# LongmaoTeamTf/deep_recommenders

Measured on AMD Instinct MI355X. Metric: examples/sec/node DeepFM (26 sparse feats, 10M vocab, dim 64), higher is better.
Workload: dtype f32; 1 GPU; DeepFM Criteo-shape synthetic training step (BASELINE.json configs[2]): 26 sparse + 13 dense, 10000000 vocab/field hashed on device, dim 64, DNN [256, 32]+[1] relu, sigmoid-CE, fused SGD; batch 65536 per GPU, ids uniform; tables on one GPU (66.6 GB); gemm_split=f16x2, global_batch=65536, parallelism=single, per_kernel_events=False

## Files before the change

### deep_recommenders_amd/_lib.py

```python
import ctypes
import os

_HERE = os.path.dirname(os.path.abspath(__file__))
SO_PATH = os.path.join(_HERE, "lib", "libdr_hotpath.so")

_i64, _i32, _u64, _f32, _p = ctypes.c_int64, ctypes.c_int32, ctypes.c_uint64, ctypes.c_float, ctypes.c_void_p

SIGNATURES = {
    "dr_hash_bucket_i64": [_p, _i64, _i32, _p, _p, _p],
    "dr_hash_bucket_bytes": [_p, _p, _i64, _u64, _p, _p],
    "dr_vocab_lookup_i64": [_p, _i64, _p, _i32, _p, _p],
    "dr_vocab_lookup_bytes": [_p, _p, _i64, _p, _p, _i32, _p, _p],
    "dr_emb_pool_fwd": [_p, _i64, _i32, _i32, _p, _p, _p, _i32, _p, _p, _p, _i64, _p, _p, _p],
    "dr_emb_pool_bwd": [_p, _i64, _i32, _i32, _p, _p, _i32, _p, _i64, _p, _i64, _p, _p, _f32, _p, _p, _p, _p],
    "dr_fm2_fwd": [_p, _i64, _i32, _i32, _p, _p],
    "dr_fm2_bwd": [_p, _p, _i64, _i32, _i32, _p, _p],
    "dr_linear_fwd": [_p, _i64, _p, _i64, _p, _i64, _i32, _i32, _i32, _p, _i64, _p],
    "dr_linear_bwd_dx": [_p, _i64, _p, _i64, _i64, _i32, _i32, _p, _i64, _i32, _p, _i64, _p],
    "dr_linear_bwd_dw": [_p, _i64, _p, _i64, _i64, _i32, _i32, _f32, _p, _i64, _p, _p, _i64, _p],
    "dr_emb_pool_fwd_ex": [_p, _i64, _i32, _i32, _p, _p, _p, _i32, _p, _p, _p, _i64, _p, _p, _i32, _p],
    "dr_lin_fields_fwd": [_p, _i64, _i32, _i32, _p, _p, _p, _p, _i64, _p],
    "dr_lin_fields_bwd": [_p, _i64, _i32, _i32, _p, _p, _p, _i64, _f32, _p, _p],
    "dr_emb_pool_bwd_sorted_adam": [_p, _p, _p, _p, _p, _p, _p, _i64, _i32, _i32, _i64, _p, _i64, _p, _i64, _p, _p, _p, _f32, _f32,
                                    _f32, _f32, _p, _p, _p, _p, _p, _p, _p, _p],
    "dr_emb_pool_bwd_sorted_adam_ex": [_p, _p, _p, _p, _p, _p, _p, _i64, _i32, _i32, _i64, _p, _i64, _p, _i64, _p, _p, _p, _f32, _f32,
                                    _f32, _f32, _p, _p, _p, _p, _p, _p, _p, _p, _p, _p],
    "dr_adam_step": [_p, _p, _p, _p, _i64, _f32, _f32, _f32, _f32, _f32, _p],
    "dr_ftrl_step": [_p, _p, _p, _p, _i64, _f32, _f32, _f32, _f32, _f32, _p],
    "dr_linear_bwd_dw_workspace_bytes": [_i64, _i32, _i32],
    "dr_linear_bwd_narrow_workspace_bytes": [_i64, _i32, _i32],
    "dr_tower_head_workspace_bytes": [_i64],
    "dr_tower_head_fwd_bwd": [_p, _i64, _p, _i64, _p, _i64, _i64, _i32, _i32, _i32, _p, _i64, _p, _p, _p, _i32, _f32, _p, _i64, _p,
                              _p, _i64, _p, _p, _p, _i64, _p, _p, _i64, _p],
    "dr_linear_bwd_narrow": [_p, _i64, _p, _i64, _p, _i64, _i64, _i32, _i32, _i32, _f32, _p, _i64, _p, _p, _i64, _p, _i64, _p],
    "dr_linear_bwd_narrow_parts": [_p, _i64, _p, _i64, _p, _i64, _i64, _i32, _i32, _i32, _f32, _p, _i64, _p, _p, _i64, _p, _i64, _i32, _p],
    "dr_linear_bwd_narrow_amax": [_p, _i64, _p, _i64, _p, _i64, _i64, _i32, _i32, _i32, _f32, _p, _i64, _p, _p, _i64, _p, _i64, _i32, _p, _p],
    "dr_tower_head_fwd_bwd_parts": [_p, _i64, _p, _i64, _p, _i64, _i64, _i32, _i32, _i32, _p, _i64, _p, _p, _p, _i32, _f32, _p, _i64, _p,
                                    _p, _i64, _p, _p, _p, _i64, _p, _p, _i64, _i32, _p],
    "dr_cross_fwd": [_p, _p, _i64, _p, _i64, _p, _f32, _i64, _i32, _p, _p, _p],
    "dr_cross_combine_bwd": [_p, _p, _p, _i64, _i32, _i64, _f32, _p, _p, _p, _p],
    "dr_bce_fwd_bwd": [_p, _p, _i64, _p, _i64, _i32, _p, _p, _p, _p, _p],
    "dr_sigmoid_fwd": [_p, _i64, _p, _p],
    "dr_sigmoid_bwd": [_p, _p, _i64, _p, _p],
    "dr_bce_prob_fwd_bwd": [_p, _p, _i64, _i32, _p, _p, _p, _p],
    "dr_shard_bucket_workspace_bytes": [_i64, _i32],
    "dr_shard_bucket_ids": [_p, _i64, _i32, _i64, _i32, _p, _p, _p, _p, _p],
    "dr_shard_bucket_ids_dedup": [_p, _p, _i64, _i32, _i64, _i32, _p, _p, _p, _p, _p],
    "dr_shard_dedup_slots": [_p, _p, _p, _i64, _i64, _p, _p],
    "dr_rows_gather": [_p, _i64, _p, _i32, _p, _p, _p, _p],
    "dr_rows_scatter_add": [_p, _i64, _p, _i32, _p, _f32, _p, _p, _p],
    "dr_axpy": [_i64, _f32, _p, _p, _p],
    "dr_emb_pack_grads": [_p, _i64, _i32, _i32, _p, _i64, _p, _i64, _p, _p, _p, _p, _p, _p],
    "dr_emb_pack_grads_dedup": [_p, _p, _i64, _i32, _i32, _p, _i64, _p, _i64, _p, _p, _p, _p, _p, _p],
    "dr_emb_sort_workspace_bytes": [_i64],
    "dr_emb_sort_slots": [_p, _i64, _i32, _p, _i64, _p, _p, _p, _p, _p, _p, _i64, _p],
    "dr_hash_sort_slots": [_p, _i64, _i32, _p, _p, _p, _p, _i64, _p, _p, _p, _p, _p, _p, _i64, _p],
    "dr_emb_plan_set_small_limit": [_i32],
    "dr_adam_catchup_rows": [_p, _i64, _i32, _p, _i32, _p, _p, _p, _p, _p, _p, _p, _i32, _i32, _f32, _f32, _f32, _f32, _p],
    "dr_emb_pool_bwd_sorted": [_p, _p, _p, _p, _p, _p, _p, _i64, _i32, _i32, _i64, _p, _i64, _p, _i64, _p, _p, _p, _f32, _p, _p,
                               _p, _p, _p],
    "dr_emb_pool_bwd_sorted_parts": [_p, _p, _p, _p, _p, _p, _p, _i64, _i32, _i32, _i64, _p, _i64, _p, _i64, _p, _p, _p, _f32, _p, _p,
                                     _p, _p, _i32, _p],
    "dr_emb_pool_bwd_sorted_ex": [_p, _p, _p, _p, _p, _p, _p, _i64, _i32, _i32, _i64, _p, _i64, _p, _i64, _p, _p, _p, _f32, _p, _p,
                                  _p, _p, _p, _i32, _p, _p],
    "dr_emb_lin_update_unique": [_p, _p, _i64, _i32, _p, _p, _p, _f32, _p, _p],
    "dr_emb_snapshot_sorted_rows": [_p, _p, _p, _p, _i32, _i64, _p, _p],
    "dr_ids_transpose_i32": [_p, _i64, _i32, _p, _p],
    "dr_linear_bwd_dx_fm": [_p, _i64, _p, _i64, _i64, _i32, _i32, _p, _p, _p, _i64, _i32, _i32, _p, _i64, _p],
    "dr_inbatch_softmax_workspace_bytes": [_i64],
    "dr_inbatch_softmax_fwd": [_p, _p, _i64, _i32, _p, _p, _p, _f32, _p, _p, _p, _p, _i64, _p],
    "dr_inbatch_softmax_grad_scores": [_p, _p, _i64, _i32, _p, _p, _p, _f32, _p, _f32, _p, _i64, _p],
    "dr_inbatch_softmax_grad_scores_ws": [_p, _p, _i64, _i32, _p, _p, _p, _f32, _p, _f32, _p, _i64, _p, _i64, _p],
    "dr_scores_nt": [_p, _i64, _p, _i64, _i64, _i32, _i32, _p, _i64, _p],
    "dr_topk_select": [_p, _i64, _i64, _i64, _i32, _i64, _i32, _p, _p, _p],
    "dr_topk_workspace_bytes": [_i64, _i64, _i32],
    "dr_topk_mips": [_p, _i64, _p, _i64, _i32, _i32, _i64, _i32, _p, _p, _p, _i64, _p],
    "dr_topk_index_bytes": [_i64, _i32],
    "dr_topk_index_build": [_p, _i64, _i32, _p, _i64, _p],
    "dr_topk_mips_indexed": [_p, _i64, _p, _p, _i64, _i32, _i32, _i64, _i32, _p, _p, _p, _i64, _p],
    "dr_ivf_pack": [_p, _i64, _i32, _p, _p, _p, _i32, _i64, _p, _p, _p, _p],
    "dr_ivf_scan": [_p, _i64, _i32, _p, _i32, _p, _p, _p, _i32, _p, _p, _p],
    "dr_topk_merge": [_p, _p, _i32, _p, _p, _i32, _i64, _i32, _p, _p, _p],
    "dr_rowdot": [_p, _p, _i64, _i32, _p, _p],
    "dr_rows_scale": [_p, _p, _i32, _p, _i64, _i32, _p, _p],
    "dr_gather_i64": [_p, _i64, _p, _i64, _p, _p],
    "dr_take_along_rows_f32": [_p, _i64, _i64, _i32, _p, _i32, _p, _p],
    "dr_take_along_rows_i64": [_p, _i64, _i64, _i32, _p, _i32, _p, _p],
    "dr_topk_hits": [_p, _p, _i64, _i32, _p, _i32, _p, _p],
    "dr_exclude_adjust": [_p, _p, _i64, _i32, _p, _i32, _p, _p],
    "dr_logits_adjust": [_p, _p, _i64, _i32, _p, _p, _f32, _p, _p],
    "dr_softmax_ce_rows": [_p, _p, _i64, _i32, _f32, _p, _p, _p, _p],
    "dr_softmax_ce_rows_bwd": [_p, _p, _i64, _i32, _f32, _p, _f32, _p, _p, _i64, _p],
    "dr_bf3_split": [_p, _i64, _i64, _i32, _p, _i64, _i64, _i64, _i64, _i32, _p],
    "dr_bf3_join": [_p, _i64, _i64, _i64, _i32, _p, _i64, _p],
    "dr_bf3_gemm_nt": [_p, _i64, _i64, _p, _i64, _i64, _i64, _i32, _i32, _p, _i32, _p, _i64, _p, _i64, _p],
    "dr_bf3_linear_nt": [_p, _i64, _p, _i64, _i64, _i64, _i32, _i32, _p, _i32, _p, _i64, _i32, _p, _i64, _p],
    "dr_bf3_linear_nt_pack": [_p, _i64, _p, _i64, _i64, _i64, _i32, _i32, _p, _i32, _p, _p, _p, _i64, _p, _p, _p, _p],
    "dr_h2_linear_nt_pack": [_p, _i64, _p, _p, _i64, _i64, _p, _i64, _i32, _i32, _p, _i32, _p, _p, _p, _i64, _p, _p, _p, _p],
    "dr_bf3_cross_fwd": [_p, _p, _i64, _p, _i64, _i64, _p, _f32, _i64, _i32, _p, _p, _p],
    "dr_linear_fwd_splitk_workspace_bytes": [_i64, _i32, _i32],
    "dr_linear_fwd_splitk": [_p, _i64, _p, _i64, _i64, _i32, _i32, _p, _i64, _p, _i64, _p],
    "dr_bf3_emb_linear_fwd": [_p, _i64, _i32, _p, _i64, _p, _i32, _p, _p, _p, _p, _i64, _i32, _p, _i64, _i64, _i32, _p, _i32, _p, _p, _p, _i64, _p],
    "dr_bf3_emb_linear_fwd_lv": [_p, _i64, _i32, _p, _i64, _p, _i32, _p, _p, _p, _p, _i64, _i32, _p, _i64, _i64, _i32, _p, _i32, _p, _p, _p, _i64,
                                 _p, _p],
    "dr_bf3_wgrad_workspace_bytes": [_i64, _i32, _i32],
    "dr_bf3_wgrad": [_p, _i64, _p, _i64, _i64, _i32, _i32, _f32, _p, _i64, _p, _p, _i64, _p],
    "dr_bf3_wgrad_emb": [_p, _i64, _i32, _p, _p, _i32, _p, _p, _i64, _i32, _i32, _f32, _p, _i64, _p, _p, _i64, _p],
    "dr_bf3_wgrad_emb_parts": [_p, _i64, _i32, _p, _p, _i32, _p, _p, _i64, _i32, _i32, _f32, _p, _i64, _p, _p, _i64, _i32, _p],
    "dr_bf3_gemm_tn_workspace_bytes": [_i64, _i32, _i32],
    "dr_bf3_gemm_tn": [_p, _i64, _i64, _p, _i64, _i64, _i64, _i32, _i32, _f32, _p, _i64, _p, _p, _p, _i64, _p],
    "dr_h2_amax": [_p, _i64, _i64, _i32, _p, _i32, _p],
    "dr_h2_split": [_p, _i64, _i64, _i32, _p, _i64, _i64, _i64, _i64, _i32, _p, _p],
    "dr_h2_refresh_weight": [_p, _i64, _i64, _i32, _p, _i64, _i64, _p, _i64, _i64, _p, _p, _p],
    "dr_h2_linear_nt": [_p, _i64, _p, _p, _i64, _i64, _p, _i64, _i32, _i32, _p, _i32, _p, _i64, _i32, _p, _i64, _p, _p],
    "dr_h2_cross_fwd": [_p, _p, _i64, _p, _p, _i64, _i64, _p, _p, _f32, _i64, _i32, _p, _p, _p, _p],
    "dr_h2_dgrad_emb_sgd": [_p, _i64, _p, _p, _i64, _i64, _p, _i64, _i32, _i32, _p, _p, _p, _p, _p, _p, _p, _p, _f32, _p, _i64, _p, _p],
    "dr_cross_combine_bwd_amax": [_p, _p, _p, _i64, _i32, _i64, _f32, _p, _p, _p, _p, _p],
    "dr_h2_emb_linear_fwd": [_p, _i64, _i32, _p, _i64, _p, _i32, _p, _p, _p, _p, _p, _p, _i64, _i32, _p, _i64, _i64, _p, _i32, _p, _i32,
                             _p, _p, _p, _i64, _p, _p],
    "dr_h2_wgrad": [_p, _i64, _p, _p, _i64, _p, _i64, _i32, _i32, _f32, _p, _i64, _p, _p, _i64, _p],
    "dr_h2_wgrad_emb": [_p, _i64, _i32, _p, _p, _i32, _p, _p, _p, _p, _i64, _p, _i32, _i32, _f32, _p, _i64, _p, _p, _i64, _i32, _p],
    "dr_cin_fwd": [_p, _p, _i64, _i32, _i32, _i32, _p, _i32, _p, _i32, _p, _p],
    "dr_cin_bwd": [_p, _p, _i64, _i32, _i32, _i32, _p, _i32, _i32, _p, _p, _p, _p, _p, _p, _p],
    "dr_cin_pool_fwd": [_p, _p, _i64, _i32, _i32, _i32, _p, _i32, _p, _i32, _p, _p, _p],
    "dr_cin_pool_bwd_workspace_bytes": [_i64, _i32, _i32, _i32, _i32],
    "dr_cin_pool_bwd": [_p, _p, _i64, _i32, _i32, _i32, _p, _i32, _i32, _p, _p, _p, _p, _i32, _p, _p, _p, _p, _i64, _p],
    "dr_din_concat_fwd": [_p, _p, _i64, _i32, _i32, _p, _i64, _p],
    "dr_din_concat_bwd": [_p, _p, _i64, _i32, _i32, _p, _i64, _p, _p, _p],
    "dr_act_fwd": [_p, _i64, _i32, _i64, _i32, _p],
    "dr_act_bwd": [_p, _i64, _p, _i64, _i64, _i32, _i32, _p],
    "dr_dropout_fwd": [_p, _i64, _i64, _i32, _f32, _u64, _p, _i64, _p, _p],
    "dr_dropout_bwd": [_p, _i64, _p, _i64, _i32, _f32, _p, _i64, _p],
    "dr_reduce_sum": [_p, _i64, _i32, _f32, _i32, _p, _p, _p],
    "dr_clock_stamp": [_p, _p],
    "dr_tower_tail_workspace_bytes": [_i64, _i32],
    "dr_tower_tail_fused": [_p, _i64, _p, _i64, _p, _i64, _i64, _i32, _i32, _p, _i64, _p, _p, _p, _i32, _f32, _p, _i64, _p, _p, _i64, _p,
                            _p, _p, _p, _i64, _p, _i64, _p, _p, _i64, _i32, _p, _p],
    "dr_copy_nt": [_p, _p, _i64, _p],
    "dr_ivf_build_workspace_bytes": [_i64, _i32],
    "dr_ivf_build_lists": [_p, _i64, _i32, _p, _p, _p, _i64, _p],
    "dr_linear_fwd_grouped": [_p, _i64, _i64, _p, _i64, _i64, _p, _i64, _i64, _i32, _i32, _i32, _i32, _p, _i64, _i64, _p],
    "dr_linear_bwd_dx_grouped": [_p, _i64, _i64, _p, _i64, _i64, _i64, _i32, _i32, _i32, _p, _i64, _i64, _i32, _p, _i64, _i64, _p],
    "dr_linear_bwd_dw_grouped_workspace_bytes": [_i64, _i32, _i32, _i32],
    "dr_linear_bwd_dw_grouped": [_p, _i64, _i64, _p, _i64, _i64, _i64, _i32, _i32, _i32, _f32, _p, _i64, _i64, _p, _i64, _p, _i64, _p],
    "dr_mmoe_gate_mix_fwd": [_p, _i64, _p, _i64, _i64, _i32, _i32, _i32, _p, _i64, _p, _i64, _p],
    "dr_mmoe_gate_mix_bwd": [_p, _i64, _p, _i64, _p, _i64, _i64, _i32, _i32, _i32, _p, _i64, _p, _i64, _p],
    "dr_mse_workspace_bytes": [_i32],
    "dr_mse_fwd_bwd": [_p, _i64, _p, _i64, _i64, _i32, _p, _p, _i64, _p, _i64, _p],
    "dr_esmm_head_fwd": [_p, _i64, _i64, _p, _p, _p, _p],
    "dr_esmm_head_bwd": [_p, _p, _p, _p, _p, _i64, _p, _i64, _p],
    "dr_adam_step_2d": [_p, _i64, _p, _i64, _p, _p, _i64, _i64, _i32, _f32, _f32, _f32, _f32, _f32, _p],
    "dr_gather_cols": [_p, _i64, _p, _i64, _p, _i64, _i32, _p, _i64, _p],
    "dr_csr_plan_bytes": [_i64],
    "dr_csr_plan_workspace_bytes": [_i64],
    "dr_csr_plan": [_p, _i64, _i64, _p, _i64, _p, _i64, _p],
    "dr_csr_spmm_workspace_bytes": [_i64, _i32],
    "dr_csr_spmm": [_p, _p, _p, _i64, _i64, _p, _i64, _i32, _p, _i64, _i32, _p, _i64, _p, _p, _i64, _p],
    "dr_csr_transpose_workspace_bytes": [_i64, _i64],
    "dr_csr_transpose": [_p, _p, _p, _i64, _i64, _i64, _p, _p, _p, _p, _i64, _p],
    "dr_softmax_rows_fwd": [_p, _i64, _i64, _i32, _p, _i64, _p],
    "dr_softmax_rows_bwd": [_p, _i64, _p, _i64, _i64, _i32, _p, _i64, _p],
    "dr_cce_prob_rows": [_p, _i64, _p, _i64, _i64, _i32, _p, _p, _p, _i64, _p],
    "dr_attn_fwd": [_p, _i64, _p, _i64, _p, _i64, _p, _i32, _i32, _i32, _i32, _i32, _i32, _f32, _u64, _p, _i64, _p, _p],
    "dr_attn_bwd": [_p, _i64, _p, _i64, _p, _i64, _p, _p, _i64, _p, _i32, _i32, _i32, _i32, _i32, _i32, _f32, _u64, _p, _i64,
                    _p, _i64, _p, _i64, _p, _p],
    "dr_add_layernorm_fwd": [_p, _i64, _p, _i64, _p, _p, _i64, _i32, _f32, _p, _i64, _p, _p],
    "dr_add_layernorm_bwd_workspace_bytes": [_i64, _i32],
    "dr_add_layernorm_bwd": [_p, _i64, _p, _i64, _p, _p, _p, _i64, _i64, _i32, _p, _i64, _p, _p, _p, _i64, _p],
    "dr_token_embedding_fwd": [_p, _i64, _i32, _p, _i64, _i32, _p, _f32, _u64, _p, _i64, _p],
    "dr_token_embedding_bwd": [_p, _p, _i64, _i64, _i32, _p, _i64, _f32, _u64, _p, _p],
    "dr_dice_fwd": [_p, _i64, _p, _i64, _i32, _f32, _p, _i64, _p],
    "dr_dice_bwd_workspace_bytes": [_i64, _i32],
    "dr_dice_bwd": [_p, _i64, _p, _p, _i64, _i64, _i32, _f32, _p, _i64, _p, _p, _i64, _p],
    "dr_din_pool_fwd": [_p, _i64, _p, _i64, _p, _p, _p, _p, _p, _p, _i64, _i32, _i32, _i32, _i32, _i32, _f32, _p, _i64, _p, _p],
    "dr_din_pool_bwd_workspace_bytes": [_i64, _i32, _i32, _i32],
    "dr_din_pool_bwd": [_p, _i64, _p, _i64, _p, _p, _p, _p, _p, _p, _p, _i64, _p, _i64, _i32, _i32, _i32, _i32, _i32, _f32,
                        _p, _i64, _p, _i64, _p, _p, _p, _p, _p, _p, _i64, _p],
    "dr_confusion_hist_workspace_bytes": [_i64, _i32],
    "dr_confusion_hist_update": [_p, _p, _p, _i64, _p, _i32, _i32, _p, _p, _p],
    "dr_version": [],
    "dr_set_gemm_mode": [_i32],
    "dr_get_gemm_mode": [],
    "dr_set_gemm_split": [_i32],
    "dr_get_gemm_split": [],
}
_RESTYPE = {"dr_version": ctypes.c_char_p, "dr_shard_bucket_workspace_bytes": ctypes.c_int64,
            "dr_emb_sort_workspace_bytes": ctypes.c_int64, "dr_tower_tail_workspace_bytes": ctypes.c_int64, "dr_ivf_build_workspace_bytes": ctypes.c_int64,
            "dr_linear_bwd_dw_workspace_bytes": ctypes.c_int64,
            "dr_linear_fwd_splitk_workspace_bytes": ctypes.c_int64,
            "dr_bf3_gemm_tn_workspace_bytes": ctypes.c_int64,
            "dr_bf3_wgrad_workspace_bytes": ctypes.c_int64,
            "dr_linear_bwd_narrow_workspace_bytes": ctypes.c_int64,
            "dr_tower_head_workspace_bytes": ctypes.c_int64,
            "dr_inbatch_softmax_workspace_bytes": ctypes.c_int64, "dr_topk_workspace_bytes": ctypes.c_int64,
            "dr_topk_index_bytes": ctypes.c_int64,
            "dr_linear_bwd_dw_grouped_workspace_bytes": ctypes.c_int64, "dr_mse_workspace_bytes": ctypes.c_int64,
            "dr_csr_plan_bytes": ctypes.c_int64, "dr_csr_plan_workspace_bytes": ctypes.c_int64,
            "dr_csr_spmm_workspace_bytes": ctypes.c_int64, "dr_csr_transpose_workspace_bytes": ctypes.c_int64,
            "dr_add_layernorm_bwd_workspace_bytes": ctypes.c_int64,
            "dr_dice_bwd_workspace_bytes": ctypes.c_int64, "dr_din_pool_bwd_workspace_bytes": ctypes.c_int64,
            "dr_confusion_hist_workspace_bytes": ctypes.c_int64, "dr_cin_pool_bwd_workspace_bytes": ctypes.c_int64}

DR_OK, DR_EINVAL, DR_ELAUNCH, DR_ESHAPE = 0, -1, -2, -3
_ERR = {DR_EINVAL: "DR_EINVAL (bad argument)", DR_ELAUNCH: "DR_ELAUNCH (HIP launch error)",
        DR_ESHAPE: "DR_ESHAPE (shape contract violated)"}

_LIB = None


class HotPathLibraryMissing(RuntimeError):
    pass


def lib():
    global _LIB
    if _LIB is None:
        if not os.path.exists(SO_PATH):
            raise HotPathLibraryMissing(
                "HIP hot-path library not built: %s is missing. Build it with "
                "`python -m deep_recommenders_amd.build` (or __graft_entry__.build()). "
                "There is no CPU/PyTorch fallback." % SO_PATH)
        L = ctypes.CDLL(SO_PATH)
        for name, args in SIGNATURES.items():
            fn = getattr(L, name)
            fn.argtypes = args
            fn.restype = _RESTYPE.get(name, ctypes.c_int)
        _LIB = L
    return _LIB


def check(status, what):
    if status != DR_OK:
        raise RuntimeError("%s failed: %s" % (what, _ERR.get(status, status)))


def ptr(t):
    if t is None:
        return None
    if not t.is_cuda:
# ... 18 lines not shown
```

### deep_recommenders_amd/csrc/bf3_planes.hip

```cpp
#include "bf3_rs_core.h"

namespace {

using namespace drrs;

constexpr int NWAVES = 8;
constexpr int NTHREADS = 64 * NWAVES;

struct NtArgs {
    const __bf16* A; int64_t a_ps, a_ld;
    const __bf16* B; int64_t b_ps, b_ld;
    int64_t M; int32_t N; int32_t K;
    float* C; int64_t ldc;
    const float* bias; int32_t act;
    const float* mask; int64_t ld_mask;
};


template <int NW, int DBG = 0>
__global__ __launch_bounds__(64 * NW, NW / 4) void bf3_gemm_nt_pipe_kernel(NtArgs g) {
    constexpr int BM = 128, BN = 128, NS = 3;
    constexpr int WN = 4, WM = NW / WN, TM = BM / (32 * WM);
    constexpr int A_PLANE = BM * 64, B_PLANE = BN * 64;
    constexpr int STAGE = 3 * (A_PLANE + B_PLANE);
// ... 480 lines not shown
                                                       _Float16* __restrict__ planes, int64_t ps, int64_t ldp, int64_t r0,
                                                       int64_t c0, int32_t transpose, const uint32_t* __restrict__ amax) {
    float sc, inv;
    h2_scale_of(amax[0], sc, inv);
    h2_mode_on();
    const int64_t total = R * C, stride = (int64_t)gridDim.x * blockDim.x;
    if (!transpose && (C & 3) == 0 && (ldp & 3) == 0 && (c0 & 3) == 0 && (ld_src & 3) == 0 && (reinterpret_cast<uintptr_t>(src) & 15) == 0 &&
        (reinterpret_cast<uintptr_t>(planes) & 7) == 0 && (ps & 3) == 0 && total < (int64_t)0x7fffffff) {
        typedef _Float16 f16x4 __attribute__((ext_vector_type(4)));
        typedef float f32x4 __attribute__((ext_vector_type(4)));
        const unsigned cq = (unsigned)C >> 2, tq = (unsigned)(total >> 2);
        for (unsigned i = blockIdx.x * blockDim.x + threadIdx.x; i < tq; i += (unsigned)stride) {
            const unsigned r = i / cq, c = (i - r * cq) << 2;
            const f32x4 v = *reinterpret_cast<const f32x4*>(src + (int64_t)r * ld_src + c) * sc;
            const f16x4 h = __builtin_convertvector(v, f16x4);
            const f16x4 l = __builtin_convertvector(v - __builtin_convertvector(h, f32x4), f16x4);
            const int64_t off = (r0 + r) * ldp + c0 + c;
            *reinterpret_cast<f16x4*>(planes + off) = h;
            *reinterpret_cast<f16x4*>(planes + ps + off) = l;
        }
        return;
    }
    for (int64_t i = (int64_t)blockIdx.x * blockDim.x + threadIdx.x; i < total; i += stride) {
        int64_t r, c, off;
        if (!transpose) { r = i / C; c = i - r * C; off = (r0 + r) * ldp + c0 + c; }
        else { c = i / R; r = i - c * R; off = (r0 + c) * ldp + c0 + r; }
        const float v = src[r * ld_src + c] * sc;
        const _Float16 h = (_Float16)v;
        planes[off] = h;
        planes[ps + off] = (_Float16)(v - (float)h);
    }
}

constexpr int H2_REFRESH_PARTS = 256;
__global__ __launch_bounds__(256) void h2_amax_parts_kernel(const float* __restrict__ src, int64_t ld, int64_t R, int32_t C,
                                                            uint32_t* __restrict__ parts) {
    uint32_t m = 0u;
    const int64_t total = R * (int64_t)C, stride = (int64_t)gridDim.x * blockDim.x;
    for (int64_t i = (int64_t)blockIdx.x * blockDim.x + threadIdx.x; i < total; i += stride) {
        const int64_t r = i / C;
        m = max(m, __float_as_uint(fabsf(src[r * ld + (i - r * C)])));
    }
#pragma unroll
    for (int o = 32; o > 0; o >>= 1) m = max(m, (uint32_t)__shfl_xor((int)m, o, 64));
    __shared__ uint32_t wm[4];
    if ((threadIdx.x & 63) == 0) wm[threadIdx.x >> 6] = m;
    __syncthreads();
    if (threadIdx.x == 0) parts[blockIdx.x] = max(max(wm[0], wm[1]), max(wm[2], wm[3]));
}
__global__ __launch_bounds__(256) void h2_split_both_kernel(const float* __restrict__ src, int64_t ld, int64_t R, int32_t C,
                                                            _Float16* __restrict__ w, int64_t w_ps, int64_t w_ld,
                                                            _Float16* __restrict__ wt, int64_t wt_ps, int64_t wt_ld,
                                                            const uint32_t* __restrict__ parts, int32_t nparts, uint32_t* __restrict__ amax) {
    uint32_t m = (int)threadIdx.x < nparts ? parts[threadIdx.x] : 0u;
#pragma unroll
    for (int o = 32; o > 0; o >>= 1) m = max(m, (uint32_t)__shfl_xor((int)m, o, 64));
    __shared__ uint32_t wm[4];
    if ((threadIdx.x & 63) == 0) wm[threadIdx.x >> 6] = m;
    __syncthreads();
    m = max(max(wm[0], wm[1]), max(wm[2], wm[3]));
    if (blockIdx.x == 0 && threadIdx.x == 0) amax[0] = m;
    float sc, inv;
    h2_scale_of(m, sc, inv);
    h2_mode_on();
    const int64_t total = R * (int64_t)C, stride = (int64_t)gridDim.x * blockDim.x;
    for (int64_t i = (int64_t)blockIdx.x * blockDim.x + threadIdx.x; i < 2 * total; i += stride) {
        int64_t r, c, off;
        _Float16* dst;
        int64_t ps;
        if (i < total) { r = i / C; c = i - r * C; off = r * w_ld + c; dst = w; ps = w_ps; }
        else { const int64_t j = i - total; c = j / R; r = j - c * R; off = c * wt_ld + r; dst = wt; ps = wt_ps; }
        const float v = src[r * ld + c] * sc;
        const _Float16 h = (_Float16)v;
        dst[off] = h;
        dst[ps + off] = (_Float16)(v - (float)h);
    }
}

__global__ __launch_bounds__(256) void bf3_join_kernel(const __bf16* __restrict__ planes, int64_t ps, int64_t ldp, int64_t R,
                                                       int32_t C, float* __restrict__ dst, int64_t ld_dst) {
    const int64_t total = R * C, stride = (int64_t)gridDim.x * blockDim.x;
    for (int64_t i = (int64_t)blockIdx.x * blockDim.x + threadIdx.x; i < total; i += stride) {
        const int64_t r = i / C;
        const int c = (int)(i - r * C);
        const int64_t off = r * ldp + c;
        dst[r * ld_dst + c] = bf3::join(planes[off], planes[ps + off], planes[2 * ps + off]);
    }
}

}

extern "C" int dr_bf3_split(const float* src, int64_t ld_src, int64_t R, int32_t C, void* planes, int64_t plane_stride,
                            int64_t ld_planes, int64_t row_offset, int64_t col_offset, int32_t transpose,
                            dr_stream_t stream) {
    if (R < 0 || C < 0 || ld_src < C || row_offset < 0 || col_offset < 0 || ld_planes <= 0 || plane_stride <= 0) return DR_EINVAL;
    if (R == 0 || C == 0) return DR_OK;
    if (!src || !planes) return DR_EINVAL;
    if (!transpose && col_offset + C > ld_planes) return DR_EINVAL;
    if (transpose && col_offset + R > ld_planes) return DR_EINVAL;
    hipLaunchKernelGGL(bf3_split_kernel, dim3(dr_grid_for(R * ((C + 3) / 4), 256)), dim3(256), 0, dr_s(stream), src, ld_src, R, C,
                       static_cast<__bf16*>(planes), plane_stride, ld_planes, row_offset, col_offset, transpose);
    DR_CHECK_LAUNCH();
    return DR_OK;
}

extern "C" int dr_bf3_join(const void* planes, int64_t plane_stride, int64_t ld_planes, int64_t R, int32_t C, float* dst,
                           int64_t ld_dst, dr_stream_t stream) {
    if (R < 0 || C < 0 || ld_planes < C || ld_dst < C || plane_stride <= 0) return DR_EINVAL;
    if (R == 0 || C == 0) return DR_OK;
    if (!planes || !dst) return DR_EINVAL;
    hipLaunchKernelGGL(bf3_join_kernel, dim3(dr_grid_for(R * C, 256)), dim3(256), 0, dr_s(stream),
                       static_cast<const __bf16*>(planes), plane_stride, ld_planes, R, C, dst, ld_dst);
    DR_CHECK_LAUNCH();
    return DR_OK;
}

extern "C" int dr_bf3_gemm_nt(const void* a_planes, int64_t a_plane_stride, int64_t a_ld, const void* b_planes,
                              int64_t b_plane_stride, int64_t b_ld, int64_t M, int32_t N, int32_t K, const float* bias,
                              int32_t act, const float* mask, int64_t ld_mask, float* C, int64_t ldc, dr_stream_t stream) {
    if (M < 0 || N <= 0 || K <= 0 || (K % BK) != 0 || act < 0 || act > 1) return DR_EINVAL;
    if (M == 0) return DR_OK;
    if (!planes_ok(a_planes, a_plane_stride, a_ld) || !planes_ok(b_planes, b_plane_stride, b_ld) || !C) return DR_EINVAL;
    if (a_ld < K || b_ld < K || ldc < N || (mask != nullptr && ld_mask < N)) return DR_EINVAL;
    NtArgs g{static_cast<const __bf16*>(a_planes), a_plane_stride, a_ld, static_cast<const __bf16*>(b_planes), b_plane_stride, b_ld,
             M, N, K, C, ldc, bias, act, mask, ld_mask};
    const int64_t tiles = ((M + 127) / 128) * ((N + 127) / 128);
    if (tiles > 0x7fffffff) return DR_EINVAL;
    const int grid = (int)(tiles < 256 ? tiles : 256);
    hipLaunchKernelGGL((bf3_gemm_nt_pipe_kernel<16>), dim3(grid), dim3(1024), 0, dr_s(stream), g);
    DR_CHECK_LAUNCH();
    return DR_OK;
// ... 14 lines not shown
    if (workspace_bytes < dr_bf3_gemm_tn_workspace_bytes(R, F, N)) return DR_EINVAL;
    TnArgs g{static_cast<const __bf16*>(x_planes), x_plane_stride, x_ld, static_cast<const __bf16*>(y_planes), y_plane_stride, y_ld,
             R, F, N, 0, 0, static_cast<float*>(workspace)};
    int split = tn_split_for(R, F, N, 128, 256);
    const int64_t rpad = (R + BK - 1) / BK * BK;
    g.per = ((rpad + split - 1) / split + BK - 1) / BK * BK;
    g.split = (int32_t)((rpad + g.per - 1) / g.per);
    const int64_t tiles = (int64_t)((F + 127) / 128) * ((N + 255) / 256) * g.split;
    const int grid = (int)(tiles < 256 ? tiles : 256);
    hipLaunchKernelGGL((bf3_gemm_tn_kernel<2, 4>), dim3(grid), dim3(NTHREADS), 0, dr_s(stream), g);
    hipLaunchKernelGGL(bf3_splitk_reduce_kernel, dim3(dr_grid_for((int64_t)F * N, 256)), dim3(256), 0, dr_s(stream), g.partial,
                       g.split, (int64_t)F, N, scale, dst, ld_dst, y_colsum, dstb);
    DR_CHECK_LAUNCH();
    return DR_OK;
}

extern "C" int dr_h2_amax(const float* src, int64_t ld, int64_t R, int32_t C, uint32_t* amax, int32_t reset, dr_stream_t stream) {
    if (R < 0 || C < 0 || ld < C || !amax) return DR_EINVAL;
    if (reset && hipMemsetAsync(amax, 0, sizeof(uint32_t), dr_s(stream)) != hipSuccess) return DR_ELAUNCH;
    if (R == 0 || C == 0) return DR_OK;
    if (!src) return DR_EINVAL;
    const int grid = (ld == C || R == 1) ? dr_grid_for(R * ((C + 3) / 4), 256 * 4) : (int)(R < 4096 ? R : 4096);
    hipLaunchKernelGGL(h2_amax_kernel, dim3(grid), dim3(256), 0, dr_s(stream), src, ld, R, C, amax);
    DR_CHECK_LAUNCH();
    return DR_OK;
}

extern "C" int dr_h2_split(const float* src, int64_t ld_src, int64_t R, int32_t C, void* planes, int64_t plane_stride,
                           int64_t ld_planes, int64_t row_offset, int64_t col_offset, int32_t transpose, const uint32_t* amax,
                           dr_stream_t stream) {
    if (R < 0 || C < 0 || ld_src < C || row_offset < 0 || col_offset < 0 || ld_planes <= 0 || plane_stride <= 0 || !amax) return DR_EINVAL;
    if (R == 0 || C == 0) return DR_OK;
    if (!src || !planes) return DR_EINVAL;
    if (!transpose && col_offset + C > ld_planes) return DR_EINVAL;
    if (transpose && col_offset + R > ld_planes) return DR_EINVAL;
    hipLaunchKernelGGL(h2_split_kernel, dim3(dr_grid_for(R * (int64_t)C, 256)), dim3(256), 0, dr_s(stream), src, ld_src, R, C,
                       static_cast<_Float16*>(planes), plane_stride, ld_planes, row_offset, col_offset, transpose, amax);
    DR_CHECK_LAUNCH();
    return DR_OK;
}

extern "C" int dr_h2_refresh_weight(const float* W, int64_t ldw, int64_t K, int32_t N, void* w_planes, int64_t w_ps, int64_t w_ld,
                                    void* wt_planes, int64_t wt_ps, int64_t wt_ld, uint32_t* amax, uint32_t* parts, dr_stream_t stream) {
    if (K <= 0 || N <= 0 || ldw < N || !W || !w_planes || !wt_planes || !amax || !parts) return DR_EINVAL;
    if (w_ld < N || wt_ld < K || w_ps <= 0 || wt_ps <= 0) return DR_EINVAL;
    const int64_t total = K * (int64_t)N;
    const int np = (int)(total < (int64_t)H2_REFRESH_PARTS * 256 ? (total + 255) / 256 : H2_REFRESH_PARTS);
    hipLaunchKernelGGL(h2_amax_parts_kernel, dim3(np), dim3(256), 0, dr_s(stream), W, ldw, K, N, parts);
    hipLaunchKernelGGL(h2_split_both_kernel, dim3(dr_grid_for(2 * total, 256, 2048)), dim3(256), 0, dr_s(stream), W, ldw, K, N,
                       static_cast<_Float16*>(w_planes), w_ps, w_ld, static_cast<_Float16*>(wt_planes), wt_ps, wt_ld, parts, np, amax);
    DR_CHECK_LAUNCH();
    return DR_OK;
}
```

### deep_recommenders_amd/csrc/bf3_wgrad.hip

```cpp
#ifndef DR_NT_WGRAD_GATHER
#define DR_NT_WGRAD_GATHER 0
#endif
#include "bf3_rs_core.h"

namespace {

using namespace drrs;

struct TnRsArgs {
    const float* X; int64_t ldx;
    const float* Y; int64_t ldy;
    int64_t R; int32_t F; int32_t N;
    int64_t per; int32_t split;
    float* partial; float* colsum;
    const int32_t* ids_t; const int64_t* row_base; const float* table; int32_t nf; const float* dense_pad;
    const uint32_t* x_amax; const uint32_t* x2_amax; const uint32_t* y_amax;
};

template <int GATHER, int H2 = 0>
__global__ __launch_bounds__(512, 2) void bf3_gemm_tn_rs_kernel(TnRsArgs g) {
    constexpr int NW = 8, BMF = 32 * NW, BN = 256, NT = BN / 32;
    constexpr int NPL = RS_NPL<H2>, B_PLANE = RS_B_PLANE, STAGE = RS_STAGE<H2>;
    __shared__ __attribute__((aligned(1024))) unsigned char smem[2 * STAGE];

// ... 156 lines not shown
#pragma unroll
            for (int s = 0; s < 2; ++s) {
#pragma unroll
                for (int j = 0; j < 8; ++j) v[j] = xa[8 * s + j];
                if constexpr (H2) h2_split8v(v, h2_sx, fa[s][0], fa[s][1]);
                else rs_split8v(v, fa[s][0], fa[s][1], fa[s][2]);
            }
        }
        if (kt + 1 < nk) stage_b(stage ^ 1);
        __builtin_amdgcn_sched_barrier(0);
        if (GATHER) {
            load_gather(xa, idv, r_begin + (int64_t)(kt + 1) * BK);
            idv = load_ids(r_begin + (int64_t)(kt + 2) * BK);
        } else {
            load_raw(xa, g.X, g.ldx, xoff, r_begin + (int64_t)(kt + 1) * BK);
        }
        load_raw(yb, g.Y, g.ldy, yoff, r_begin + (int64_t)(kt + 2) * BK);
        __builtin_amdgcn_sched_barrier(0);
#pragma unroll
        for (int q = 0; q < 16; ++q) {
            if (q < 14) {
                rs_wait_frag<NPL, NPL>(fb[q & 3]);
                read_b((q + 2) & 3, stage, q + 2);
            } else if (q == 14) {
                rs_wait_frag<NPL, 0>(fb[2]);
                asm volatile("s_barrier" ::: "memory");
                if (kt + 1 < nk) read_b(0, stage ^ 1, 0);
            } else {
                if (kt + 1 < nk) read_b(1, stage ^ 1, 1);
            }
            __builtin_amdgcn_sched_barrier(0);
#pragma unroll
            for (int term = 0; term < RS_TERMS<H2>; ++term) acc[q & 7] = rs_mma_term<H2>(term, fa[q >> 3], fb[q & 3], acc[q & 7]);
            __builtin_amdgcn_sched_barrier(0);
        }
    }
    float* out = g.partial + ((int64_t)slice * Fp + f0 + wave * 32 + 4 * hi) * Np + n0 + l31;
#pragma unroll
    for (int nt = 0; nt < NT; ++nt)
#pragma unroll
        for (int reg = 0; reg < 16; ++reg) out[(int64_t)((reg & 3) + 8 * (reg >> 2)) * Np + nt * 32] = acc[nt][reg];
    if (want_cs) {
        cs += __shfl_xor(cs, 32, 64);
        if (hi == 0) g.colsum[(int64_t)slice * Np + n0 + wave * 32 + l31] = cs;
    }
}

template <int V>
__global__ __launch_bounds__(64) void bf3_tn_rs_reduce_kernel(const float* __restrict__ partial, const float* __restrict__ colsum,
                                                              int32_t split, int32_t F, int32_t N, int32_t Fp, int32_t Np,
                                                              float scale, float* __restrict__ dst, int64_t ld,
                                                              float* __restrict__ dstb, const uint32_t* __restrict__ x_amax = nullptr,
                                                              const uint32_t* __restrict__ x2_amax = nullptr,
                                                              const uint32_t* __restrict__ y_amax = nullptr) {
    typedef float vec_t __attribute__((ext_vector_type(V)));
    const int f = blockIdx.x;
    const int n = ((int)blockIdx.y * 64 + (int)threadIdx.x) * V;
    if (n >= N) return;
    const int64_t ps = (int64_t)Fp * Np;
    float wscale = scale;
    if (x_amax != nullptr) {
        float sx, ix, sy, iy;
        h2_scale_of(max(x_amax[0], x2_amax != nullptr ? x2_amax[0] : 0u), sx, ix);
        h2_scale_of(y_amax[0], sy, iy);
        wscale = scale * (ix * iy);
    }
    auto sum_slices = [&](const float* p, int64_t stride) -> vec_t {
        vec_t acc = 0.f;
        int s = 0;
        for (; s + 8 <= split; s += 8) {
            vec_t v[8];
#pragma unroll
            for (int u = 0; u < 8; ++u) v[u] = *reinterpret_cast<const vec_t*>(p + (s + u) * stride);
#pragma unroll
            for (int u = 0; u < 8; ++u) acc += v[u];
        }
        for (; s < split; ++s) acc += *reinterpret_cast<const vec_t*>(p + s * stride);
        return acc;
    };
    const vec_t acc = sum_slices(partial + (int64_t)f * Np + n, ps);
    float* d = dst + (int64_t)f * ld + n;
    if (V == 1 || n + V <= N) {
        vec_t o = *reinterpret_cast<vec_t*>(d);
#pragma unroll
        for (int c = 0; c < V; ++c) o[c] = fmaf(wscale, acc[c], o[c]);
        *reinterpret_cast<vec_t*>(d) = o;
    } else {
#pragma unroll
        for (int c = 0; c < V; ++c)
            if (n + c < N) d[c] = fmaf(wscale, acc[c], d[c]);
    }
    if (f == 0 && colsum != nullptr && dstb != nullptr) {
        const vec_t cacc = sum_slices(colsum + n, Np);
#pragma unroll
        for (int c = 0; c < V; ++c)
            if (n + c < N) dstb[n + c] = fmaf(scale, cacc[c], dstb[n + c]);
    }
}

void launch_tn_rs_reduce(const float* partial, const float* colsum, int split, int32_t F, int32_t N, int Fp, int Np, float scale,
                         float* dst, int64_t ld, float* dstb, const uint32_t* x_amax, const uint32_t* x2_amax, const uint32_t* y_amax,
                         dr_stream_t stream) {
    const bool vec = ((reinterpret_cast<uintptr_t>(partial) | reinterpret_cast<uintptr_t>(dst)) & 15) == 0 && (ld & 3) == 0;
    if (vec)
        hipLaunchKernelGGL(bf3_tn_rs_reduce_kernel<4>, dim3(F, (N + 255) / 256), dim3(64), 0, dr_s(stream), partial, colsum, split, F, N,
                           Fp, Np, scale, dst, ld, dstb, x_amax, x2_amax, y_amax);
    else
        hipLaunchKernelGGL(bf3_tn_rs_reduce_kernel<1>, dim3(F, (N + 63) / 64), dim3(64), 0, dr_s(stream), partial, colsum, split, F, N,
                           Fp, Np, scale, dst, ld, dstb, x_amax, x2_amax, y_amax);
}

void tn_rs_plan(int64_t R, int32_t F, int32_t N, int& split, int64_t& per, int& Fp, int& Np) {
    const int tf = (F + 255) / 256, tn = (N + 255) / 256;
    Fp = tf * 256;
    Np = tn * 256;
    int64_t sp = 256 / ((int64_t)tf * tn);
    const int64_t max_split = (R + 16 * BK - 1) / (16 * BK);
    if (sp > max_split) sp = max_split;
    if (sp < 1) sp = 1;
    per = ((R + sp - 1) / sp + BK - 1) / BK * BK;
    split = (int)((R + per - 1) / per);
}
}

extern "C" int64_t dr_bf3_wgrad_workspace_bytes(int64_t R, int32_t F, int32_t N) {
    if (R <= 0 || F <= 0 || N <= 0) return 0;
    int split, Fp, Np;
    int64_t per;
    tn_rs_plan(R, F, N, split, per, Fp, Np);
    return ((int64_t)split * Fp * Np + (int64_t)split * Np) * (int64_t)sizeof(float);
}

static int wgrad_impl(const float* x, int64_t ld_x, const float* dy, int64_t ld_dy, int64_t R, int32_t F, int32_t N,
                      float scale, float* dstW, int64_t ld_w, float* dstb, void* workspace, int64_t workspace_bytes,
                      dr_stream_t stream, const uint32_t* x_amax = nullptr, const uint32_t* dy_amax = nullptr) {
    if (R <= 0 || F <= 0 || N <= 0) return DR_EINVAL;
    if (!x || !dy || !dstW || !workspace || ld_x < F || ld_dy < N || ld_w < N) return DR_EINVAL;
    if (workspace_bytes < dr_bf3_wgrad_workspace_bytes(R, F, N)) return DR_EINVAL;
    int split, Fp, Np;
    int64_t per;
    tn_rs_plan(R, F, N, split, per, Fp, Np);
    float* partial = static_cast<float*>(workspace);
    float* colsum = partial + (int64_t)split * Fp * Np;
    TnRsArgs g{x, ld_x, dy, ld_dy, R, F, N, per, split, partial, dstb != nullptr ? colsum : nullptr, nullptr, nullptr, nullptr, 0, nullptr,
               x_amax, nullptr, dy_amax};
    const int grid = (Fp / 256) * (Np / 256) * split;
    if (x_amax != nullptr) hipLaunchKernelGGL((bf3_gemm_tn_rs_kernel<0, 1>), dim3(grid), dim3(512), 0, dr_s(stream), g);
    else hipLaunchKernelGGL((bf3_gemm_tn_rs_kernel<0, 0>), dim3(grid), dim3(512), 0, dr_s(stream), g);
    launch_tn_rs_reduce(partial, dstb != nullptr ? colsum : nullptr, split, F, N, Fp, Np, scale, dstW, ld_w, dstb, x_amax, nullptr, dy_amax,
                        stream);
    DR_CHECK_LAUNCH();
    return DR_OK;
}

extern "C" int dr_bf3_wgrad(const float* x, int64_t ld_x, const float* dy, int64_t ld_dy, int64_t R, int32_t F, int32_t N,
                            float scale, float* dstW, int64_t ld_w, float* dstb, void* workspace, int64_t workspace_bytes,
                            dr_stream_t stream) {
    return wgrad_impl(x, ld_x, dy, ld_dy, R, F, N, scale, dstW, ld_w, dstb, workspace, workspace_bytes, stream);
}

extern "C" int dr_h2_wgrad(const float* x, int64_t ld_x, const uint32_t* x_amax, const float* dy, int64_t ld_dy, const uint32_t* dy_amax,
                           int64_t R, int32_t F, int32_t N, float scale, float* dstW, int64_t ld_w, float* dstb, void* workspace,
                           int64_t workspace_bytes, dr_stream_t stream) {
    if (!x_amax || !dy_amax) return DR_EINVAL;
    return wgrad_impl(x, ld_x, dy, ld_dy, R, F, N, scale, dstW, ld_w, dstb, workspace, workspace_bytes, stream, x_amax, dy_amax);
}

static int wgrad_emb_impl(const int32_t* ids_t, int64_t R, int32_t nf, const int64_t* row_base, const float* table, int32_t D,
                          const float* dense_pad, const float* dy, int64_t ld_dy, int32_t F, int32_t N, float scale, float* dstW,
                          int64_t ld_w, float* dstb, void* workspace, int64_t workspace_bytes, int32_t parts, dr_stream_t stream,
                          const uint32_t* table_amax = nullptr, const uint32_t* dense_amax = nullptr, const uint32_t* dy_amax = nullptr) {
    if (R <= 0 || F <= 0 || N <= 0 || nf <= 0) return DR_EINVAL;
    if (table_amax != nullptr && (!dy_amax || (F > 64 * nf && !dense_amax))) return DR_EINVAL;
    if (D != 64 || F < 64 * nf || F > 64 * nf + 32) return DR_ESHAPE;
    if (!ids_t || !row_base || !table || !dy || !dstW || !workspace || ld_dy < N || ld_w < N) return DR_EINVAL;
    if (F > 64 * nf && !dense_pad) return DR_EINVAL;
    if (workspace_bytes < dr_bf3_wgrad_workspace_bytes(R, F, N)) return DR_EINVAL;
    int split, Fp, Np;
    int64_t per;
    tn_rs_plan(R, F, N, split, per, Fp, Np);
    float* partial = static_cast<float*>(workspace);
    float* colsum = partial + (int64_t)split * Fp * Np;
    TnRsArgs g{nullptr, 0, dy, ld_dy, R, F, N, per, split, partial, dstb != nullptr ? colsum : nullptr, ids_t, row_base, table, nf,
               F > 64 * nf ? dense_pad : nullptr, table_amax, F > 64 * nf ? dense_amax : nullptr, dy_amax};
    const int grid = (Fp / 256) * (Np / 256) * split;
    if (parts & 1) {
        if (table_amax != nullptr) hipLaunchKernelGGL((bf3_gemm_tn_rs_kernel<1, 1>), dim3(grid), dim3(512), 0, dr_s(stream), g);
        else hipLaunchKernelGGL((bf3_gemm_tn_rs_kernel<1, 0>), dim3(grid), dim3(512), 0, dr_s(stream), g);
    }
    if (parts & 2)
        launch_tn_rs_reduce(partial, dstb != nullptr ? colsum : nullptr, split, F, N, Fp, Np, scale, dstW, ld_w, dstb, table_amax,
                            F > 64 * nf ? dense_amax : nullptr, dy_amax, stream);
    DR_CHECK_LAUNCH();
    return DR_OK;
}

extern "C" int dr_bf3_wgrad_emb(const int32_t* ids_t, int64_t R, int32_t nf, const int64_t* row_base, const float* table, int32_t D,
                                const float* dense_pad, const float* dy, int64_t ld_dy, int32_t F, int32_t N, float scale, float* dstW,
                                int64_t ld_w, float* dstb, void* workspace, int64_t workspace_bytes, dr_stream_t stream) {
    return wgrad_emb_impl(ids_t, R, nf, row_base, table, D, dense_pad, dy, ld_dy, F, N, scale, dstW, ld_w, dstb, workspace, workspace_bytes,
                          3, stream);
}

extern "C" int dr_bf3_wgrad_emb_parts(const int32_t* ids_t, int64_t R, int32_t nf, const int64_t* row_base, const float* table, int32_t D,
                                      const float* dense_pad, const float* dy, int64_t ld_dy, int32_t F, int32_t N, float scale,
                                      float* dstW, int64_t ld_w, float* dstb, void* workspace, int64_t workspace_bytes, int32_t parts,
                                      dr_stream_t stream) {
    if (parts < 1 || parts > 3) return DR_EINVAL;
    return wgrad_emb_impl(ids_t, R, nf, row_base, table, D, dense_pad, dy, ld_dy, F, N, scale, dstW, ld_w, dstb, workspace, workspace_bytes,
                          parts, stream);
}

extern "C" int dr_h2_wgrad_emb(const int32_t* ids_t, int64_t R, int32_t nf, const int64_t* row_base, const float* table, int32_t D,
                               const uint32_t* table_amax, const float* dense_pad, const uint32_t* dense_amax, const float* dy, int64_t ld_dy,
                               const uint32_t* dy_amax, int32_t F, int32_t N, float scale, float* dstW, int64_t ld_w, float* dstb,
                               void* workspace, int64_t workspace_bytes, int32_t parts, dr_stream_t stream) {
    if (parts < 1 || parts > 3 || !table_amax || !dy_amax) return DR_EINVAL;
    return wgrad_emb_impl(ids_t, R, nf, row_base, table, D, dense_pad, dy, ld_dy, F, N, scale, dstW, ld_w, dstb, workspace, workspace_bytes,
                          parts, stream, table_amax, dense_amax, dy_amax);
}
```

### deep_recommenders_amd/csrc/dr_common.h

```cpp
#pragma once
#include <hip/hip_runtime.h>
#include <stdint.h>
#include "../../include/dr_hotpath.h"

#define DR_WAVE 64

#define DR_CHECK_LAUNCH()                                   \
    do {                                                    \
        hipError_t e__ = hipGetLastError();                 \
        if (e__ != hipSuccess) return DR_ELAUNCH;           \
    } while (0)

static inline hipStream_t dr_s(dr_stream_t s) { return reinterpret_cast<hipStream_t>(s); }

static inline int dr_grid_for(int64_t work_items, int items_per_block, int max_blocks = 2048) {
    int64_t g = (work_items + items_per_block - 1) / items_per_block;
    if (g < 1) g = 1;
    if (g > max_blocks) g = max_blocks;
    return (int)g;
}

__device__ __forceinline__ float dr_wave_sum(float v) {
#pragma unroll
    for (int o = 32; o > 0; o >>= 1) v += __shfl_xor(v, o, 64);
    return v;
}

__host__ __device__ __forceinline__ uint32_t dr_mix32(uint64_t seed, uint64_t idx) {
    uint64_t z = idx * 0x9E3779B97F4A7C15ull + seed;
    z = (z ^ (z >> 30)) * 0xBF58476D1CE4E5B9ull;
    z = (z ^ (z >> 27)) * 0x94D049BB133111EBull;
    return (uint32_t)((z ^ (z >> 31)) >> 32);
}
__host__ __device__ __forceinline__ uint32_t dr_drop_thresh(float rate) {
    return (uint32_t)fminf(4294967040.f, rate * 4294967296.f);
}

__device__ __forceinline__ float dr_sigmoidf(float x) { return 1.f / (1.f + expf(-x)); }

__device__ __forceinline__ void dr_bce_terms(float x, float z, int mode, float& p, float& l, float& g) {
    p = 1.f / (1.f + expf(-x));
    if (mode == 0) {
        l = fmaxf(x, 0.f) - x * z + log1pf(expf(-fabsf(x)));
        g = p - z;
    } else {
        const float eps = 1e-7f;
        float pc = p;
        float dclip = 1.f;
        if (mode == 2) {
            if (p < eps) { pc = eps; dclip = 0.f; }
            else if (p > 1.f - eps) { pc = 1.f - eps; dclip = 0.f; }
        }
        l = -z * logf(pc + eps) - (1.f - z) * logf(1.f - pc + eps);
        const float dl_dp = -z / (pc + eps) + (1.f - z) / (1.f - pc + eps);
        g = dl_dp * dclip * p * (1.f - p);
    }
}

__device__ __forceinline__ void dr_block_sum_axpy(const float* __restrict__ x, int64_t n, float alpha,
                                                  float* __restrict__ dst) {
    __shared__ float dr_wsum_[4];
    float acc = 0.f;
    const int64_t nv = (reinterpret_cast<uintptr_t>(x) & 15) == 0 ? (n >> 2) : 0;
    const float4* x4 = reinterpret_cast<const float4*>(x);
    for (int64_t i = threadIdx.x; i < nv; i += 256 * 4) {
        float4 a[4];
#pragma unroll
        for (int j = 0; j < 4; ++j) {
            const int64_t q = i + j * 256;
            a[j] = x4[q < nv ? q : i];
            if (q >= nv) a[j] = make_float4(0.f, 0.f, 0.f, 0.f);
        }
#pragma unroll
        for (int j = 0; j < 4; ++j) acc += (a[j].x + a[j].y) + (a[j].z + a[j].w);
    }
    for (int64_t i = (nv << 2) + threadIdx.x; i < n; i += 256) acc += x[i];
    acc = dr_wave_sum(acc);
    if ((threadIdx.x & 63) == 0) dr_wsum_[threadIdx.x >> 6] = acc;
// ... 4 lines not shown
```

### deep_recommenders_amd/csrc/emb_plan.hip

```cpp
#include "dr_common.h"
#include "hash_i64.h"
#include <atomic>

namespace {

constexpr int CH = 32;
constexpr uint32_t EMPTY = 0xFFFFFFFFu;
constexpr uint32_t DUPBIT = 0x80000000u;
constexpr int SMALL_CAP = 16384;
constexpr int RADIX_BITS = 8, RADIX = 1 << RADIX_BITS;
constexpr int NBK = RADIX, CAPB = 128;
constexpr int LDS_TAB_MAX_LOG = 15;
constexpr int RADIX_CHUNK = 1664, RADIX_MAX_BLOCKS = 1024;
constexpr int MARK_BLOCKS = 512, MARK_MAX_CHUNK = 8192;
static_assert(NBK * CAPB >= SMALL_CAP, "buckets must hold the largest SMALL list");

std::atomic<int> g_small_limit{SMALL_CAP};

struct Ctrl {
    int32_t large;
    int32_t pad[3];
    int32_t bcnt[NBK];
};

size_t align_up(size_t v, size_t a) { return (v + a - 1) / a * a; }

unsigned bits_for(uint64_t v) {
    unsigned b = 1;
    while (b < 64 && (v >> b) != 0) ++b;
    return b;
}

__device__ __forceinline__ unsigned bits_for_dev(uint32_t v) { return v == 0 ? 1u : 32u - (unsigned)__clz((int)v); }

int radix_blocks(int64_t n) {
    int64_t nb = (n + RADIX_CHUNK - 1) / RADIX_CHUNK;
    return (int)(nb < 1 ? 1 : (nb > RADIX_MAX_BLOCKS ? RADIX_MAX_BLOCKS : nb));
}

struct Layout {
    size_t keys_x, vals_x, blist, ghist, tot, ctrl, total;
};
Layout layout_for(int64_t n) {
    Layout L{};
    size_t off = 0;
    L.keys_x = off; off += align_up((size_t)n * 8, 256);
    L.vals_x = off; off += align_up((size_t)n * 4, 256);
    L.blist = off;  off += align_up((size_t)NBK * CAPB * 8, 256);
    L.ghist = off;  off += align_up((size_t)RADIX * RADIX_MAX_BLOCKS * 4, 256);
    L.tot = off;    off += align_up((size_t)RADIX * 4, 256);
    L.ctrl = off;   off += align_up(sizeof(Ctrl), 256);
    L.total = off;
    return L;
}

template <int MODE>
__device__ __forceinline__ uint32_t digit_of(uint64_t k, uint32_t shift_or_mul) {
    if (MODE == 0) return (uint32_t)(k >> shift_or_mul) & (RADIX - 1);
    const uint32_t d = (uint32_t)(((k >> 24) * shift_or_mul) >> 32);
    return d < RADIX - 1 ? d : RADIX - 1;
}

__global__ __launch_bounds__(256) void radix_make_keys_kernel(const int64_t* __restrict__ ids, int32_t n, int32_t F,
                                                              const int64_t* __restrict__ row_base, uint64_t sentinel,
                                                              uint64_t* __restrict__ keys, uint32_t* __restrict__ vals) {
    const int32_t stride = gridDim.x * blockDim.x;
    for (int32_t p = blockIdx.x * blockDim.x + threadIdx.x; p < n; p += stride) {
        const int64_t id = ids[p];
        const uint64_t r0 = id >= 0 ? (uint64_t)(row_base[p % F] + id) : sentinel;
        keys[p] = r0 < sentinel ? r0 : sentinel;
        vals[p] = (uint32_t)p;
    }
}

constexpr int FRONT_GROUP = 4;
template <bool HASH, bool TRANS>
__global__ __launch_bounds__(256) void plan_front_kernel(const int64_t* __restrict__ src, int64_t B, int32_t F,
                                                         const uint64_t* __restrict__ col_buckets, int64_t* __restrict__ ids_out,
                                                         int32_t* __restrict__ ids_t, const int64_t* __restrict__ row_base,
                                                         uint64_t sentinel, uint32_t mul, int32_t sub, uint64_t* __restrict__ keys,
                                                         uint32_t* __restrict__ ghist) {
    extern __shared__ uint64_t fsm[];
    __shared__ uint32_t h[RADIX];
    int64_t* rb = reinterpret_cast<int64_t*>(fsm);
    uint64_t* cb = fsm + F;
    int32_t* tile = reinterpret_cast<int32_t*>(fsm + (HASH ? 3 : 1) * F);
    const int nb = gridDim.x, t = threadIdx.x;
    for (int c = t; c < F; c += 256) {
        rb[c] = row_base[c];
        if (HASH) {
            const uint64_t nbk = col_buckets[c];
            cb[c] = nbk;
            cb[F + c] = nbk != 0 ? ~0ull / nbk : 0;
        }
    }
    h[t] = 0;
    __syncthreads();
    const int64_t e0 = (int64_t)blockIdx.x * sub;
    const int64_t e1 = e0 + sub < B ? e0 + sub : B;
    for (int64_t g0 = e0; g0 < e1; g0 += 64) {
        const int ge = (int)(e1 - g0 < 64 ? e1 - g0 : 64);
        const int ns = ge * F;
        const int64_t p0 = g0 * F;
        for (int q = t; q < ns; q += 256) {
            const int r = q / F, f = q - r * F;
            const int64_t p = p0 + q;
            int64_t id = src[p];
            if (HASH) {
                id = drhash::bucket_of_key(id, cb[f], cb[F + f]);
                ids_out[p] = id;
            }
            if (TRANS) tile[r * (F + 1) + f] = (int32_t)id;
            const uint64_t r0 = id >= 0 ? (uint64_t)(rb[f] + id) : sentinel;
            const uint64_t row = r0 < sentinel ? r0 : sentinel;
            const uint64_t ck = (row << 24) | (uint32_t)p;
            keys[p] = ck;
            atomicAdd(&h[digit_of<1>(ck, mul)], 1u);
        }
        if (TRANS) {
            __syncthreads();
            for (int q = t; q < F * 64; q += 256) {
                const int f = q >> 6, r = q & 63;
                if (r < ge) ids_t[(int64_t)f * B + g0 + r] = tile[r * (F + 1) + f];
            }
            __syncthreads();
        }
    }
    __syncthreads();
    ghist[t * nb + blockIdx.x] = h[t];
}

__global__ __launch_bounds__(256) void radix_hist_kernel(const uint64_t* __restrict__ keys, int32_t n, uint32_t shift,
                                                         uint32_t* __restrict__ ghist) {
    __shared__ uint32_t h[RADIX];
    const int nb = gridDim.x, t = threadIdx.x;
    const int32_t chunk = (n + nb - 1) / nb;
    const int32_t beg = (int32_t)blockIdx.x * chunk, end = beg + chunk < n ? beg + chunk : n;
    h[t] = 0;
    __syncthreads();
    for (int32_t i = beg + t; i < end; i += 256) atomicAdd(&h[digit_of<0>(keys[i], shift)], 1u);
    __syncthreads();
    ghist[t * nb + blockIdx.x] = h[t];
}

template <bool ZERO>
__global__ __launch_bounds__(256) void radix_scan_kernel(uint32_t* __restrict__ ghist, int32_t nb, uint32_t* __restrict__ tot,
                                                         Ctrl* __restrict__ ctrl, int32_t* __restrict__ dup_count) {
    if (ZERO && blockIdx.x == 0) {
        int32_t* c = reinterpret_cast<int32_t*>(ctrl);
        for (int i = threadIdx.x; i < (int)(sizeof(Ctrl) / 4); i += 256) c[i] = 0;
        if (threadIdx.x < 2) dup_count[threadIdx.x] = 0;
    }
    __shared__ uint32_t part[256];
    const int t = threadIdx.x, d = blockIdx.x;
    const int32_t per = (nb + 255) / 256;
    const int32_t beg = t * per, end = beg + per < nb ? beg + per : nb;
    uint32_t* col = ghist + (int64_t)d * nb;
    uint32_t sum = 0;
    for (int32_t i = beg; i < end; ++i) sum += col[i];
    part[t] = sum;
    __syncthreads();
    for (int o = 1; o < 256; o <<= 1) {
        const uint32_t x = t >= o ? part[t - o] : 0u;
        __syncthreads();
        part[t] += x;
        __syncthreads();
    }
    uint32_t run = part[t] - sum;
    for (int32_t i = beg; i < end; ++i) {
        const uint32_t c = col[i];
        col[i] = run;
        run += c;
    }
    if (t == 255) tot[d] = part[255];
}

__global__ __launch_bounds__(256) void radix_scatter_kernel(const uint64_t* __restrict__ kin, const uint32_t* __restrict__ vin,
                                                            uint64_t* __restrict__ kout, uint32_t* __restrict__ vout, int32_t n,
                                                            uint32_t shift, const uint32_t* __restrict__ ghist,
                                                            const uint32_t* __restrict__ tot) {
    __shared__ uint32_t running[RADIX];
    __shared__ uint32_t wcnt[4][RADIX];
// ... 123 lines not shown
    const int hsh = 32 - log_tab;
    if (t < RADIX) starts[t] = tot[t];
    if (t == 0) ndup = 0;
    for (int i = t; i < LDS_TAB; i += CLAIM_T) tab[i] = EMPTY;
    __syncthreads();
    uint32_t beg = 0;
    for (int i = 0; i < b; ++i) beg += starts[i];
    const uint32_t cnt = starts[b];
    if (cnt > (uint32_t)(LDS_TAB / 10 * 7)) {
        if (t == 0) ctrl->large = 1;
        return;
    }
    for (uint32_t i = t; i < cnt; i += CLAIM_T) {
        const uint64_t k = keys[beg + i] >> 24;
        if (k >= num_rows) continue;
        const uint32_t r = (uint32_t)k;
        uint32_t h = (r * 2654435761u) >> hsh;
        for (;;) {
            const uint32_t old = atomicCAS(&tab[h], EMPTY, r);
            if (old == EMPTY) break;
            if ((old & ~DUPBIT) == r) {
                if (!(old & DUPBIT)) atomicOr(&tab[h], DUPBIT);
                break;
            }
            h = (h + 1) & (LDS_TAB - 1);
        }
    }
    __syncthreads();
    for (uint32_t i = t; i < cnt; i += CLAIM_T) {
        const uint64_t ck = keys[beg + i];
        const uint64_t k = ck >> 24;
        const uint32_t slot = (uint32_t)(ck & 0xFFFFFFu);
        bool dup = false;
        if (k < num_rows) {
            const uint32_t r = (uint32_t)k;
            uint32_t h = (r * 2654435761u) >> hsh;
            uint32_t v = tab[h];
            while ((v & ~DUPBIT) != r) {
                h = (h + 1) & (LDS_TAB - 1);
                v = tab[h];
            }
            dup = (v & DUPBIT) != 0;
            if (dup) {
                const int pos = atomicAdd(&ndup, 1);
                if (pos < CAPB) blist[b * CAPB + pos] = ((uint64_t)r << 24) | slot;
            }
        }
        flags[slot] = (k < num_rows && !dup) ? 1 : 0;
    }
    __syncthreads();
    if (t == 0) ctrl->bcnt[b] = ndup;
}

__global__ __launch_bounds__(256) void plan_bucket_sort_kernel(const uint64_t* __restrict__ blist, Ctrl* __restrict__ ctrl,
                                                               int32_t small_limit, uint64_t* __restrict__ rows,
                                                               int32_t* __restrict__ slots, int32_t* __restrict__ dup_heads,
                                                               int32_t* __restrict__ dup_count) {
    __shared__ uint64_t s[CAPB];
    __shared__ int32_t cnts[NBK];
    __shared__ int32_t nheads, hbase;
    const int t = threadIdx.x, b = blockIdx.x;
    if (ctrl->large != 0) return;
    if (t < NBK) cnts[t] = ctrl->bcnt[t];
    if (t == 0) nheads = 0;
    __syncthreads();
    int32_t m = 0, off = 0;
    bool over = false;
    for (int i = 0; i < NBK; ++i) {
        const int32_t c = cnts[i];
        over |= c > CAPB;
        if (i < b) off += c;
        m += c;
    }
    if (over || m > small_limit) {
        if (b == 0 && t == 0) ctrl->large = 1;
        return;
    }
    const int cnt = cnts[b];
    int n2 = 64;
    while (n2 < cnt) n2 <<= 1;
    if (t < n2) s[t] = t < cnt ? blist[b * CAPB + t] : ~0ull;
    __syncthreads();
    for (int k = 2; k <= n2; k <<= 1) {
        for (int j = k >> 1; j > 0; j >>= 1) {
            if (t < (n2 >> 1)) {
                const int i = ((t & ~(j - 1)) << 1) | (t & (j - 1));
                const int ixj = i | j;
                const uint64_t x = s[i], y = s[ixj];
                const bool asc = (i & k) == 0;
                if ((x > y) == asc) {
                    s[i] = y;
                    s[ixj] = x;
                }
            }
            __syncthreads();
        }
    }
    const bool in = t < cnt;
    const int gi = off + t;
    bool head = false;
    if (in) {
        const uint64_t k = s[t] >> 24;
        rows[gi] = k;
        slots[gi] = (int32_t)(s[t] & 0xFFFFFFu);
        const bool seg_start = (t == 0) || ((s[t - 1] >> 24) != k);
        head = seg_start || ((gi % CH) == 0 && t >= CH && (s[t - CH] >> 24) == k);
    }
    const uint64_t bal = __ballot(head);
    const int lane = t & 63;
    int wbase = 0;
    if (bal != 0 && lane == __ffsll((unsigned long long)bal) - 1) wbase = atomicAdd(&nheads, __popcll(bal));
    __syncthreads();
    if (t == 0) hbase = nheads > 0 ? atomicAdd(&dup_count[0], nheads) : 0;
    __syncthreads();
    if (bal != 0) {
        wbase = __shfl(wbase, __ffsll((unsigned long long)bal) - 1, 64);
        if (head) dup_heads[hbase + wbase + __popcll(bal & ((1ull << lane) - 1ull))] = gi;
    }
    if (b == 0 && t == 0) dup_count[1] = m;
}

__global__ __launch_bounds__(256) void radix_mark_kernel(const uint64_t* __restrict__ rows, const int32_t* __restrict__ slots,
                                                         int32_t n, uint64_t num_rows, uint8_t* __restrict__ flags,
                                                         int32_t* __restrict__ dup_heads, int32_t* __restrict__ dup_count) {
    __shared__ int32_t hl[MARK_MAX_CHUNK];
    __shared__ int32_t nh, gbase;
    const int t = threadIdx.x, lane = t & 63;
    const int32_t chunk = (n + (int32_t)gridDim.x - 1) / (int32_t)gridDim.x;
    const int32_t beg = (int32_t)blockIdx.x * chunk, end = beg + chunk < n ? beg + chunk : n;
    if (blockIdx.x == 0 && t == 0) dup_count[1] = n;
    if (t == 0) nh = 0;
    __syncthreads();
    for (int32_t i0 = beg; i0 < end; i0 += 256) {
        const int32_t i = i0 + t;
        const bool in = i < end;
        const uint64_t k = in ? rows[i] : ~0ull;
        const bool valid = in && k < num_rows;
        const bool seg_start = in && ((i == 0) || (rows[i - 1] != k));
        const bool has_next = in && (i + 1 < n) && (rows[i + 1] == k);
        if (in) flags[slots[i]] = (valid && seg_start && !has_next) ? 1 : 0;
        const bool head = valid && ((seg_start && has_next) || (!seg_start && (i % CH) == 0 && i >= CH && rows[i - CH] == k));
        const uint64_t bal = __ballot(head);
        if (bal != 0) {
            const int leader = __ffsll((unsigned long long)bal) - 1;
            int base = 0;
            if (lane == leader) base = atomicAdd(&nh, __popcll(bal));
            base = __shfl(base, leader, 64);
            if (head) hl[base + __popcll(bal & ((1ull << lane) - 1ull))] = i;
        }
    }
    __syncthreads();
    if (t == 0) gbase = nh > 0 ? atomicAdd(dup_count, nh) : 0;
    __syncthreads();
    for (int j = t; j < nh; j += 256) dup_heads[gbase + j] = hl[j];
}

__global__ __launch_bounds__(LG_T) void plan_large_kernel(uint64_t* __restrict__ ka, const uint32_t* __restrict__ tot,
                                                          uint64_t num_rows, int32_t n, uint64_t* __restrict__ rows,
                                                          int32_t* __restrict__ slots, uint8_t* __restrict__ flags,
                                                          int32_t* __restrict__ dup_heads, int32_t* __restrict__ dup_count,
                                                          const Ctrl* __restrict__ ctrl) {
    if (ctrl->large == 0) return;
    __shared__ uint32_t running[RADIX];
    __shared__ uint32_t wcnt[LG_W][RADIX];
    __shared__ uint32_t starts[RADIX];
    __shared__ uint32_t rmin, rmax;
    __shared__ int32_t nh, gbase;
    const int t = threadIdx.x, b = blockIdx.x, lane = t & 63;
    if (t < RADIX) starts[t] = tot[t];
    if (t == 0) { rmin = 0xFFFFFFFFu; rmax = 0u; }
    if (b == 0 && t == 0) dup_count[1] = n;
    __syncthreads();
    uint32_t beg = 0;
    for (int i = 0; i < b; ++i) beg += starts[i];
    const int32_t cnt = (int32_t)starts[b];
    uint64_t* src = ka + beg;
    uint64_t* dst = rows + beg;
    {
        uint32_t lo = 0xFFFFFFFFu, hi = 0u;
        for (int32_t i = t; i < cnt; i += LG_T) {
            const uint32_t r = (uint32_t)(src[i] >> 24);
            lo = r < lo ? r : lo;
            hi = r > hi ? r : hi;
        }
        if (lo <= hi) { atomicMin(&rmin, lo); atomicMax(&rmax, hi); }
    }
    __syncthreads();
    const uint32_t base_row = rmin;
    int passes = 0;
    if (cnt > 1 && rmax > rmin) passes = (int)((bits_for_dev(rmax - rmin) + RADIX_BITS - 1) / RADIX_BITS);
    if (passes & 1) {
        for (int32_t i = t; i < cnt; i += LG_T) dst[i] = src[i];
        uint64_t* x = src; src = dst; dst = x;
        __syncthreads();
    }
    for (int p = 0; p < passes; ++p) {
        const uint32_t shift = (uint32_t)(p * RADIX_BITS);
        if (t < RADIX) running[t] = 0;
        __syncthreads();
        for (int32_t i = t; i < cnt; i += LG_T)
            atomicAdd(&running[(((uint32_t)(src[i] >> 24) - base_row) >> shift) & (RADIX - 1)], 1u);
        __syncthreads();
        {
            const uint32_t mine = t < RADIX ? running[t] : 0u;
            for (int o = 1; o < RADIX; o <<= 1) {
                const uint32_t x = (t < RADIX && t >= o) ? running[t - o] : 0u;
                __syncthreads();
                if (t < RADIX) running[t] += x;
                __syncthreads();
            }
            if (t < RADIX) running[t] -= mine;
        }
        __syncthreads();
        for (int32_t base = 0; base < cnt; base += LG_T) {
            const int32_t i = base + t;
            const bool live = i < cnt;
            const uint64_t k = live ? src[i] : 0ull;
            scatter_step_1024(live, k, (((uint32_t)(k >> 24) - base_row) >> shift) & (RADIX - 1), running, wcnt, dst);
        }
        uint64_t* x = src; src = dst; dst = x;
    }
    for (int32_t base = 0; base < cnt; base += LG_T) {
        const int32_t i = base + t;
        const bool in = i < cnt;
        const uint64_t ck = in ? src[i] : ~0ull;
        const uint64_t k = ck >> 24;
        const int32_t gi = (int32_t)beg + i;
        const bool valid = in && k < num_rows;
        const bool seg_start = in && (i == 0 || (src[i - 1] >> 24) != k);
        const bool has_next = in && (i + 1 < cnt) && (src[i + 1] >> 24) == k;
        if (in) {
            const int32_t slot = (int32_t)(ck & 0xFFFFFFu);
            rows[gi] = k;
            slots[gi] = slot;
            flags[slot] = (valid && seg_start && !has_next) ? 1 : 0;
        }
        const bool head = valid && ((seg_start && has_next) || (!seg_start && (gi % CH) == 0 && i >= CH && (src[i - CH] >> 24) == k));
        if (t == 0) nh = 0;
        __syncthreads();
        const uint64_t bal = __ballot(head);
        int wbase = 0;
        const int leader = bal != 0 ? __ffsll((unsigned long long)bal) - 1 : 0;
        if (bal != 0 && lane == leader) wbase = atomicAdd(&nh, __popcll(bal));
        __syncthreads();
        if (t == 0) gbase = nh > 0 ? atomicAdd(dup_count, nh) : 0;
        __syncthreads();
        if (bal != 0) {
            wbase = __shfl(wbase, leader, 64);
            if (head) dup_heads[gbase + wbase + __popcll(bal & ((1ull << lane) - 1ull))] = gi;
        }
    }
}

}

extern "C" int32_t dr_emb_plan_set_small_limit(int32_t limit) {
    if (limit < 0) limit = 0;
    if (limit > SMALL_CAP) limit = SMALL_CAP;
    return g_small_limit.exchange(limit);
}

extern "C" int64_t dr_emb_sort_workspace_bytes(int64_t n) {
    if (n <= 0) return 256;
    return (int64_t)layout_for(n).total;
}

namespace {
int plan_small_front(const int64_t* raw, const uint64_t* col_buckets, int64_t* ids_out, int32_t* ids_t, const int64_t* ids, int64_t B,
                     int32_t F, const int64_t* row_base, int64_t num_rows, uint64_t* rows_y, uint64_t* keys_x, uint32_t* ghist,
                     uint32_t* tot, Ctrl* ctrl, int32_t* dup_count, hipStream_t s) {
    const int64_t n64 = B * F;
    const int32_t n = (int32_t)n64;
    const uint32_t mul = (uint32_t)((((uint64_t)RADIX) << 32) / (uint64_t)num_rows);
    int64_t sub = 64;
    while ((B + sub - 1) / sub > RADIX_MAX_BLOCKS) sub += 64;
    const int nbf = (int)((B + sub - 1) / sub);
    const int nbs = (nbf + FRONT_GROUP - 1) / FRONT_GROUP;
    const int64_t chunk = sub * FRONT_GROUP * F;
    if (chunk > 0x7fffffff) return DR_EINVAL;
    const bool trans = ids_t != nullptr;
    const size_t lds = (size_t)8 * (raw ? 3 : 1) * F + (trans ? (size_t)4 * 64 * (F + 1) : 0);
    if (raw) {
        if (trans)
            hipLaunchKernelGGL((plan_front_kernel<true, true>), dim3(nbf), dim3(256), lds, s, raw, B, F, col_buckets, ids_out, ids_t, row_base,
                               (uint64_t)num_rows, mul, (int32_t)sub, rows_y, ghist);
        else
            hipLaunchKernelGGL((plan_front_kernel<true, false>), dim3(nbf), dim3(256), lds, s, raw, B, F, col_buckets, ids_out, ids_t,
                               row_base, (uint64_t)num_rows, mul, (int32_t)sub, rows_y, ghist);
    } else {
        hipLaunchKernelGGL((plan_front_kernel<false, false>), dim3(nbf), dim3(256), lds, s, ids, B, F, col_buckets, ids_out, ids_t, row_base,
                           (uint64_t)num_rows, mul, (int32_t)sub, rows_y, ghist);
    }
    hipLaunchKernelGGL((radix_scan_kernel<true>), dim3(RADIX), dim3(256), 0, s, ghist, (int32_t)nbf, tot, ctrl, dup_count);
    hipLaunchKernelGGL(plan_scatter_kernel, dim3(nbs), dim3(LG_T), 0, s, rows_y, keys_x, n, mul, (int32_t)chunk, ghist, (int32_t)nbf, tot);
    return DR_OK;
}

int sort_slots_impl(const int64_t* raw, const uint64_t* col_buckets, int32_t* ids_t, const int64_t* ids, int64_t B, int32_t F,
                    const int64_t* row_base, int64_t num_rows, int64_t* sorted_rows, int32_t* sorted_slots, uint8_t* unique_flags,
                    int32_t* dup_heads, int32_t* dup_count, void* workspace, int64_t workspace_bytes, dr_stream_t stream) {
    if (B < 0 || F <= 0 || num_rows <= 0) return DR_EINVAL;
    const int64_t n64 = B * F;
    if (n64 == 0) return DR_OK;
    if (n64 > 0x7fffff00) return DR_EINVAL;
    if (!ids || !row_base || !sorted_rows || !sorted_slots || !unique_flags || !dup_heads || !dup_count || !workspace)
        return DR_EINVAL;
    if (workspace_bytes < dr_emb_sort_workspace_bytes(n64)) return DR_EINVAL;
    const int32_t n = (int32_t)n64;
    const Layout L = layout_for(n64);
    char* w = static_cast<char*>(workspace);
    uint64_t* keys_x = reinterpret_cast<uint64_t*>(w + L.keys_x);
    uint32_t* vals_x = reinterpret_cast<uint32_t*>(w + L.vals_x);
    uint64_t* blist = reinterpret_cast<uint64_t*>(w + L.blist);
    uint32_t* ghist = reinterpret_cast<uint32_t*>(w + L.ghist);
    uint32_t* tot = reinterpret_cast<uint32_t*>(w + L.tot);
    Ctrl* ctrl = reinterpret_cast<Ctrl*>(w + L.ctrl);
    uint64_t* rows_y = reinterpret_cast<uint64_t*>(sorted_rows);
    uint32_t* slots_y = reinterpret_cast<uint32_t*>(sorted_slots);
    hipStream_t s = dr_s(stream);
    const int grid = dr_grid_for(n, 256);
    const int nb = radix_blocks(n);

    const bool claimable = n64 <= (1 << 24) && num_rows < 0x7fffffffLL;
    const bool fused_front = raw != nullptr && claimable && F <= 64;
    if (raw && !fused_front) {
        int rc = dr_hash_bucket_i64(raw, B, F, col_buckets, const_cast<int64_t*>(ids), stream);
        if (rc == DR_OK && ids_t) rc = dr_ids_transpose_i32(ids, B, F, ids_t, stream);
        if (rc != DR_OK) return rc;
    }
    if (claimable) {
        int rc = plan_small_front(fused_front ? raw : nullptr, col_buckets, const_cast<int64_t*>(ids), fused_front ? ids_t : nullptr, ids, B,
                                  F, row_base, num_rows, rows_y, keys_x, ghist, tot, ctrl, dup_count, s);
        if (rc != DR_OK) return rc;
        static const hipError_t lds_optin = hipFuncSetAttribute(reinterpret_cast<const void*>(plan_lds_claim_kernel),
                                                                hipFuncAttributeMaxDynamicSharedMemorySize, 4 << LDS_TAB_MAX_LOG);
        if (lds_optin != hipSuccess) return DR_ELAUNCH;
        int log_tab = 12;
        while (log_tab < LDS_TAB_MAX_LOG && (1 << log_tab) < 2 * ((n + NBK - 1) / NBK)) ++log_tab;
        hipLaunchKernelGGL(plan_lds_claim_kernel, dim3(NBK), dim3(CLAIM_T), (size_t)4 << log_tab, s, keys_x, tot, (uint64_t)num_rows,
                           (int32_t)log_tab, unique_flags, blist, ctrl);
        hipLaunchKernelGGL(plan_bucket_sort_kernel, dim3(NBK), dim3(256), 0, s, blist, ctrl, (int32_t)g_small_limit.load(), rows_y,
                           sorted_slots, dup_heads, dup_count);
        hipLaunchKernelGGL(plan_large_kernel, dim3(NBK), dim3(LG_T), 0, s, keys_x, tot, (uint64_t)num_rows, n, rows_y, sorted_slots,
                           unique_flags, dup_heads, dup_count, ctrl);
        DR_CHECK_LAUNCH();
        return DR_OK;
    }
    if (hipMemsetAsync(dup_count, 0, 2 * sizeof(int32_t), s) != hipSuccess) return DR_ELAUNCH;
    const unsigned bits = bits_for((uint64_t)num_rows);
    const int passes = (int)((bits + RADIX_BITS - 1) / RADIX_BITS);
    uint64_t* kbuf[2] = {keys_x, rows_y};
    uint32_t* vbuf[2] = {vals_x, slots_y};
    int cur = (passes & 1) ? 0 : 1;
    hipLaunchKernelGGL(radix_make_keys_kernel, dim3(grid), dim3(256), 0, s, ids, n, F, row_base, (uint64_t)num_rows, kbuf[cur], vbuf[cur]);
    for (int p = 0; p < passes; ++p) {
        const uint32_t shift = (uint32_t)(p * RADIX_BITS);
        hipLaunchKernelGGL(radix_hist_kernel, dim3(nb), dim3(256), 0, s, kbuf[cur], n, shift, ghist);
        hipLaunchKernelGGL((radix_scan_kernel<false>), dim3(RADIX), dim3(256), 0, s, ghist, (int32_t)nb, tot, ctrl, dup_count);
        hipLaunchKernelGGL(radix_scatter_kernel, dim3(nb), dim3(256), 0, s, kbuf[cur], vbuf[cur], kbuf[cur ^ 1], vbuf[cur ^ 1], n, shift, ghist,
                           tot);
        cur ^= 1;
    }
    int mark_blocks = MARK_BLOCKS;
    while ((n + mark_blocks - 1) / mark_blocks > MARK_MAX_CHUNK) mark_blocks *= 2;
    hipLaunchKernelGGL(radix_mark_kernel, dim3(mark_blocks), dim3(256), 0, s, rows_y, sorted_slots, n, (uint64_t)num_rows, unique_flags, dup_heads,
                       dup_count);
    DR_CHECK_LAUNCH();
    return DR_OK;
}
}

extern "C" int dr_emb_sort_slots(const int64_t* ids, int64_t B, int32_t F, const int64_t* row_base, int64_t num_rows,
                                 int64_t* sorted_rows, int32_t* sorted_slots, uint8_t* unique_flags, int32_t* dup_heads,
                                 int32_t* dup_count, void* workspace, int64_t workspace_bytes, dr_stream_t stream) {
    return sort_slots_impl(nullptr, nullptr, nullptr, ids, B, F, row_base, num_rows, sorted_rows, sorted_slots, unique_flags, dup_heads,
                           dup_count, workspace, workspace_bytes, stream);
}

extern "C" int dr_hash_sort_slots(const int64_t* keys, int64_t B, int32_t F, const uint64_t* col_buckets, int64_t* ids_out,
                                  int32_t* ids_t_out, const int64_t* row_base, int64_t num_rows, int64_t* sorted_rows,
                                  int32_t* sorted_slots, uint8_t* unique_flags, int32_t* dup_heads, int32_t* dup_count, void* workspace,
                                  int64_t workspace_bytes, dr_stream_t stream) {
    if (!keys || !col_buckets || !ids_out) return DR_EINVAL;
    return sort_slots_impl(keys, col_buckets, ids_t_out, ids_out, B, F, row_base, num_rows, sorted_rows, sorted_slots, unique_flags,
                           dup_heads, dup_count, workspace, workspace_bytes, stream);
}
```

### deep_recommenders_amd/engine.py

```python
import math
import os
from typing import List, Optional, Sequence

import torch

from . import ops


_SIDE_STREAMS = {}


def _side_streams(device):
    key = str(torch.device(device))
    if key not in _SIDE_STREAMS:
        _SIDE_STREAMS[key] = (torch.cuda.Stream(device=device), torch.cuda.Stream(device=device))
    return _SIDE_STREAMS[key]


def _pad4(n):
    return (n + 3) // 4 * 4


class DeepFMEngine:
    def __init__(self, num_fields: int, vocab_per_field: int, dim: int, dnn_units: Sequence[int], batch: int,
# ... 55 lines not shown
            self.g_lin_bias = self.flat_grads[self._bias_off:self._bias_off + 1]
            self.m_table = torch.zeros_like(self.table)
            self.v_table = torch.zeros_like(self.table)
            self.mv_lin = torch.zeros((self.R, 2), dtype=torch.float32, device=device)
            self.m_lin, self.v_lin = self.mv_lin[:, 0], self.mv_lin[:, 1]
            self.row_step = torch.zeros(self.R, dtype=torch.int32, device=device) if self.adam_tf else None
        self.acts = [1] * len(dnn_units) + [0]
        self.wplanes = [ops.WeightPlanes(W) if (u > 1 and ops.planes_worthwhile(B, W.shape[0], W.shape[1])) else None
                        for W, u in zip(self.Ws, units)]
        self.dw_ws = [ops.linear_bwd_dw_workspace(B, W.shape[0], W.shape[1], device) for W in self.Ws]
        self.wg_ws = [ops.bf3_wgrad_workspace(B, W.shape[0], W.shape[1], device) if wp is not None else None
                      for W, wp in zip(self.Ws, self.wplanes)]
        nl = len(self.Ws)
        self.fuse_head = nl >= 2 and self.Ws[-1].shape[1] == 1 and self.Ws[-2].shape[1] <= 32 and self.acts[-2] == 1
        self.head_ws = ops.tower_head_workspace(B, device) if self.fuse_head else None
        self._head_done = False
        self._tail_done = False
        self.narrow_ws = [ops.linear_bwd_narrow_workspace(B, W.shape[0], W.shape[1], device)
                          if (i > 0 and self.acts[i - 1] and ops.linear_bwd_narrow_supported(B, W.shape[0], W.shape[1])) else None
                          for i, W in enumerate(self.Ws)]
        self.fuse_tail = (os.environ.get("DR_FUSE_TAIL", "1") == "1" and self.fuse_head and nl >= 3
                          and self.narrow_ws[nl - 2] is not None and self.acts[nl - 3] == 1
                          and ops.tower_tail_supported(B, self.Ws[-2].shape[0], self.Ws[-2].shape[1]))
        self.tail_ws = ops.tower_tail_workspace(B, self.Ws[-2].shape[0], device) if self.fuse_tail else None
        self.row_base = torch.arange(F, device=device, dtype=torch.int64) * V
        self.col_start = torch.arange(F + 1, device=device, dtype=torch.int32)
        self.col_buckets = torch.full((F,), V if hashed else 0, dtype=torch.int64, device=device)
        f32 = dict(dtype=torch.float32, device=device)
        self._ids = [torch.empty((B, F), dtype=torch.int64, device=device) for _ in range(2)]
        self.cur = 0
        self._pref = None
        self._pref_dense = None
        self._next_keys = None
        self._next_dense = None
        self.concat = torch.zeros((B, self.ld), **f32)
        self.sum_x = torch.empty((B, D), **f32)
        self.fm_logit = torch.empty((B,), **f32)
        self.hs = [torch.empty((B, _pad4(u)), **f32)[:, :u] for u in units]
        self.dhs = [torch.empty((B, _pad4(u)), **f32)[:, :u] for u in units[:-1]]
        self.d_concat = torch.empty((B, self.ld), **f32)
        self.prob = torch.empty((B,), **f32)
        self.d_logit = torch.empty((B,), **f32)
        self.loss = torch.zeros(1, **f32)
        self.ws = torch.empty(1024, **f32)
        self._events = None
        self._ev_every, self._ev_step, self._ev_live = 1, 0, False
        self._ev_pool = []
        self._ev_only = None
        self.sorted_bwd = sorted_bwd
        self.fuse_k3 = os.environ.get("DR_FUSE_K3", "1") == "1" and D == 64 and self.Nd <= 32 and V <= (1 << 24)
        self._dense_pads = ([torch.zeros((B, 32), dtype=torch.float32, device=device) for _ in range(2)]
                            if (self.fuse_k3 and self.Nd) else None)
        self._dense_amaxs = None
        self.no_concat = (os.environ.get("DR_NO_CONCAT", "1") == "1" and self.fuse_k3 and self.wplanes[0] is not None
                          and self.wg_ws[0] is not None and sorted_bwd and self.acts[0] in (0, 1) and len(dnn_units) >= 1
                          and not (self.fuse_head and len(self.Ws) == 2) and V < (1 << 24) - 1)
        if self.no_concat:
            self._ids_t = [torch.empty((F, B), dtype=torch.int32, device=device) for _ in range(2)]
            self.x_sorted = torch.empty((B * F, D), dtype=torch.float32, device=device)
        self.lin_old_t = (torch.empty((F, B), dtype=torch.float32, device=device)
                          if (self.fuse_k3 and sorted_bwd) else None)
        self._lin_old_valid = False
        self.h2 = (ops.get_gemm_split() == "f16x2" and self.no_concat and self.wplanes[0] is not None
                   and not self.adam_tf and os.environ.get("DR_OVERLAP_DW", "0") != "1")
        if self.h2:
            self.wplanes[0] = ops.H2WeightPlanes(self.Ws[0], double_buffer=True)
            self.tab_amax = ops.h2_amax(self.table)
            self._tab_ver = (self.table.data_ptr(), self.table._version)
            self._dense_amaxs = [ops.h2_record(device) for _ in range(2)] if self._dense_pads is not None else None
            self.dh0_amax = ops.h2_record(device)
            self._amax_scratch = ops.h2_record(device)
        self._tighten_every = int(os.environ.get("DR_AMAX_TIGHTEN_STEPS", "2048"))
        self._steps_since_tighten = 0
        _pe = os.environ.get("DR_PREFETCH_EARLY", "2")
        self.prefetch_early = _pe in ("1", "2")
        self.prefetch_after_fwd = _pe == "2" and self.fuse_k3
        self._plan_prefetched = False
        if sorted_bwd:
            self._plans = [ops.SortPlan(B * F, device) for _ in range(2)]
            self.side, self.side_r = _side_streams(device)
            self._refresh_stream = self.side
            self.ev_ids = torch.cuda.Event()
            self._ev_sorted = [torch.cuda.Event(), torch.cuda.Event()]
            self._ev_hashed = [torch.cuda.Event(), torch.cuda.Event()]
            self.ev_k4 = torch.cuda.Event()
            self.ev_dw_done = torch.cuda.Event()
            self.ev_planes = torch.cuda.Event()
            self.ev_dlogit = torch.cuda.Event()
            self.ev_lin = torch.cuda.Event()
            self.ev_fwd0 = torch.cuda.Event()
            self.ev_part1 = torch.cuda.Event()
            self.ev_small = torch.cuda.Event()
            self._ev_dense = [torch.cuda.Event(), torch.cuda.Event()]
            self._dense_by_event = False
        self.lin_side = (sorted_bwd and optimizer == "sgd" and os.environ.get("DR_LIN_SIDE", "0") == "1")
        self._k4_det = not os.environ.get("DR_K4_DETERMINISTIC", "1").startswith("0")
        self.fuse_k4 = (os.environ.get("DR_FUSE_K4", "1") != "0" and self.h2 and optimizer == "sgd" and sorted_bwd and self.no_concat
                        and D == 64 and not self.lin_side and self.lin_old_t is not None
                        and self.Ws[0].shape[0] >= F * D)
        _rs = os.environ.get("DR_REDUCE_SIDE", "0")
        self.reduce_side = sorted_bwd and optimizer == "sgd" and _rs in ("1", "2")
        self.reduce_side_wgrad = self.reduce_side and _rs == "1" and not self.h2
        self._small_pending = False
        self._planes_pending = False
        self._planes_pending_l0 = False
        self._k4_fused_done = False
# ... 52 lines not shown
        nxt = self.cur ^ 1
        early_done = self._early_issued
        self._early_issued = False
        st = self._refresh_stream if (early_done and ordered) else self.side
        nk.record_stream(st)
        with torch.cuda.stream(st):
            if not ordered:
                st.wait_event(self.ev_k4)
            if not early_done:
                self._k("next_batch: hash_bucket_i64(side stream, overlapped)", "overlap", self.B * self.F * 16,
                        lambda: ops.hash_bucket_i64(nk, self.col_buckets, out=self._ids[nxt]))
                if self.no_concat:
                    ops.ids_transpose_i32(self._ids[nxt], out=self._ids_t[nxt])
            nd = self._next_dense
            self._pref_dense = None
            if early_done and getattr(self, "_dense_early", False):
                self._pref_dense = self._token(nd)
            elif nd is not None and self.Nd and not self.overlap_dw:
                nd.record_stream(st)
                if not self.no_concat:
                    self.concat[:, self.F * self.D:self.F * self.D + self.Nd].copy_(nd)
                if self._dense_pads is not None:
                    self._dense_pads[nxt][:, :self.Nd].copy_(nd)
                    if self.h2:
                        ops.h2_amax(self._dense_pads[nxt], self._dense_amaxs[nxt])
                self._pref_dense = self._token(nd)
            if early_done and getattr(self, "_dense_early", False):
                self._dense_by_event = True
            elif early_done:
                self._ev_dense[nxt].record(st)
                self._dense_by_event = True
            else:
                self._dense_by_event = False
                self._ev_hashed[nxt].record(st)
                self._k("next_batch: emb_sort_slots(side stream, overlapped)", "overlap", self.B * self.F * 36,
                        lambda: ops.emb_sort_slots(self._ids[nxt], self.row_base, self.R, self._plans[nxt]))
                self._ev_sorted[nxt].record(st)
        self._pref = self._token(nk)

    def _prefetch_early(self):
        nk = self._next_keys
        self._early_issued = False
        if nk is None or not (self.prefetch_early and self.sorted_bwd):
            return
        nxt = self.cur ^ 1
        self.ev_fwd0.record()
        nk.record_stream(self.side)
        nd = self._next_dense
        self._dense_early = (nd is not None and self.Nd and self.no_concat and self._dense_pads is not None and not self.overlap_dw)
        if self._dense_early:
            nd.record_stream(self.side_r)
            with torch.cuda.stream(self.side_r):
                self.side_r.wait_event(self.ev_fwd0)
                self._dense_pads[nxt][:, :self.Nd].copy_(nd)
                if self.h2:
                    ops.h2_amax(self._dense_pads[nxt], self._dense_amaxs[nxt])
                self._ev_dense[nxt].record(self.side_r)
        with torch.cuda.stream(self.side):
            self.side.wait_event(self.ev_fwd0)
            self._k("next_batch: hash_sort_slots(side stream, overlapped)", "overlap", self.B * self.F * 52,
                    lambda: ops.hash_sort_slots(nk, self.col_buckets, self.row_base, self.R, self._ids[nxt],
                                                self._ids_t[nxt] if self.no_concat else None, self._plans[nxt]))
            self._ev_hashed[nxt].record(self.side)
            self._ev_sorted[nxt].record(self.side)
        self._early_issued = True

    def enable_kernel_events(self, on: bool, every: int = 1, only=None):
        self._ev_only = set(only) if only is not None else None
        for rec in (getattr(self, "_events", None) or {}).values():
            self._ev_pool.extend(rec[2])
        self._events = {} if on else None
        self._ev_every = max(1, int(every))
        self._ev_step = 0
        self._ev_live = bool(on)

    def reserve_kernel_events(self, n_pairs: int):
        while len(self._ev_pool) < n_pairs:
            self._ev_pool.append((torch.cuda.Event(enable_timing=True), torch.cuda.Event(enable_timing=True)))

    def _k(self, name, bound, work, fn):
        if self._events is None or not self._ev_live or (self._ev_only is not None and name not in self._ev_only):
            return fn()
        s, e = self._ev_pool.pop() if self._ev_pool else (torch.cuda.Event(enable_timing=True), torch.cuda.Event(enable_timing=True))
        s.record()
        r = fn()
        e.record()
        self._events.setdefault(name, [bound, work, []])[2].append((s, e))
        return r

    def kernel_event_summary(self):
        torch.cuda.synchronize()
        out = {}
        for name, (bound, work, evs) in (self._events or {}).items():
            ms = sum(s.elapsed_time(e) for s, e in evs) / len(evs)
            out[name] = {"bound": bound, "ms": ms, "n": len(evs),
                         "alg_bytes" if bound in ("hbm", "overlap") else "alg_flops": work}
            if name in getattr(self, "concurrent", {}):
                out[name]["concurrent_with"] = self.concurrent[name]
        return out

    def concurrent_pair_summary(self):
        torch.cuda.synchronize()
        done, out = set(), []
        for a, b in getattr(self, "concurrent", {}).items():
            if a in done or b in done or a not in (self._events or {}) or b not in (self._events or {}):
                continue
            done.update((a, b))
            ea, eb = self._events[a][2], self._events[b][2]
            n = min(len(ea), len(eb))
            tot = 0.0
            for (sa, fa), (sb, fb) in zip(ea[-n:], eb[-n:]):
                first = sa if sa.elapsed_time(sb) >= 0 else sb
                tot += max(first.elapsed_time(fa), first.elapsed_time(fb))
            out.append({"kernels": [a, b], "joint_us": tot / n * 1e3})
        return out

    def _wgrad_reduce_deferred(self, i):
        return self.reduce_side_wgrad and i == 0 and self.no_concat and self.wplanes[0] is not None and not self.overlap_dw

    def _side_part2(self, fn):
        self.ev_part1.record()
        with torch.cuda.stream(self.side):
            self.side.wait_event(self.ev_part1)
            fn()
            self.ev_small.record(self.side)
        self._small_pending = True

    def _wgrad(self, i, x, dy, sc, dstW, dstb):
        if i == 0 and self.h2:
            ops.h2_wgrad_emb(self._ids_t[self.cur], self.row_base, self.table, self.tab_amax, self.dense_pad, self.dense_amax, dy,
                             self.dh0_amax, sc, dstW, dstb, workspace=self.wg_ws[0], parts=1 if self._wgrad_reduce_deferred(i) else 3)
        elif i == 0 and self.no_concat:
            ops.bf3_wgrad_emb(self._ids_t[self.cur], self.row_base, self.table, self.dense_pad, dy, sc, dstW, dstb,
                              workspace=self.wg_ws[0], parts=1 if self._wgrad_reduce_deferred(i) else 3)
        elif self.wg_ws[i] is not None:
            ops.bf3_wgrad(x, dy, sc, dstW, dstb, workspace=self.wg_ws[i])
        else:
            ops.linear_bwd_dw(x, dy, sc, dstW, dstb, workspace=self.dw_ws[i])

    def forward(self, keys: torch.Tensor, dense: Optional[torch.Tensor], labels: Optional[torch.Tensor],
                loss_mode: int = ops.LOSS_SIGMOID_CE):
        F, D = self.F, self.D
        B = self.B
        if self.optimizer == "adam":
            self.flat_grads.zero_()
        if self._planes_pending:
            torch.cuda.current_stream().wait_event(self.ev_planes)
            self._planes_pending = False
        for wp in self.wplanes:
            if wp is not None:
                wp.ensure_fresh()
        if self.h2 and (self.table.data_ptr(), self.table._version) != self._tab_ver:
            ops.h2_amax(self.table, self.tab_amax)
            self._tab_ver = (self.table.data_ptr(), self.table._version)
        pref_tok = self._pref
        prefetched = pref_tok is not None and pref_tok == self._token(keys)
        self._pref = None
        self._plan_prefetched = prefetched
        if prefetched:
            self.cur ^= 1
            torch.cuda.current_stream().wait_event(self._ev_hashed[self.cur])
            if getattr(self, "_dense_by_event", False):
                torch.cuda.current_stream().wait_event(self._ev_dense[self.cur])
        else:
            if pref_tok is not None:
                torch.cuda.current_stream().wait_event(self._ev_hashed[self.cur ^ 1])
            self._k("hash_bucket_i64", "hbm", B * F * 16,
                    lambda: ops.hash_bucket_i64(keys, self.col_buckets, out=self.ids))
            if self.no_concat:
                ops.ids_transpose_i32(self.ids, out=self._ids_t[self.cur])
        if self._in_train_step and not self.prefetch_after_fwd:
            self._prefetch_early()
        if self.sorted_bwd and not prefetched:
            self._launch_sort()
        if self.adam_tf:
            if not self._in_train_step:
                raise RuntimeError("optimizer='adam_tf': forward() is only valid inside train_step() (it stamps the looked-up rows "
                                   "with the step that backward_and_update is about to apply)")
            self._k("adam_catchup_rows", "hbm", 0,
                    lambda: ops.adam_catchup_rows(self.ids, self.row_base, self.table, self.m_table, self.v_table, self.lin_w, self.m_lin,
                                                  self.v_lin, self.row_step, self.t, self.t + 1, self.lr, self.beta1, self.beta2, self.eps))
        fused_l0 = self.fuse_k3 and self.wplanes[0] is not None
        if not fused_l0:
            self._k("emb_pool_fwd", "hbm", self.alg_bytes_fwd(),
# ... 111 lines not shown
                dx = self.d_concat[:, :self.in_dim]
                rs = None
            if i > 0 and self.narrow_ws[i] is not None:
                def narrow(parts, x=x, dy=dy, W=W, dx=dx, i=i, dstW=dstW, dstb=dstb):
                    return ops.linear_bwd_narrow(x, dy, W, sc, dstW, dstb, dx, relu_mask=True, workspace=self.narrow_ws[i], parts=parts,
                                                 dx_amax=self.dh0_amax if (i == 1 and self.h2 and (parts & 1)) else None)
                if self.reduce_side and self._in_train_step:
                    self._k("linear_bwd_narrow_L%d" % i, "hbm", 4.0 * self.B * (2 * W.shape[0] + W.shape[1]), lambda: narrow(1))
                    self._side_part2(lambda: narrow(2))
                else:
                    self._k("linear_bwd_narrow_L%d" % i, "hbm", 4.0 * self.B * (2 * W.shape[0] + W.shape[1]), lambda: narrow(3))
                dy = dx
                continue
            if i == 0 and self.fuse_k4 and self._lin_old_valid and not adam and not self.overlap_dw:
                if self.h2 and not (n > 1 and self.narrow_ws[1] is not None):
                    ops.h2_amax(dy, self.dh0_amax)
                self._backward_l0_fused_k4(x, dy, sc, dstW, dstb, fl)
                dy = None
                continue
            if i == 0 and self.h2:
                if not (n > 1 and self.narrow_ws[1] is not None):
                    ops.h2_amax(dy, self.dh0_amax)
                self._k("linear_bwd_dx_L%d" % i, "mfma", fl,
                        lambda dy=dy, rs=rs, dx=dx, i=i: ops.h2_linear_nt(dy, self.dh0_amax, self.wplanes[i].w, mask=rs, out=dx))
            elif self.wplanes[i] is not None:
                self._k("linear_bwd_dx_L%d" % i, "mfma", fl,
                        lambda dy=dy, rs=rs, dx=dx, i=i: ops.bf3_linear_nt(dy, self.wplanes[i].w, mask=rs, out=dx))
            else:
                self._k("linear_bwd_dx_L%d" % i, "mfma", fl,
                        lambda dy=dy, W=W, rs=rs, dx=dx: ops.linear_bwd_dx(dy, W, relu_src=rs, out=dx))
            if i == 0 and self.sorted_bwd and self._plan_prefetched:
                torch.cuda.current_stream().wait_event(self.ev_sorted)
            if i == 0 and self.overlap_dw:
                self.ev_dx.record()
                with torch.cuda.stream(self.side2):
                    self.side2.wait_event(self.ev_dx)
                    self._k("linear_bwd_dw_L%d" % i, "mfma", fl,
                            lambda x=x, dy=dy, i=i, dstW=dstW, dstb=dstb: self._wgrad(i, x, dy, sc, dstW, dstb))
                    if self.wplanes[i] is not None and not adam:
                        self.wplanes[i].refresh()
                    self.ev_dw.record(self.side2)
                dy = dx
                continue
            self._k("linear_bwd_dw_L%d" % i, "mfma", fl,
                    lambda x=x, dy=dy, i=i, dstW=dstW, dstb=dstb: self._wgrad(i, x, dy, sc, dstW, dstb))
            if self.wplanes[i] is not None and not adam:
                if self.sorted_bwd:
                    self.ev_dw_done.record()
                    self._refresh_stream = self.side
                    with torch.cuda.stream(self.side):
                        self.side.wait_event(self.ev_dw_done)
                        if self._wgrad_reduce_deferred(i) and self.h2:
                            ops.h2_wgrad_emb(self._ids_t[self.cur], self.row_base, self.table, self.tab_amax, self.dense_pad, self.dense_amax,
                                             dy, self.dh0_amax, sc, dstW, dstb, workspace=self.wg_ws[0], parts=2)
                        elif self._wgrad_reduce_deferred(i):
                            ops.bf3_wgrad_emb(self._ids_t[self.cur], self.row_base, self.table, self.dense_pad, dy, sc, dstW, dstb,
                                              workspace=self.wg_ws[0], parts=2)
                        self.wplanes[i].refresh()
                        self.ev_planes.record(self.side)
                    self._planes_pending = True
                    self._planes_pending_l0 = (i == 0)
                else:
                    self.wplanes[i].refresh()
            dy = dx
        if adam:
            self._adam_finish()
        elif self._k4_fused_done:
            self._k4_fused_done = False
        elif self.sorted_bwd:
            if not self._plan_prefetched:
                torch.cuda.current_stream().wait_event(self.ev_sorted)
            if self.no_concat and not self._k4_det:
                ops.emb_snapshot_sorted_rows(self.plan, self.table, self.R, self.x_sorted)
            mark = self._prefetch_mark()
            k4 = lambda parts: ops.emb_pool_bwd_sorted(self.ids, self.row_base, self.plan, D, self.R, self.d_concat, self.d_logit,
                                                       -lr, self.table, self.lin_w, self.lin_bias,
                                                       concat=None if self.no_concat else self.concat, sum_x=self.sum_x,
                                                       x_sorted=self.x_sorted if self.no_concat else None, parts=parts,
                                                       lin_old_t=self.lin_old_t if (self._lin_old_valid and not lin_side) else None,
                                                       table_amax=self.tab_amax if self.h2 else None)
            sk = 4 if lin_side else 0
            self._k("emb_pool_bwd", "hbm", self.alg_bytes_bwd() - (self.B * self.F * 8 if lin_side else 0),
                    lambda: k4(1 | sk))
            if self.no_concat:
                self._k("emb_hot_rows_apply", "hbm", 0, lambda: k4(2 | sk))
            if lin_side:
                torch.cuda.current_stream().wait_event(self.ev_lin)
            self._prefetch_issue(mark)
        else:
            self._k("emb_pool_bwd", "hbm", self.alg_bytes_bwd(),
                    lambda: ops.emb_pool_bwd(self.ids, F, self.col_start, self.row_base, D, self.d_concat, self.concat,
                                             self.sum_x, self.d_logit, -lr, self.table, self.lin_w, self.lin_bias))
        if self._small_pending:
            torch.cuda.current_stream().wait_event(self.ev_small)
            self._small_pending = False
        if self.overlap_dw and not adam:
            torch.cuda.current_stream().wait_event(self.ev_dw)

    def _backward_l0_fused_k4(self, x, dy, sc, dstW, dstb, fl):
        lr = self.lr
        torch.cuda.current_stream().wait_event(self.ev_sorted)
        self._k("linear_bwd_dw_L0", "mfma", fl, lambda: self._wgrad(0, x, dy, sc, dstW, dstb))
        w_old = self.wplanes[0].w
        early = self._early_issued
        rs = self.side_r if early else self.side
        self._refresh_stream = rs
        self.ev_dw_done.record()
        with torch.cuda.stream(rs):
            rs.wait_event(self.ev_dw_done)
            self.wplanes[0].refresh()
            self.ev_planes.record(rs)
        self._planes_pending = True
        self._planes_pending_l0 = True
        mark = self._prefetch_mark()
        if early:
            self._prefetch_issue(mark)
        if not self._k4_det:
            ops.emb_snapshot_sorted_rows(self.plan, self.table, self.R, self.x_sorted)
        work = self.alg_bytes_bwd() - 4.0 * self.B * self.F * self.D + 4.0 * self.B * dy.shape[1]
        self._k("emb_pool_bwd_fused_dgrad_L0", "hbm", work,
                lambda: ops.h2_dgrad_emb_sgd(dy, self.dh0_amax, w_old, self._ids_t[self.cur], self.plan, self.row_base, self.table,
                                             self.lin_w, self.lin_old_t, self.sum_x, self.d_logit, -lr, self.d_concat, table_amax=self.tab_amax))
        k4 = lambda parts: ops.emb_pool_bwd_sorted(self.ids, self.row_base, self.plan, self.D, self.R, self.d_concat, self.d_logit, -lr,
                                                   self.table, self.lin_w, self.lin_bias, sum_x=self.sum_x, x_sorted=self.x_sorted,
                                                   parts=parts | 8, lin_old_t=self.lin_old_t, table_amax=self.tab_amax)
        self._k("emb_pool_bwd_dups", "hbm", 0, lambda: k4(1))
        self._k("emb_hot_rows_apply", "hbm", 0, lambda: k4(2))
        if not early:
            self._prefetch_issue(mark)
        self._k4_fused_done = True

    def _launch_sort(self):
        self.ev_ids.record()
        with torch.cuda.stream(self.side):
            self.side.wait_event(self.ev_ids)
            self._k("emb_sort_slots(side stream, overlapped)", "overlap", self.B * self.F * 36,
                    lambda: ops.emb_sort_slots(self.ids, self.row_base, self.R, self.plan))
            self.ev_sorted.record(self.side)

    def _adam_finish(self):
        self.t += 1
        lr_t = ops.adam_lr_t(self.lr, self.beta1, self.beta2, self.t)
        if not self._plan_prefetched:
            torch.cuda.current_stream().wait_event(self.ev_sorted)
        if self.no_concat:
            ops.emb_snapshot_sorted_rows(self.plan, self.table, self.R, self.x_sorted)
        mark = self._prefetch_mark()
        self._k("emb_pool_bwd_adam", "hbm", self.B * (28 * self.F * self.D + 40 * self.F),
                lambda: ops.emb_pool_bwd_sorted_adam(self.ids, self.row_base, self.plan, self.D, self.R, self.d_concat,
                                                     self.d_logit, lr_t, self.beta1, self.beta2, self.eps, self.table,
                                                     self.m_table, self.v_table, self.lin_w, self.m_lin, self.v_lin,
                                                     concat=None if self.no_concat else self.concat, sum_x=self.sum_x,
                                                     x_sorted=self.x_sorted if self.no_concat else None,
                                                     lin_old_t=self.lin_old_t if self._lin_old_valid else None,
                                                     table_amax=self.tab_amax if self.h2 else None))
        self._prefetch_issue(mark)
        ops.reduce_sum(self.d_logit, out=self.g_lin_bias)
        if self.overlap_dw:
            torch.cuda.current_stream().wait_event(self.ev_dw)
        self._k("adam_step_dense", "hbm", 28.0 * self.flat_params.numel(),
                lambda: ops.adam_step(self.flat_params, self.flat_grads, self.flat_m, self.flat_v, lr_t, self.beta1, self.beta2,
                                      self.eps))
        for wp in self.wplanes:
# ... 56 lines not shown
```

### deep_recommenders_amd/ops.py

```python
from typing import Optional, Sequence

import torch

from . import _lib
from ._lib import check, lib, ptr, stream_ptr


def _c(t: torch.Tensor, dtype) -> torch.Tensor:
    if t.dtype != dtype:
        raise TypeError("expected %s, got %s" % (dtype, t.dtype))
    return t if t.is_contiguous() else t.contiguous()


def hash_bucket_i64(keys: torch.Tensor, col_buckets: torch.Tensor, out: Optional[torch.Tensor] = None):
    keys = _c(keys, torch.int64)
    B, C = keys.shape
    col_buckets = _c(col_buckets, torch.int64)
    assert col_buckets.numel() == C
    if out is None:
        out = torch.empty_like(keys)
    check(lib().dr_hash_bucket_i64(ptr(keys), B, C, ptr(col_buckets), ptr(out), stream_ptr()), "dr_hash_bucket_i64")
    return out


def _csr_bytes(values: Sequence, device):
    import numpy as np
    flat = [v if isinstance(v, (bytes, bytearray)) else str(v).encode("utf-8") for v in values]
    offs = np.zeros(len(flat) + 1, dtype=np.int64)
    if flat:
        offs[1:] = np.cumsum([len(b) for b in flat])
    blob = np.frombuffer(b"".join(flat) + b"\0", dtype=np.uint8).copy()
    return torch.from_numpy(blob).to(device), torch.from_numpy(offs).to(device), len(flat)


def hash_bucket_strings(values: Sequence, num_buckets: int, device="cuda"):
    blob, offs, n = _csr_bytes(values, device)
    out = torch.empty(n, dtype=torch.int64, device=device)
    check(lib().dr_hash_bucket_bytes(ptr(blob), ptr(offs), n, int(num_buckets), ptr(out), stream_ptr()),
          "dr_hash_bucket_bytes")
    return out


def vocab_lookup_i64(keys: torch.Tensor, vocab: torch.Tensor):
    keys = _c(keys, torch.int64)
    vocab = _c(vocab, torch.int64)
    out = torch.empty_like(keys)
    check(lib().dr_vocab_lookup_i64(ptr(keys), keys.numel(), ptr(vocab), vocab.numel(), ptr(out), stream_ptr()),
          "dr_vocab_lookup_i64")
    return out


def vocab_lookup_strings(values: Sequence, vocab: Sequence, device="cuda"):
# ... 364 lines not shown
    if pos is None:
        pos = torch.empty((B, C), dtype=torch.int64, device=dev)
    if workspace is None:
        nbytes = lib().dr_shard_bucket_workspace_bytes(n, world)
        workspace = torch.empty(nbytes // 8, dtype=torch.int64, device=dev)
    if rep is not None:
        check(lib().dr_shard_bucket_ids_dedup(ptr(ids), ptr(rep), n, C, int(rows_per_shard), int(world), ptr(counts), ptr(send_rows),
                                              ptr(pos), ptr(workspace), stream_ptr()), "dr_shard_bucket_ids_dedup")
        return counts, send_rows, pos
    check(lib().dr_shard_bucket_ids(ptr(ids), n, C, int(rows_per_shard), int(world), ptr(counts), ptr(send_rows),
                                    ptr(pos), ptr(workspace), stream_ptr()), "dr_shard_bucket_ids")
    return counts, send_rows, pos


def rows_gather(rows, table, lin_w=None, out_rows=None, out_lin=None):
    rows = _c(rows, torch.int64)
    n = rows.numel()
    D = table.shape[1]
    if out_rows is None:
        out_rows = torch.empty((n, D), dtype=torch.float32, device=rows.device)
    if out_lin is None and lin_w is not None:
        out_lin = torch.empty(n, dtype=torch.float32, device=rows.device)
    check(lib().dr_rows_gather(ptr(rows), n, ptr(table), D, ptr(lin_w), ptr(out_rows), ptr(out_lin), stream_ptr()),
          "dr_rows_gather")
    return out_rows, out_lin


def rows_scatter_add(rows, grads, lin_grads, scale, table, lin_w):
    rows = _c(rows, torch.int64)
    n = rows.numel()
    D = table.shape[1]
    check(lib().dr_rows_scatter_add(ptr(rows), n, ptr(grads), D, ptr(lin_grads), float(scale), ptr(table), ptr(lin_w),
                                    stream_ptr()), "dr_rows_scatter_add")


def axpy(alpha, x, y):
    assert x.is_contiguous() and y.is_contiguous() and x.numel() == y.numel()
    check(lib().dr_axpy(x.numel(), float(alpha), ptr(x), ptr(y), stream_ptr()), "dr_axpy")


def emb_sort_workspace(n, device):
    return torch.empty(lib().dr_emb_sort_workspace_bytes(int(n)), dtype=torch.uint8, device=device)


class SortPlan:

    def __init__(self, n, device):
        self.n = int(n)
        self.rows = torch.empty(n, dtype=torch.int64, device=device)
        self.slots = torch.empty(n, dtype=torch.int32, device=device)
        self.flags = torch.empty(n, dtype=torch.uint8, device=device)
        self.dup_heads = torch.empty(n, dtype=torch.int32, device=device)
        self.dup_count = torch.zeros(4, dtype=torch.int32, device=device)
        self.workspace = emb_sort_workspace(n, device)

    def sorted_len(self):
        return int(self.dup_count[1].item())


def emb_sort_slots(ids, row_base, num_rows, plan=None):
    ids = _c(ids, torch.int64)
    B, F = ids.shape
    if plan is None or plan.n < B * F:
        plan = SortPlan(B * F, ids.device)
    check(lib().dr_emb_sort_slots(ptr(ids), B, F, ptr(row_base), int(num_rows), ptr(plan.rows), ptr(plan.slots),
                                  ptr(plan.flags), ptr(plan.dup_heads), ptr(plan.dup_count), ptr(plan.workspace),
                                  plan.workspace.numel(), stream_ptr()), "dr_emb_sort_slots")
    return plan


def hash_sort_slots(keys, col_buckets, row_base, num_rows, ids_out, ids_t_out=None, plan=None):
    keys = _c(keys, torch.int64)
    B, F = keys.shape
    assert ids_out.shape == (B, F) and ids_out.dtype == torch.int64 and ids_out.is_contiguous()
    if ids_t_out is not None:
        assert ids_t_out.shape == (F, B) and ids_t_out.dtype == torch.int32 and ids_t_out.is_contiguous()
    if plan is None or plan.n < B * F:
        plan = SortPlan(B * F, keys.device)
    check(lib().dr_hash_sort_slots(ptr(keys), B, F, ptr(col_buckets), ptr(ids_out), ptr(ids_t_out), ptr(row_base), int(num_rows),
                                   ptr(plan.rows), ptr(plan.slots), ptr(plan.flags), ptr(plan.dup_heads), ptr(plan.dup_count),
                                   ptr(plan.workspace), plan.workspace.numel(), stream_ptr()), "dr_hash_sort_slots")
    return plan


def emb_plan_set_small_limit(limit):
    return int(lib().dr_emb_plan_set_small_limit(int(limit)))


def emb_snapshot_sorted_rows(plan, table, num_rows, out):
    assert out.is_contiguous() and out.shape[0] >= plan.n and out.shape[1] == table.shape[1]
    check(lib().dr_emb_snapshot_sorted_rows(ptr(plan.rows), ptr(plan.dup_heads), ptr(plan.dup_count), ptr(table), table.shape[1],
                                            int(num_rows), ptr(out), stream_ptr()), "dr_emb_snapshot_sorted_rows")
    return out


def ids_transpose_i32(ids, out=None):
    ids = _c(ids, torch.int64)
    B, F = ids.shape
    if out is None:
        out = torch.empty((F, B), dtype=torch.int32, device=ids.device)
    check(lib().dr_ids_transpose_i32(ptr(ids), B, F, ptr(out), stream_ptr()), "dr_ids_transpose_i32")
    return out


def emb_pool_bwd_sorted(ids, row_base, plan, D, num_rows, grad, d_fm_logit, scale, dst_table, dst_lin=None, dst_bias=None,
                        concat=None, sum_x=None, slot_lin_grad=None, x_sorted=None, parts=3, lin_old_t=None, table_amax=None):
    ids = _c(ids, torch.int64)
    B, F = ids.shape
    assert grad.stride(1) == 1
    args = (ptr(ids), ptr(row_base), ptr(plan.rows), ptr(plan.slots), ptr(plan.flags),
            ptr(plan.dup_heads), ptr(plan.dup_count), B, F, D, int(num_rows), ptr(grad),
            grad.stride(0), ptr(concat), concat.stride(0) if concat is not None else 0,
            ptr(sum_x), ptr(d_fm_logit), ptr(slot_lin_grad), float(scale), ptr(dst_table), ptr(dst_lin),
            ptr(dst_bias), ptr(x_sorted))
    if lin_old_t is not None or table_amax is not None:
        assert lin_old_t is None or (lin_old_t.shape == (F, B) and lin_old_t.is_contiguous() and lin_old_t.dtype == torch.float32)
        check(lib().dr_emb_pool_bwd_sorted_ex(*args, ptr(lin_old_t), int(parts), ptr(table_amax), stream_ptr()), "dr_emb_pool_bwd_sorted_ex")
    elif parts == 3:
        check(lib().dr_emb_pool_bwd_sorted(*args, stream_ptr()), "dr_emb_pool_bwd_sorted")
    else:
        check(lib().dr_emb_pool_bwd_sorted_parts(*args, int(parts), stream_ptr()), "dr_emb_pool_bwd_sorted_parts")


def h2_dgrad_emb_sgd(dy, dy_amax, w: "H2Planes", ids_t, plan, row_base, table, lin_w, lin_old_t, sum_x, d_fm_logit, scale, d_concat,
                     table_amax=None):
    F, M = ids_t.shape
    K = dy.shape[1]
    assert dy.stride(1) == 1 and d_concat.stride(1) == 1 and table.is_contiguous() and table.shape[1] == 64 and sum_x.is_contiguous()
    assert ids_t.dtype == torch.int32 and ids_t.is_contiguous() and dy.shape[0] == M and w.rows >= 64 * F
    assert (lin_w is None) == (lin_old_t is None)
    assert lin_old_t is None or (lin_old_t.shape == (F, M) and lin_old_t.is_contiguous())
    check(lib().dr_h2_dgrad_emb_sgd(ptr(dy), dy.stride(0), ptr(dy_amax), ptr(w.buf), w.plane_stride, w.ld, ptr(w.amax), M, F, K,
                                    ptr(ids_t), ptr(plan.flags), ptr(row_base), ptr(table), ptr(lin_w), ptr(lin_old_t), ptr(sum_x),
                                    ptr(d_fm_logit), float(scale), ptr(d_concat), d_concat.stride(0), ptr(table_amax), stream_ptr()),
# ... 534 lines not shown
                                           int(parts), stream_ptr()), "dr_bf3_wgrad_emb_parts")
        return dstW
    check(lib().dr_bf3_wgrad_emb(ptr(ids_t), R, nf, ptr(row_base), ptr(table), table.shape[1], ptr(dense_pad), ptr(dy), dy.stride(0),
                                 F, N, float(scale), ptr(dstW), dstW.stride(0), ptr(dstb), ptr(workspace), workspace.numel() * 4,
                                 stream_ptr()), "dr_bf3_wgrad_emb")
    return dstW


def bf3_wgrad(x, dy, scale, dstW, dstb=None, workspace=None):
    R, F = x.shape
    N = dy.shape[1]
    assert x.stride(1) == 1 and dy.stride(1) == 1 and dstW.shape == (F, N) and dstW.stride(1) == 1 and dy.shape[0] == R
    if workspace is None:
        workspace = bf3_wgrad_workspace(R, F, N, x.device)
    check(lib().dr_bf3_wgrad(ptr(x), x.stride(0), ptr(dy), dy.stride(0), R, F, N, float(scale), ptr(dstW), dstW.stride(0),
                             ptr(dstb), ptr(workspace), workspace.numel() * 4, stream_ptr()), "dr_bf3_wgrad")
    return dstW


class WeightPlanes:

    def __init__(self, W):
        K, N = W.shape
        self.W = W
        self.wt = Planes(N, K, W.device)
        self.w = Planes(K, N, W.device)
        self.refresh()

    def refresh(self):
        bf3_split(self.W, self.wt, transpose=True)
        bf3_split(self.W, self.w)
        self._ver = self.W._version

    def ensure_fresh(self):
        if self.W._version != self._ver:
            self.refresh()


def h2_record(device):
    return torch.zeros(1, dtype=torch.int32, device=device)


def h2_amax(src, amax=None, reset=True):
    if src.dim() == 1:
        src = src.view(1, -1)
    assert src.dim() == 2 and src.stride(1) == 1 and src.dtype == torch.float32
    if amax is None:
        amax = h2_record(src.device)
    R, C = src.shape
    check(lib().dr_h2_amax(ptr(src), src.stride(0) if R > 1 else max(C, 1), R, C, ptr(amax), 1 if reset else 0, stream_ptr()), "dr_h2_amax")
    return amax


def h2_amax_value(amax):
    return float(amax.view(torch.float32).item())


class H2Planes:

    def __init__(self, rows, cols, device, amax=None):
        self.rows, self.cols = int(rows), int(cols)
        self.rows_alloc = (self.rows + 31) // 32 * 32
        self.ld = (self.cols + 31) // 32 * 32
        self.buf = torch.zeros((2, self.rows_alloc, self.ld), dtype=torch.float16, device=device)
        self.amax = amax if amax is not None else h2_record(device)

    @property
    def plane_stride(self):
        return self.rows_alloc * self.ld


def h2_split(src, planes: H2Planes, row_offset=0, col_offset=0, transpose=False):
    assert src.dim() == 2 and src.stride(1) == 1 and src.dtype == torch.float32
    R, C = src.shape
    check(lib().dr_h2_split(ptr(src), src.stride(0), R, C, ptr(planes.buf), planes.plane_stride, planes.ld, row_offset, col_offset,
                            1 if transpose else 0, ptr(planes.amax), stream_ptr()), "dr_h2_split")
    return planes


def h2_linear_nt(a, a_amax, b: H2Planes, bias=None, act=0, mask=None, accumulate=False, out=None, out_amax=None):
    a = _rowmajor_ld4(a)
    M, K = a.shape
    if a.stride(0) % 4 or a.data_ptr() % 16:
        buf = torch.zeros((M, _pad4(K)), dtype=torch.float32, device=a.device)
        buf[:, :K].copy_(a)
        a = buf[:, :K]
    N = b.rows
    assert b.cols == K, "weights' planes must have the reduction length as columns"
    if out is None:
        assert not accumulate
        out = torch.empty((M, _pad4(N)), dtype=torch.float32, device=a.device)[:, :N]
    assert out.shape == (M, N) and out.stride(1) == 1
    check(lib().dr_h2_linear_nt(ptr(a), a.stride(0), ptr(a_amax), ptr(b.buf), b.plane_stride, b.ld, ptr(b.amax), M, N, K, ptr(bias), int(act),
                                ptr(mask), mask.stride(0) if mask is not None else 0, int(bool(accumulate)), ptr(out), out.stride(0),
                                ptr(out_amax), stream_ptr()), "dr_h2_linear_nt")
    return out


def h2_cross_fwd(x0, x, x_amax, wt: H2Planes, b=None, diag_scale=0.0, want_prod=False, prod=None, out_amax=None):
    M, Dm = x.shape
    assert x0.shape == x.shape and x0.stride(0) == x.stride(0) and wt.rows == Dm and wt.cols == Dm
    ld = x.stride(0)
    out = torch.empty((M, ld), dtype=torch.float32, device=x.device)[:, :Dm]
    if want_prod and prod is None:
        prod = torch.empty((M, ld), dtype=torch.float32, device=x.device)[:, :Dm]
    if prod is not None:
        assert prod.stride(0) == ld
    check(lib().dr_h2_cross_fwd(ptr(x0), ptr(x), ld, ptr(x_amax), ptr(wt.buf), wt.plane_stride, wt.ld, ptr(wt.amax), ptr(b), float(diag_scale),
                                M, Dm, ptr(out), ptr(prod), ptr(out_amax), stream_ptr()), "dr_h2_cross_fwd")
    return out, prod


def h2_emb_linear_fwd(ids, row_base, field_rows_max, table, table_amax, lin_w, lin_bias, dense_pad, dense_amax, concat, K, wt: H2Planes, bias, act,
                      sum_x, fm_logit, out, lin_vals_t=None):
    ids = _c(ids, torch.int64)
    M, F = ids.shape
    assert (concat is None or concat.stride(1) == 1) and out.stride(1) == 1 and wt.cols == K and out.shape == (M, wt.rows)
    assert dense_pad is None or (dense_pad.shape == (M, 32) and dense_pad.is_contiguous())
    assert lin_vals_t is None or (lin_vals_t.shape == (F, M) and lin_vals_t.is_contiguous() and lin_vals_t.dtype == torch.float32)
    check(lib().dr_h2_emb_linear_fwd(ptr(ids), M, F, ptr(row_base), int(field_rows_max), ptr(table), table.shape[1], ptr(table_amax), ptr(lin_w),
                                     ptr(lin_bias), ptr(dense_pad), ptr(dense_amax), ptr(concat), concat.stride(0) if concat is not None else 0,
                                     int(K), ptr(wt.buf), wt.plane_stride, wt.ld, ptr(wt.amax), wt.rows, ptr(bias), int(act), ptr(sum_x),
                                     ptr(fm_logit), ptr(out), out.stride(0), ptr(lin_vals_t), stream_ptr()), "dr_h2_emb_linear_fwd")
    return out


def h2_wgrad(x, x_amax, dy, dy_amax, scale, dstW, dstb=None, workspace=None):
    R, F = x.shape
    N = dy.shape[1]
    assert x.stride(1) == 1 and dy.stride(1) == 1 and dstW.shape == (F, N) and dstW.stride(1) == 1 and dy.shape[0] == R
    if workspace is None:
        workspace = bf3_wgrad_workspace(R, F, N, x.device)
    check(lib().dr_h2_wgrad(ptr(x), x.stride(0), ptr(x_amax), ptr(dy), dy.stride(0), ptr(dy_amax), R, F, N, float(scale), ptr(dstW),
                            dstW.stride(0), ptr(dstb), ptr(workspace), workspace.numel() * 4, stream_ptr()), "dr_h2_wgrad")
    return dstW


def h2_wgrad_emb(ids_t, row_base, table, table_amax, dense_pad, dense_amax, dy, dy_amax, scale, dstW, dstb=None, workspace=None, parts=3):
    nf, R = ids_t.shape
    F, N = dstW.shape
    assert ids_t.dtype == torch.int32 and ids_t.is_contiguous() and dy.stride(1) == 1 and dstW.stride(1) == 1 and dy.shape == (R, N)
    assert dense_pad is None or (dense_pad.shape == (R, 32) and dense_pad.is_contiguous())
    if workspace is None:
        workspace = bf3_wgrad_workspace(R, F, N, dy.device)
    check(lib().dr_h2_wgrad_emb(ptr(ids_t), R, nf, ptr(row_base), ptr(table), table.shape[1], ptr(table_amax), ptr(dense_pad), ptr(dense_amax),
                                ptr(dy), dy.stride(0), ptr(dy_amax), F, N, float(scale), ptr(dstW), dstW.stride(0), ptr(dstb), ptr(workspace),
                                workspace.numel() * 4, int(parts), stream_ptr()), "dr_h2_wgrad_emb")
    return dstW


class H2WeightPlanes:

    def __init__(self, W, double_buffer=False):
        K, N = W.shape
        self.W = W
        self.amax = h2_record(W.device)
        self.wt = H2Planes(N, K, W.device, self.amax)
        self.w = H2Planes(K, N, W.device, self.amax)
        self._w_alt = H2Planes(K, N, W.device, h2_record(W.device)) if double_buffer else None
        self._parts = None
        self.refresh()

    def refresh(self):
        if self._parts is None:
            self._parts = torch.zeros(256, dtype=torch.int32, device=self.W.device)
        K, N = self.W.shape
        if self._w_alt is not None:
            self.w, self._w_alt = self._w_alt, self.w
            self.amax = self.w.amax
            self.wt.amax = self.amax
        check(lib().dr_h2_refresh_weight(ptr(self.W), self.W.stride(0), K, N, ptr(self.w.buf), self.w.plane_stride, self.w.ld,
                                         ptr(self.wt.buf), self.wt.plane_stride, self.wt.ld, ptr(self.amax), ptr(self._parts),
                                         stream_ptr()), "dr_h2_refresh_weight")
        self._ver = self.W._version

    def ensure_fresh(self):
        if self.W._version != self._ver:
            self.refresh()


def planes_worthwhile(M, K, N):
    return get_gemm_mode() == "bf16x3" and M >= 2048 and N >= 128 and K >= 64


def bf3_gemm_tn_workspace(R, F, N, device):
    return torch.empty(max(64, lib().dr_bf3_gemm_tn_workspace_bytes(int(R), int(F), int(N)) // 4), dtype=torch.float32,
                       device=device)


def bf3_gemm_tn(x: Planes, y: Planes, scale, dstW, y_colsum=None, dstb=None, workspace=None):
    R, F, N = x.rows, x.cols, y.cols
    assert y.rows == R and dstW.shape == (F, N) and dstW.stride(1) == 1
    if workspace is None:
        workspace = bf3_gemm_tn_workspace(R, F, N, x.buf.device)
    check(lib().dr_bf3_gemm_tn(ptr(x.buf), x.plane_stride, x.ld, ptr(y.buf), y.plane_stride, y.ld, R, F, N, float(scale),
                               ptr(dstW), dstW.stride(0), ptr(y_colsum), ptr(dstb), ptr(workspace), workspace.numel() * 4,
                               stream_ptr()), "dr_bf3_gemm_tn")
    return dstW


ACT_CODES = {None: 0, "linear": 0, "relu": 1, "sigmoid": 2, "tanh": 3}


def cin_fwd(x0, x, W, bias=None, act=2):
    x0, x, W = _c(x0, torch.float32), _c(x, torch.float32), _c(W, torch.float32)
    B, H0, D = x0.shape
    Hk = x.shape[1]
    Fm = W.shape[1]
    assert x.shape == (B, Hk, D) and W.shape[0] == H0 * Hk
    out = torch.empty((B, Fm, D), dtype=torch.float32, device=x0.device)
    check(lib().dr_cin_fwd(ptr(x0), ptr(x), B, H0, Hk, D, ptr(W), Fm, ptr(bias), int(act), ptr(out), stream_ptr()), "dr_cin_fwd")
    return out


def cin_bwd(x0, x, W, act, out, d_out, want_bias=False):
    x0, x, W, d_out = _c(x0, torch.float32), _c(x, torch.float32), _c(W, torch.float32), _c(d_out, torch.float32)
    B, H0, D = x0.shape
    Hk, Fm = x.shape[1], W.shape[1]
    d_x0, d_x, dW = torch.empty_like(x0), torch.empty_like(x), torch.empty_like(W)
    dbias = torch.empty(Fm, dtype=torch.float32, device=x0.device) if want_bias else None
    check(lib().dr_cin_bwd(ptr(x0), ptr(x), B, H0, Hk, D, ptr(W), Fm, int(act), ptr(out), ptr(d_out), ptr(d_x0), ptr(d_x), ptr(dW),
                           ptr(dbias), stream_ptr()), "dr_cin_bwd")
    return d_x0, d_x, dW, dbias
# ... 592 lines not shown
```

### include/dr_hotpath.h

```cpp
#ifndef DR_HOTPATH_H
#define DR_HOTPATH_H

#include <stdint.h>

#ifdef __cplusplus
extern "C" {
#endif

#define DR_OK 0
#define DR_EINVAL (-1)
#define DR_ELAUNCH (-2)
#define DR_ESHAPE (-3)

typedef void* dr_stream_t;

const char* dr_version(void);

#define DR_GEMM_BF16X3 0
#define DR_GEMM_NATIVE_F32 1
int32_t dr_set_gemm_mode(int32_t mode);
int32_t dr_get_gemm_mode(void);

#define DR_GEMM_SPLIT_BF16X3 0
#define DR_GEMM_SPLIT_F16X2 1
int32_t dr_set_gemm_split(int32_t split);
int32_t dr_get_gemm_split(void);

int dr_hash_bucket_i64(const int64_t* keys, int64_t B, int32_t C, const uint64_t* col_buckets,
                       int64_t* ids_out, dr_stream_t stream);

int dr_ids_transpose_i32(const int64_t* ids, int64_t B, int32_t F, int32_t* out, dr_stream_t stream);
int dr_hash_bucket_bytes(const uint8_t* bytes, const int64_t* offsets, int64_t n,
                         uint64_t num_buckets, int64_t* ids_out, dr_stream_t stream);

int dr_vocab_lookup_i64(const int64_t* keys, int64_t n, const int64_t* vocab, int32_t vocab_len,
                        int64_t* ids_out, dr_stream_t stream);
int dr_vocab_lookup_bytes(const uint8_t* bytes, const int64_t* offsets, int64_t n,
                          const uint8_t* vocab_bytes, const int64_t* vocab_offsets,
                          int32_t vocab_len, int64_t* ids_out, dr_stream_t stream);

int dr_emb_pool_fwd(const int64_t* ids, int64_t B, int32_t F, int32_t C, const int32_t* col_start,
                    const int64_t* row_base, const float* table, int32_t D,
                    const float* lin_w, const float* lin_bias,
                    float* concat, int64_t ld_concat, float* sum_x, float* fm_logit,
                    dr_stream_t stream);

#define DR_POOL_FIRST_ORDER_ONLY 1
int dr_emb_pool_fwd_ex(const int64_t* ids, int64_t B, int32_t F, int32_t C, const int32_t* col_start,
                       const int64_t* row_base, const float* table, int32_t D, const float* lin_w,
                       const float* lin_bias, float* concat, int64_t ld_concat, float* sum_x,
                       float* fm_logit, int32_t flags, dr_stream_t stream);
int dr_lin_fields_fwd(const int64_t* ids, int64_t B, int32_t F, int32_t C, const int32_t* col_start,
                      const int64_t* row_base, const float* lin_w, float* out, int64_t ld_out,
                      dr_stream_t stream);
int dr_lin_fields_bwd(const int64_t* ids, int64_t B, int32_t F, int32_t C, const int32_t* col_start,
                      const int64_t* row_base, const float* d_out, int64_t ld_dout, float scale,
                      float* dst_lin, dr_stream_t stream);


int dr_emb_pool_bwd(const int64_t* ids, int64_t B, int32_t F, int32_t C, const int32_t* col_start,
                    const int64_t* row_base, int32_t D,
                    const float* d_concat, int64_t ld_dconcat,
                    const float* concat, int64_t ld_concat, const float* sum_x,
                    const float* d_fm_logit, float scale,
                    float* dst_table, float* dst_lin, float* dst_bias, dr_stream_t stream);

int64_t dr_emb_sort_workspace_bytes(int64_t n);
int32_t dr_emb_plan_set_small_limit(int32_t limit);
int dr_emb_sort_slots(const int64_t* ids, int64_t B, int32_t F, const int64_t* row_base, int64_t num_rows,
                      int64_t* sorted_rows, int32_t* sorted_slots, uint8_t* unique_flags,
                      int32_t* dup_heads, int32_t* dup_count, void* workspace, int64_t workspace_bytes,
                      dr_stream_t stream);
int dr_hash_sort_slots(const int64_t* keys, int64_t B, int32_t F, const uint64_t* col_buckets, int64_t* ids_out,
                       int32_t* ids_t_out, const int64_t* row_base, int64_t num_rows, int64_t* sorted_rows,
                       int32_t* sorted_slots, uint8_t* unique_flags, int32_t* dup_heads, int32_t* dup_count, void* workspace,
                       int64_t workspace_bytes, dr_stream_t stream);
int dr_emb_pool_bwd_sorted(const int64_t* ids, const int64_t* row_base, const int64_t* sorted_rows,
                           const int32_t* sorted_slots, const uint8_t* unique_flags,
                           const int32_t* dup_heads, const int32_t* dup_count, int64_t B, int32_t F,
                           int32_t D, int64_t num_rows, const float* grad, int64_t ld_grad,
                           const float* concat, int64_t ld_concat, const float* sum_x,
                           const float* d_fm_logit, const float* slot_lin_grad, float scale,
                           float* dst_table, float* dst_lin, float* dst_bias, float* x_sorted, dr_stream_t stream);
int dr_emb_pool_bwd_sorted_parts(const int64_t* ids, const int64_t* row_base, const int64_t* sorted_rows,
                                 const int32_t* sorted_slots, const uint8_t* unique_flags,
                                 const int32_t* dup_heads, const int32_t* dup_count, int64_t B, int32_t F,
                                 int32_t D, int64_t num_rows, const float* grad, int64_t ld_grad,
                                 const float* concat, int64_t ld_concat, const float* sum_x,
                                 const float* d_fm_logit, const float* slot_lin_grad, float scale,
                                 float* dst_table, float* dst_lin, float* dst_bias, float* x_sorted, int32_t parts,
                                 dr_stream_t stream);
int dr_emb_lin_update_unique(const int64_t* ids, const uint8_t* unique_flags, int64_t B, int32_t F, const int64_t* row_base,
                             const float* d_fm_logit, const float* slot_lin_grad, float scale, float* dst_lin, dr_stream_t stream);
int dr_emb_pool_bwd_sorted_ex(const int64_t* ids, const int64_t* row_base, const int64_t* sorted_rows,
                              const int32_t* sorted_slots, const uint8_t* unique_flags,
                              const int32_t* dup_heads, const int32_t* dup_count, int64_t B, int32_t F,
                              int32_t D, int64_t num_rows, const float* grad, int64_t ld_grad,
                              const float* concat, int64_t ld_concat, const float* sum_x,
                              const float* d_fm_logit, const float* slot_lin_grad, float scale,
                              float* dst_table, float* dst_lin, float* dst_bias, float* x_sorted,
                              const float* lin_old_t, int32_t parts, uint32_t* table_amax, dr_stream_t stream);
int dr_emb_snapshot_sorted_rows(const int64_t* sorted_rows, const int32_t* dup_heads, const int32_t* dup_count,
                                const float* table, int32_t D, int64_t num_rows, float* x_sorted, dr_stream_t stream);

int dr_emb_pool_bwd_sorted_adam(const int64_t* ids, const int64_t* row_base, const int64_t* sorted_rows,
                                const int32_t* sorted_slots, const uint8_t* unique_flags,
                                const int32_t* dup_heads, const int32_t* dup_count, int64_t B, int32_t F,
                                int32_t D, int64_t num_rows, const float* grad, int64_t ld_grad,
                                const float* concat, int64_t ld_concat, const float* sum_x,
                                const float* d_fm_logit, const float* slot_lin_grad, float lr_t, float beta1,
                                float beta2, float eps, float* table, float* m_table, float* v_table,
                                float* lin_w, float* m_lin, float* v_lin, float* x_sorted, dr_stream_t stream);
int dr_emb_pool_bwd_sorted_adam_ex(const int64_t* ids, const int64_t* row_base, const int64_t* sorted_rows,
                                const int32_t* sorted_slots, const uint8_t* unique_flags,
                                const int32_t* dup_heads, const int32_t* dup_count, int64_t B, int32_t F,
                                int32_t D, int64_t num_rows, const float* grad, int64_t ld_grad,
                                const float* concat, int64_t ld_concat, const float* sum_x,
                                const float* d_fm_logit, const float* slot_lin_grad, float lr_t, float beta1,
                                float beta2, float eps, float* table, float* m_table, float* v_table,
                                float* lin_w, float* m_lin, float* v_lin, float* x_sorted, const float* lin_old_t, uint32_t* table_amax, dr_stream_t stream);
int dr_adam_catchup_rows(const int64_t* ids, int64_t n, int32_t F, const int64_t* row_base, int32_t D, float* table,
                         float* m_table, float* v_table, float* lin_w, float* m_lin, float* v_lin, int32_t* row_step,
                         int32_t upto, int32_t stamp, float lr, float beta1, float beta2, float eps, dr_stream_t stream);
int dr_adam_step(float* param, const float* grad, float* m, float* v, int64_t n, float lr_t, float beta1,
                 float beta2, float eps, float grad_scale, dr_stream_t stream);

int dr_ftrl_step(float* param, const float* grad, float* accum, float* linear, int64_t n, float lr,
                 float lr_power, float l1, float l2, float grad_scale, dr_stream_t stream);

// ... 159 lines not shown

int dr_bf3_split(const float* src, int64_t ld_src, int64_t R, int32_t C, void* planes, int64_t plane_stride,
                 int64_t ld_planes, int64_t row_offset, int64_t col_offset, int32_t transpose,
                 dr_stream_t stream);
int dr_bf3_join(const void* planes, int64_t plane_stride, int64_t ld_planes, int64_t R, int32_t C, float* dst,
                int64_t ld_dst, dr_stream_t stream);
int dr_bf3_gemm_nt(const void* a_planes, int64_t a_plane_stride, int64_t a_ld, const void* b_planes,
                   int64_t b_plane_stride, int64_t b_ld, int64_t M, int32_t N, int32_t K, const float* bias,
                   int32_t act, const float* mask, int64_t ld_mask, float* C, int64_t ldc, dr_stream_t stream);
int dr_bf3_linear_nt(const float* A, int64_t lda, const void* b_planes, int64_t b_plane_stride, int64_t b_ld, int64_t M,
                     int32_t N, int32_t K, const float* bias, int32_t act, const float* mask, int64_t ld_mask,
                     int32_t accumulate, float* C, int64_t ldc, dr_stream_t stream);
int dr_bf3_linear_nt_pack(const float* dy, int64_t ld_dy, const void* w_planes, int64_t plane_stride, int64_t b_ld, int64_t M,
                          int32_t N, int32_t K, const int64_t* pos, int32_t F, const float* d_fm_logit, const float* sum_x,
                          const float* x, int64_t ld_x, float* out_rows, float* out_lin, float* bias_sum, dr_stream_t stream);
int dr_h2_linear_nt_pack(const float* dy, int64_t ld_dy, const uint32_t* dy_amax, const void* w_planes, int64_t plane_stride,
                         int64_t b_ld, const uint32_t* w_amax, int64_t M, int32_t N, int32_t K, const int64_t* pos, int32_t F,
                         const float* d_fm_logit, const float* sum_x, const float* x, int64_t ld_x, float* out_rows,
                         float* out_lin, float* bias_sum, dr_stream_t stream);
int dr_bf3_cross_fwd(const float* x0, const float* x, int64_t ld, const void* wt_planes, int64_t plane_stride,
                     int64_t ld_planes, const float* b, float diag_scale, int64_t M, int32_t Dm, float* out,
                     float* prod_out, dr_stream_t stream);
int dr_bf3_emb_linear_fwd(const int64_t* ids, int64_t M, int32_t F, const int64_t* row_base, int64_t field_rows_max,
                          const float* table, int32_t D, const float* lin_w, const float* lin_bias, const float* dense_pad, float* concat,
                          int64_t ld_concat, int32_t K, const void* wt_planes, int64_t plane_stride, int64_t ld_planes, int32_t N,
                          const float* bias, int32_t act, float* sum_x, float* fm_logit, float* out, int64_t ld_out,
                          dr_stream_t stream);
int dr_bf3_emb_linear_fwd_lv(const int64_t* ids, int64_t M, int32_t F, const int64_t* row_base, int64_t field_rows_max,
                             const float* table, int32_t D, const float* lin_w, const float* lin_bias, const float* dense_pad, float* concat,
                             int64_t ld_concat, int32_t K, const void* wt_planes, int64_t plane_stride, int64_t ld_planes, int32_t N,
                             const float* bias, int32_t act, float* sum_x, float* fm_logit, float* out, int64_t ld_out,
                             float* lin_vals_t, dr_stream_t stream);
int64_t dr_bf3_wgrad_workspace_bytes(int64_t R, int32_t F, int32_t N);
int dr_bf3_wgrad(const float* x, int64_t ld_x, const float* dy, int64_t ld_dy, int64_t R, int32_t F, int32_t N,
                 float scale, float* dstW, int64_t ld_w, float* dstb, void* workspace, int64_t workspace_bytes,
                 dr_stream_t stream);
int dr_bf3_wgrad_emb(const int32_t* ids_t, int64_t R, int32_t nf, const int64_t* row_base, const float* table, int32_t D,
                     const float* dense_pad, const float* dy, int64_t ld_dy, int32_t F, int32_t N, float scale, float* dstW,
                     int64_t ld_w, float* dstb, void* workspace, int64_t workspace_bytes, dr_stream_t stream);
int dr_bf3_wgrad_emb_parts(const int32_t* ids_t, int64_t R, int32_t nf, const int64_t* row_base, const float* table, int32_t D,
                           const float* dense_pad, const float* dy, int64_t ld_dy, int32_t F, int32_t N, float scale, float* dstW,
                           int64_t ld_w, float* dstb, void* workspace, int64_t workspace_bytes, int32_t parts, dr_stream_t stream);
int64_t dr_bf3_gemm_tn_workspace_bytes(int64_t R, int32_t F, int32_t N);
int dr_bf3_gemm_tn(const void* x_planes, int64_t x_plane_stride, int64_t x_ld, const void* y_planes,
                   int64_t y_plane_stride, int64_t y_ld, int64_t R, int32_t F, int32_t N, float scale, float* dst,
                   int64_t ld_dst, const float* y_colsum, float* dstb, void* workspace, int64_t workspace_bytes,
                   dr_stream_t stream);

int dr_h2_amax(const float* src, int64_t ld, int64_t R, int32_t C, uint32_t* amax, int32_t reset, dr_stream_t stream);
int dr_h2_split(const float* src, int64_t ld_src, int64_t R, int32_t C, void* planes, int64_t plane_stride, int64_t ld_planes,
                int64_t row_offset, int64_t col_offset, int32_t transpose, const uint32_t* amax, dr_stream_t stream);
int dr_h2_refresh_weight(const float* W, int64_t ldw, int64_t K, int32_t N, void* w_planes, int64_t w_plane_stride, int64_t w_ld,
                         void* wt_planes, int64_t wt_plane_stride, int64_t wt_ld, uint32_t* amax, uint32_t* parts, dr_stream_t stream);
int dr_h2_linear_nt(const float* A, int64_t lda, const uint32_t* a_amax, const void* b_planes, int64_t b_plane_stride, int64_t b_ld,
                    const uint32_t* b_amax, int64_t M, int32_t N, int32_t K, const float* bias, int32_t act, const float* mask,
                    int64_t ld_mask, int32_t accumulate, float* C, int64_t ldc, uint32_t* c_amax, dr_stream_t stream);
int dr_h2_dgrad_emb_sgd(const float* dy, int64_t ld_dy, const uint32_t* dy_amax, const void* w_planes, int64_t w_plane_stride,
                        int64_t w_ld, const uint32_t* w_amax, int64_t M, int32_t F, int32_t K, const int32_t* ids_t,
                        const uint8_t* unique_flags, const int64_t* row_base, float* table, float* lin_w, const float* lin_old_t,
                        const float* sum_x, const float* d_fm_logit, float scale, float* d_concat, int64_t ld_dconcat,
                        uint32_t* table_amax, dr_stream_t stream);
int dr_h2_cross_fwd(const float* x0, const float* x, int64_t ld, const uint32_t* x_amax, const void* wt_planes, int64_t plane_stride,
                    int64_t ld_planes, const uint32_t* w_amax, const float* b, float diag_scale, int64_t M, int32_t Dm, float* out,
                    float* prod_out, uint32_t* out_amax, dr_stream_t stream);
int dr_cross_combine_bwd_amax(const float* x0, const float* prod, const float* d_out, int64_t M, int32_t Dm, int64_t ld, float diag_scale,
                              float* d_prod, float* d_x0_accum, float* d_x_accum, uint32_t* d_prod_amax, dr_stream_t stream);
int dr_h2_emb_linear_fwd(const int64_t* ids, int64_t M, int32_t F, const int64_t* row_base, int64_t field_rows_max, const float* table,
                         int32_t D, const uint32_t* table_amax, const float* lin_w, const float* lin_bias, const float* dense_pad,
                         const uint32_t* dense_amax, float* concat, int64_t ld_concat, int32_t K, const void* wt_planes,
                         int64_t plane_stride, int64_t ld_planes, const uint32_t* w_amax, int32_t N, const float* bias, int32_t act,
                         float* sum_x, float* fm_logit, float* out, int64_t ld_out, float* lin_vals_t, dr_stream_t stream);
int dr_h2_wgrad(const float* x, int64_t ld_x, const uint32_t* x_amax, const float* dy, int64_t ld_dy, const uint32_t* dy_amax, int64_t R,
                int32_t F, int32_t N, float scale, float* dstW, int64_t ld_w, float* dstb, void* workspace, int64_t workspace_bytes,
                dr_stream_t stream);
int dr_h2_wgrad_emb(const int32_t* ids_t, int64_t R, int32_t nf, const int64_t* row_base, const float* table, int32_t D,
                    const uint32_t* table_amax, const float* dense_pad, const uint32_t* dense_amax, const float* dy, int64_t ld_dy,
                    const uint32_t* dy_amax, int32_t F, int32_t N, float scale, float* dstW, int64_t ld_w, float* dstb, void* workspace,
                    int64_t workspace_bytes, int32_t parts, dr_stream_t stream);


int dr_cin_fwd(const float* x0, const float* x, int64_t B, int32_t H0, int32_t Hk, int32_t D, const float* W,
               int32_t Fm, const float* bias, int32_t act, float* out, dr_stream_t stream);
int dr_cin_bwd(const float* x0, const float* x, int64_t B, int32_t H0, int32_t Hk, int32_t D, const float* W,
               int32_t Fm, int32_t act, const float* out, const float* d_out, float* d_x0, float* d_x, float* dW,
               float* dbias, dr_stream_t stream);

int dr_cin_pool_fwd(const float* x0, const float* x, int64_t B, int32_t H0, int32_t Hk, int32_t D, const float* W, int32_t Fm,
                    const float* bias, int32_t act, float* out, float* pooled, dr_stream_t stream);
int64_t dr_cin_pool_bwd_workspace_bytes(int64_t B, int32_t H0, int32_t Hk, int32_t D, int32_t Fm);
int dr_cin_pool_bwd(const float* x0, const float* x, int64_t B, int32_t H0, int32_t Hk, int32_t D, const float* W, int32_t Fm,
                    int32_t act, const float* out, const float* d_out, const float* d_pooled, float* d_x0, int32_t accumulate_x0,
                    float* d_x, float* dW, float* dbias, void* ws, int64_t ws_bytes, dr_stream_t stream);

int dr_din_concat_fwd(const float* x, const float* y, int64_t B, int32_t D, int32_t mode, float* out, int64_t ld_out,
                      dr_stream_t stream);
int dr_din_concat_bwd(const float* x, const float* y, int64_t B, int32_t D, int32_t mode, const float* d_out,
                      int64_t ld_dout, float* d_x, float* d_y, dr_stream_t stream);

int dr_act_fwd(float* x, int64_t M, int32_t N, int64_t ld, int32_t act, dr_stream_t stream);
int dr_act_bwd(const float* y, int64_t ld_y, float* dy, int64_t ld_dy, int64_t M, int32_t N, int32_t act,
               dr_stream_t stream);
int dr_dropout_fwd(const float* x, int64_t ld_x, int64_t M, int32_t N, float rate, uint64_t seed, float* y,
                   int64_t ld_y, uint8_t* mask, dr_stream_t stream);
int dr_dropout_bwd(const float* dy, int64_t ld_dy, const uint8_t* mask, int64_t M, int32_t N, float rate, float* dx,
                   int64_t ld_dx, dr_stream_t stream);
int dr_reduce_sum(const float* x, int64_t n, int32_t squared, float alpha, int32_t accumulate, float* out,
                  float* workspace, dr_stream_t stream);

int dr_linear_fwd_grouped(const float* x, int64_t ld_x, int64_t x_gs, const float* W, int64_t ld_w, int64_t w_gs, const float* b,
                          int64_t b_gs, int64_t M, int32_t K, int32_t N, int32_t G, int32_t act, float* y, int64_t ld_y, int64_t y_gs,
                          dr_stream_t stream);
int dr_linear_bwd_dx_grouped(const float* dy, int64_t ld_dy, int64_t dy_gs, const float* W, int64_t ld_w, int64_t w_gs, int64_t M,
                             int32_t K, int32_t N, int32_t G, const float* relu_src, int64_t ld_relu_src, int64_t rs_gs,
                             int32_t accumulate, float* dx, int64_t ld_dx, int64_t dx_gs, dr_stream_t stream);
int64_t dr_linear_bwd_dw_grouped_workspace_bytes(int64_t M, int32_t K, int32_t N, int32_t G);
int dr_linear_bwd_dw_grouped(const float* x, int64_t ld_x, int64_t x_gs, const float* dy, int64_t ld_dy, int64_t dy_gs, int64_t M,
                             int32_t K, int32_t N, int32_t G, float scale, float* dstW, int64_t ld_w, int64_t w_gs, float* dstb,
                             int64_t b_gs, float* workspace, int64_t workspace_bytes, dr_stream_t stream);

int dr_mmoe_gate_mix_fwd(const float* h, int64_t ld_h, const float* logits, int64_t ld_l, int64_t B, int32_t E, int32_t T, int32_t U,
                         float* p, int64_t ld_p, float* out, int64_t ld_out, dr_stream_t stream);
int dr_mmoe_gate_mix_bwd(const float* h, int64_t ld_h, const float* p, int64_t ld_p, const float* d_out, int64_t ld_do, int64_t B,
                         int32_t E, int32_t T, int32_t U, float* d_h, int64_t ld_dh, float* d_l, int64_t ld_dl, dr_stream_t stream);

int64_t dr_mse_workspace_bytes(int32_t T);
int dr_mse_fwd_bwd(const float* pred, int64_t ld_pred, const float* labels, int64_t ld_labels, int64_t B, int32_t T, float* loss,
                   float* d_pred, int64_t ld_dpred, float* workspace, int64_t workspace_bytes, dr_stream_t stream);

int dr_esmm_head_fwd(const float* logits, int64_t ld_logits, int64_t B, float* p_cvr, float* p_ctr, float* p_ctcvr, dr_stream_t stream);
int dr_esmm_head_bwd(const float* p_cvr, const float* p_ctr, const float* d_cvr, const float* d_ctr, const float* d_ctcvr, int64_t B,
                     float* d_logits, int64_t ld_dlogits, dr_stream_t stream);
// ... 70 lines not shown
```

Baseline: 68.29 million examples/sec.

## Fuse weight amax into wgrad reduce and merge sort/dense-place amax passes

The wgrad split-K reduce kernel now computes per-block abs-max of the updated weights, and the f16x2 weight-plane refresh consumes those partials instead of running a separate amax pass over the weights. A new kernel copies dense features into the padded buffer and computes their amax in one launch using a last-block-arrives ticket, and merged sort-slot variants use a similar ticket to cut launches. This removes extra kernel launches and full rereads of small tensors each step, at the cost of cross-block ticket synchronisation and a coupling between the wgrad and refresh paths.

```diff
diff --git a/deep_recommenders_amd/_lib.py b/deep_recommenders_amd/_lib.py
--- a/deep_recommenders_amd/_lib.py
+++ b/deep_recommenders_amd/_lib.py
@@ -55,6 +55,8 @@
     "dr_emb_sort_workspace_bytes": [_i64],
     "dr_emb_sort_slots": [_p, _i64, _i32, _p, _i64, _p, _p, _p, _p, _p, _p, _i64, _p],
     "dr_hash_sort_slots": [_p, _i64, _i32, _p, _p, _p, _p, _i64, _p, _p, _p, _p, _p, _p, _i64, _p],
+    "dr_emb_sort_slots_merged": [_p, _i64, _i32, _p, _i64, _p, _p, _p, _p, _p, _p, _i64, _p, _p],
+    "dr_hash_sort_slots_merged": [_p, _i64, _i32, _p, _p, _p, _p, _i64, _p, _p, _p, _p, _p, _p, _i64, _p, _p],
     "dr_emb_plan_set_small_limit": [_i32],
     "dr_adam_catchup_rows": [_p, _i64, _i32, _p, _i32, _p, _p, _p, _p, _p, _p, _p, _i32, _i32, _f32, _f32, _f32, _f32, _p],
     "dr_emb_pool_bwd_sorted": [_p, _p, _p, _p, _p, _p, _p, _i64, _i32, _i32, _i64, _p, _i64, _p, _i64, _p, _p, _p, _f32, _p, _p,
@@ -112,6 +114,11 @@
     "dr_h2_amax": [_p, _i64, _i64, _i32, _p, _i32, _p],
     "dr_h2_split": [_p, _i64, _i64, _i32, _p, _i64, _i64, _i64, _i64, _i32, _p, _p],
     "dr_h2_refresh_weight": [_p, _i64, _i64, _i32, _p, _i64, _i64, _p, _i64, _i64, _p, _p, _p],
+    "dr_h2_refresh_weight_from_parts": [_p, _i64, _i64, _i32, _p, _i64, _i64, _p, _i64, _i64, _p, _p, _i32, _p],
+    "dr_h2_place_dense": [_p, _i64, _i64, _i32, _p, _p, _p, _p],
+    "dr_h2_wgrad_amax_parts_max": [_i32, _i32],
+    "dr_h2_wgrad_ex": [_p, _i64, _p, _p, _i64, _p, _i64, _i32, _i32, _f32, _p, _i64, _p, _p, _i64, _p, _p, _p],
+    "dr_h2_wgrad_emb_ex": [_p, _i64, _i32, _p, _p, _i32, _p, _p, _p, _p, _i64, _p, _i32, _i32, _f32, _p, _i64, _p, _p, _i64, _i32, _p, _p, _p],
     "dr_h2_linear_nt": [_p, _i64, _p, _p, _i64, _i64, _p, _i64, _i32, _i32, _p, _i32, _p, _i64, _i32, _p, _i64, _p, _p],
     "dr_h2_cross_fwd": [_p, _p, _i64, _p, _p, _i64, _i64, _p, _p, _f32, _i64, _i32, _p, _p, _p, _p],
     "dr_h2_dgrad_emb_sgd": [_p, _i64, _p, _p, _i64, _i64, _p, _i64, _i32, _i32, _p, _p, _p, _p, _p, _p, _p, _p, _f32, _p, _i64, _p, _p],
@@ -184,7 +191,7 @@
     "dr_set_gemm_split": [_i32],
     "dr_get_gemm_split": [],
 }
-_RESTYPE = {"dr_version": ctypes.c_char_p, "dr_shard_bucket_workspace_bytes": ctypes.c_int64,
+_RESTYPE = {"dr_version": ctypes.c_char_p, "dr_h2_wgrad_amax_parts_max": ctypes.c_int64, "dr_shard_bucket_workspace_bytes": ctypes.c_int64,
             "dr_emb_sort_workspace_bytes": ctypes.c_int64, "dr_tower_tail_workspace_bytes": ctypes.c_int64, "dr_ivf_build_workspace_bytes": ctypes.c_int64,
             "dr_linear_bwd_dw_workspace_bytes": ctypes.c_int64,
             "dr_linear_fwd_splitk_workspace_bytes": ctypes.c_int64,
diff --git a/deep_recommenders_amd/csrc/bf3_planes.hip b/deep_recommenders_amd/csrc/bf3_planes.hip
--- a/deep_recommenders_amd/csrc/bf3_planes.hip
+++ b/deep_recommenders_amd/csrc/bf3_planes.hip
@@ -556,7 +556,8 @@
                                                             _Float16* __restrict__ w, int64_t w_ps, int64_t w_ld,
                                                             _Float16* __restrict__ wt, int64_t wt_ps, int64_t wt_ld,
                                                             const uint32_t* __restrict__ parts, int32_t nparts, uint32_t* __restrict__ amax) {
-    uint32_t m = (int)threadIdx.x < nparts ? parts[threadIdx.x] : 0u;
+    uint32_t m = 0u;
+    for (int i = threadIdx.x; i < nparts; i += 256) m = max(m, parts[i]);
 #pragma unroll
     for (int o = 32; o > 0; o >>= 1) m = max(m, (uint32_t)__shfl_xor((int)m, o, 64));
     __shared__ uint32_t wm[4];
@@ -581,6 +582,43 @@
     }
 }
 
+constexpr int H2_PLACE_PARTS = 256, H2_PAD = 32;
+__global__ __launch_bounds__(256) void h2_place_dense_kernel(const float* __restrict__ src, int64_t ld_src, int64_t B, int32_t Nd,
+                                                             float* __restrict__ dst, uint32_t* __restrict__ amax,
+                                                             uint32_t* __restrict__ scratch) {
+    uint32_t m = 0u;
+    const int64_t total = B * H2_PAD, stride = (int64_t)gridDim.x * blockDim.x;
+    for (int64_t i = (int64_t)blockIdx.x * blockDim.x + threadIdx.x; i < total; i += stride) {
+        const int64_t r = i >> 5;
+        const int c = (int)(i & (H2_PAD - 1));
+        float v;
+        if (c < Nd) {
+            v = src[r * ld_src + c];
+            dst[i] = v;
+        } else {
+            v = dst[i];
+        }
+        m = max(m, __float_as_uint(fabsf(v)));
+    }
+#pragma unroll
+    for (int o = 32; o > 0; o >>= 1) m = max(m, (uint32_t)__shfl_xor((int)m, o, 64));
+    __shared__ uint32_t wm[4];
+    if ((threadIdx.x & 63) == 0) wm[threadIdx.x >> 6] = m;
+    __syncthreads();
+    if (threadIdx.x == 0) scratch[blockIdx.x] = max(max(wm[0], wm[1]), max(wm[2], wm[3]));
+    if (!dr_last_block_arrives(scratch + H2_PLACE_PARTS, gridDim.x)) return;
+    m = threadIdx.x < gridDim.x ? scratch[threadIdx.x] : 0u;
+#pragma unroll
+    for (int o = 32; o > 0; o >>= 1) m = max(m, (uint32_t)__shfl_xor((int)m, o, 64));
+    __syncthreads();
+    if ((threadIdx.x & 63) == 0) wm[threadIdx.x >> 6] = m;
+    __syncthreads();
+    if (threadIdx.x == 0) {
+        amax[0] = max(max(wm[0], wm[1]), max(wm[2], wm[3]));
+        dr_ticket_reset(scratch + H2_PLACE_PARTS);
+    }
+}
+
 __global__ __launch_bounds__(256) void bf3_join_kernel(const __bf16* __restrict__ planes, int64_t ps, int64_t ldp, int64_t R,
                                                        int32_t C, float* __restrict__ dst, int64_t ld_dst) {
     const int64_t total = R * C, stride = (int64_t)gridDim.x * blockDim.x;
@@ -701,3 +739,24 @@
     DR_CHECK_LAUNCH();
     return DR_OK;
 }
+
+extern "C" int dr_h2_refresh_weight_from_parts(const float* W, int64_t ldw, int64_t K, int32_t N, void* w_planes, int64_t w_ps, int64_t w_ld,
+                                               void* wt_planes, int64_t wt_ps, int64_t wt_ld, uint32_t* amax, const uint32_t* parts,
+                                               int32_t np, dr_stream_t stream) {
+    if (K <= 0 || N <= 0 || ldw < N || !W || !w_planes || !wt_planes || !amax || !parts || np <= 0) return DR_EINVAL;
+    if (w_ld < N || wt_ld < K || w_ps <= 0 || wt_ps <= 0) return DR_EINVAL;
+    const int64_t total = K * (int64_t)N;
+    hipLaunchKernelGGL(h2_split_both_kernel, dim3(dr_grid_for(2 * total, 256, 2048)), dim3(256), 0, dr_s(stream), W, ldw, K, N,
+                       static_cast<_Float16*>(w_planes), w_ps, w_ld, static_cast<_Float16*>(wt_planes), wt_ps, wt_ld, parts, np, amax);
+    DR_CHECK_LAUNCH();
+    return DR_OK;
+}
+
+extern "C" int dr_h2_place_dense(const float* src, int64_t ld_src, int64_t B, int32_t Nd, float* dst_pad, uint32_t* amax,
+                                 uint32_t* scratch, dr_stream_t stream) {
+    if (B <= 0 || Nd <= 0 || Nd > H2_PAD || ld_src < Nd || !src || !dst_pad || !amax || !scratch) return DR_EINVAL;
+    const int grid = dr_grid_for(B * H2_PAD, 256 * 8, H2_PLACE_PARTS);
+    hipLaunchKernelGGL(h2_place_dense_kernel, dim3(grid), dim3(256), 0, dr_s(stream), src, ld_src, B, Nd, dst_pad, amax, scratch);
+    DR_CHECK_LAUNCH();
+    return DR_OK;
+}
diff --git a/deep_recommenders_amd/csrc/bf3_wgrad.hip b/deep_recommenders_amd/csrc/bf3_wgrad.hip
--- a/deep_recommenders_amd/csrc/bf3_wgrad.hip
+++ b/deep_recommenders_amd/csrc/bf3_wgrad.hip
@@ -232,11 +232,13 @@
                                                               float scale, float* __restrict__ dst, int64_t ld,
                                                               float* __restrict__ dstb, const uint32_t* __restrict__ x_amax = nullptr,
                                                               const uint32_t* __restrict__ x2_amax = nullptr,
-                                                              const uint32_t* __restrict__ y_amax = nullptr) {
+                                                              const uint32_t* __restrict__ y_amax = nullptr,
+                                                              uint32_t* __restrict__ w_amax_parts = nullptr) {
     typedef float vec_t __attribute__((ext_vector_type(V)));
     const int f = blockIdx.x;
     const int n = ((int)blockIdx.y * 64 + (int)threadIdx.x) * V;
-    if (n >= N) return;
+    uint32_t wm = 0u;
+    if (n < N) {
     const int64_t ps = (int64_t)Fp * Np;
     float wscale = scale;
     if (x_amax != nullptr) {
@@ -263,12 +265,19 @@
     if (V == 1 || n + V <= N) {
         vec_t o = *reinterpret_cast<vec_t*>(d);
 #pragma unroll
-        for (int c = 0; c < V; ++c) o[c] = fmaf(wscale, acc[c], o[c]);
+        for (int c = 0; c < V; ++c) {
+            o[c] = fmaf(wscale, acc[c], o[c]);
+            wm = max(wm, __float_as_uint(fabsf(o[c])));
+        }
         *reinterpret_cast<vec_t*>(d) = o;
     } else {
 #pragma unroll
         for (int c = 0; c < V; ++c)
-            if (n + c < N) d[c] = fmaf(wscale, acc[c], d[c]);
+            if (n + c < N) {
+                const float o = fmaf(wscale, acc[c], d[c]);
+                d[c] = o;
+                wm = max(wm, __float_as_uint(fabsf(o)));
+            }
     }
     if (f == 0 && colsum != nullptr && dstb != nullptr) {
         const vec_t cacc = sum_slices(colsum + n, Np);
@@ -276,18 +285,26 @@
         for (int c = 0; c < V; ++c)
             if (n + c < N) dstb[n + c] = fmaf(scale, cacc[c], dstb[n + c]);
     }
-}
-
-void launch_tn_rs_reduce(const float* partial, const float* colsum, int split, int32_t F, int32_t N, int Fp, int Np, float scale,
-                         float* dst, int64_t ld, float* dstb, const uint32_t* x_amax, const uint32_t* x2_amax, const uint32_t* y_amax,
-                         dr_stream_t stream) {
+    }
+    if (w_amax_parts != nullptr) {
+#pragma unroll
+        for (int o = 32; o > 0; o >>= 1) wm = max(wm, (uint32_t)__shfl_xor((int)wm, o, 64));
+        if (threadIdx.x == 0) w_amax_parts[(int64_t)f * gridDim.y + blockIdx.y] = wm;
+    }
+}
+
+int launch_tn_rs_reduce(const float* partial, const float* colsum, int split, int32_t F, int32_t N, int Fp, int Np, float scale,
+                        float* dst, int64_t ld, float* dstb, const uint32_t* x_amax, const uint32_t* x2_amax, const uint32_t* y_amax,
+                        dr_stream_t stream, uint32_t* w_amax_parts = nullptr) {
     const bool vec = ((reinterpret_cast<uintptr_t>(partial) | reinterpret_cast<uintptr_t>(dst)) & 15) == 0 && (ld & 3) == 0;
+    const int gy = vec ? (N + 255) / 256 : (N + 63) / 64;
     if (vec)
-        hipLaunchKernelGGL(bf3_tn_rs_reduce_kernel<4>, dim3(F, (N + 255) / 256), dim3(64), 0, dr_s(stream), partial, colsum, split, F, N,
-                           Fp, Np, scale, dst, ld, dstb, x_amax, x2_amax, y_amax);
+        hipLaunchKernelGGL(bf3_tn_rs_reduce_kernel<4>, dim3(F, gy), dim3(64), 0, dr_s(stream), partial, colsum, split, F, N,
+                           Fp, Np, scale, dst, ld, dstb, x_amax, x2_amax, y_amax, w_amax_parts);
     else
-        hipLaunchKernelGGL(bf3_tn_rs_reduce_kernel<1>, dim3(F, (N + 63) / 64), dim3(64), 0, dr_s(stream), partial, colsum, split, F, N,
-                           Fp, Np, scale, dst, ld, dstb, x_amax, x2_amax, y_amax);
+        hipLaunchKernelGGL(bf3_tn_rs_reduce_kernel<1>, dim3(F, gy), dim3(64), 0, dr_s(stream), partial, colsum, split, F, N,
+                           Fp, Np, scale, dst, ld, dstb, x_amax, x2_amax, y_amax, w_amax_parts);
+    return F * gy;
 }
 
 void tn_rs_plan(int64_t R, int32_t F, int32_t N, int& split, int64_t& per, int& Fp, int& Np) {
@@ -313,7 +330,8 @@
 
 static int wgrad_impl(const float* x, int64_t ld_x, const float* dy, int64_t ld_dy, int64_t R, int32_t F, int32_t N,
                       float scale, float* dstW, int64_t ld_w, float* dstb, void* workspace, int64_t workspace_bytes,
-                      dr_stream_t stream, const uint32_t* x_amax = nullptr, const uint32_t* dy_amax = nullptr) {
+                      dr_stream_t stream, const uint32_t* x_amax = nullptr, const uint32_t* dy_amax = nullptr,
+                      uint32_t* w_amax_parts = nullptr, int32_t* w_amax_np = nullptr) {
     if (R <= 0 || F <= 0 || N <= 0) return DR_EINVAL;
     if (!x || !dy || !dstW || !workspace || ld_x < F || ld_dy < N || ld_w < N) return DR_EINVAL;
     if (workspace_bytes < dr_bf3_wgrad_workspace_bytes(R, F, N)) return DR_EINVAL;
@@ -327,8 +345,9 @@
     const int grid = (Fp / 256) * (Np / 256) * split;
     if (x_amax != nullptr) hipLaunchKernelGGL((bf3_gemm_tn_rs_kernel<0, 1>), dim3(grid), dim3(512), 0, dr_s(stream), g);
     else hipLaunchKernelGGL((bf3_gemm_tn_rs_kernel<0, 0>), dim3(grid), dim3(512), 0, dr_s(stream), g);
-    launch_tn_rs_reduce(partial, dstb != nullptr ? colsum : nullptr, split, F, N, Fp, Np, scale, dstW, ld_w, dstb, x_amax, nullptr, dy_amax,
-                        stream);
+    const int np = launch_tn_rs_reduce(partial, dstb != nullptr ? colsum : nullptr, split, F, N, Fp, Np, scale, dstW, ld_w, dstb, x_amax,
+                                       nullptr, dy_amax, stream, w_amax_parts);
+    if (w_amax_np != nullptr) *w_amax_np = np;
     DR_CHECK_LAUNCH();
     return DR_OK;
 }
@@ -349,7 +368,8 @@
 static int wgrad_emb_impl(const int32_t* ids_t, int64_t R, int32_t nf, const int64_t* row_base, const float* table, int32_t D,
                           const float* dense_pad, const float* dy, int64_t ld_dy, int32_t F, int32_t N, float scale, float* dstW,
                           int64_t ld_w, float* dstb, void* workspace, int64_t workspace_bytes, int32_t parts, dr_stream_t stream,
-                          const uint32_t* table_amax = nullptr, const uint32_t* dense_amax = nullptr, const uint32_t* dy_amax = nullptr) {
+                          const uint32_t* table_amax = nullptr, const uint32_t* dense_amax = nullptr, const uint32_t* dy_amax = nullptr,
+                          uint32_t* w_amax_parts = nullptr, int32_t* w_amax_np = nullptr) {
     if (R <= 0 || F <= 0 || N <= 0 || nf <= 0) return DR_EINVAL;
     if (table_amax != nullptr && (!dy_amax || (F > 64 * nf && !dense_amax))) return DR_EINVAL;
     if (D != 64 || F < 64 * nf || F > 64 * nf + 32) return DR_ESHAPE;
@@ -368,9 +388,11 @@
         if (table_amax != nullptr) hipLaunchKernelGGL((bf3_gemm_tn_rs_kernel<1, 1>), dim3(grid), dim3(512), 0, dr_s(stream), g);
         else hipLaunchKernelGGL((bf3_gemm_tn_rs_kernel<1, 0>), dim3(grid), dim3(512), 0, dr_s(stream), g);
     }
-    if (parts & 2)
-        launch_tn_rs_reduce(partial, dstb != nullptr ? colsum : nullptr, split, F, N, Fp, Np, scale, dstW, ld_w, dstb, table_amax,
-                            F > 64 * nf ? dense_amax : nullptr, dy_amax, stream);
+    if (parts & 2) {
+        const int np = launch_tn_rs_reduce(partial, dstb != nullptr ? colsum : nullptr, split, F, N, Fp, Np, scale, dstW, ld_w, dstb,
+                                           table_amax, F > 64 * nf ? dense_amax : nullptr, dy_amax, stream, w_amax_parts);
+        if (w_amax_np != nullptr) *w_amax_np = np;
+    }
     DR_CHECK_LAUNCH();
     return DR_OK;
 }
@@ -399,3 +421,26 @@
     return wgrad_emb_impl(ids_t, R, nf, row_base, table, D, dense_pad, dy, ld_dy, F, N, scale, dstW, ld_w, dstb, workspace, workspace_bytes,
                           parts, stream, table_amax, dense_amax, dy_amax);
 }
+
+extern "C" int64_t dr_h2_wgrad_amax_parts_max(int32_t F, int32_t N) {
+    if (F <= 0 || N <= 0) return 0;
+    return (int64_t)F * ((N + 63) / 64);
+}
+
+extern "C" int dr_h2_wgrad_ex(const float* x, int64_t ld_x, const uint32_t* x_amax, const float* dy, int64_t ld_dy, const uint32_t* dy_amax,
+                              int64_t R, int32_t F, int32_t N, float scale, float* dstW, int64_t ld_w, float* dstb, void* workspace,
+                              int64_t workspace_bytes, uint32_t* w_amax_parts, int32_t* w_amax_np, dr_stream_t stream) {
+    if (!x_amax || !dy_amax || (w_amax_parts != nullptr && !w_amax_np)) return DR_EINVAL;
+    return wgrad_impl(x, ld_x, dy, ld_dy, R, F, N, scale, dstW, ld_w, dstb, workspace, workspace_bytes, stream, x_amax, dy_amax, w_amax_parts,
+                      w_amax_np);
+}
+
+extern "C" int dr_h2_wgrad_emb_ex(const int32_t* ids_t, int64_t R, int32_t nf, const int64_t* row_base, const float* table, int32_t D,
+                                  const uint32_t* table_amax, const float* dense_pad, const uint32_t* dense_amax, const float* dy,
+                                  int64_t ld_dy, const uint32_t* dy_amax, int32_t F, int32_t N, float scale, float* dstW, int64_t ld_w,
+                                  float* dstb, void* workspace, int64_t workspace_bytes, int32_t parts, uint32_t* w_amax_parts,
+                                  int32_t* w_amax_np, dr_stream_t stream) {
+    if (parts < 1 || parts > 3 || !table_amax || !dy_amax || (w_amax_parts != nullptr && !w_amax_np)) return DR_EINVAL;
+    return wgrad_emb_impl(ids_t, R, nf, row_base, table, D, dense_pad, dy, ld_dy, F, N, scale, dstW, ld_w, dstb, workspace, workspace_bytes,
+                          parts, stream, table_amax, dense_amax, dy_amax, w_amax_parts, w_amax_np);
+}
diff --git a/deep_recommenders_amd/csrc/dr_common.h b/deep_recommenders_amd/csrc/dr_common.h
--- a/deep_recommenders_amd/csrc/dr_common.h
+++ b/deep_recommenders_amd/csrc/dr_common.h
@@ -24,6 +24,28 @@
 #pragma unroll
     for (int o = 32; o > 0; o >>= 1) v += __shfl_xor(v, o, 64);
     return v;
+}
+
+__device__ __forceinline__ bool dr_last_block_arrives(uint32_t* __restrict__ ticket, uint32_t nblocks) {
+    __shared__ uint32_t dr_last_;
+    asm volatile("s_waitcnt vmcnt(0)" ::: "memory");
+    __syncthreads();
+    if (threadIdx.x == 0) {
+        __builtin_amdgcn_fence(__ATOMIC_RELEASE, "agent");
+        asm volatile("s_waitcnt vmcnt(0)" ::: "memory");
+        const uint32_t prev = __hip_atomic_fetch_add(ticket, 1u, __ATOMIC_RELAXED, __HIP_MEMORY_SCOPE_AGENT);
+        const bool last = prev == nblocks - 1u;
+        if (last) {
+            __builtin_amdgcn_fence(__ATOMIC_ACQUIRE, "agent");
+            asm volatile("s_waitcnt vmcnt(0)" ::: "memory");
+        }
+        dr_last_ = last ? 1u : 0u;
+    }
+    __syncthreads();
+    return dr_last_ != 0u;
+}
+__device__ __forceinline__ void dr_ticket_reset(uint32_t* __restrict__ ticket) {
+    __hip_atomic_store(ticket, 0u, __ATOMIC_RELAXED, __HIP_MEMORY_SCOPE_AGENT);
 }
 
 __host__ __device__ __forceinline__ uint32_t dr_mix32(uint64_t seed, uint64_t idx) {
diff --git a/deep_recommenders_amd/csrc/emb_plan.hip b/deep_recommenders_amd/csrc/emb_plan.hip
--- a/deep_recommenders_amd/csrc/emb_plan.hip
+++ b/deep_recommenders_amd/csrc/emb_plan.hip
@@ -73,13 +73,60 @@
     }
 }
 
+template <int VEC>
+__device__ __forceinline__ void scan_digits_one_block(uint32_t* __restrict__ ghist, int32_t nb, uint32_t* __restrict__ tot) {
+    constexpr int JMAX = RADIX_MAX_BLOCKS / (64 * VEC), DIG = 2;
+    typedef uint32_t vec_t __attribute__((ext_vector_type(VEC)));
+    const int lane = threadIdx.x & 63, w = threadIdx.x >> 6;
+    for (int d0 = w * DIG; d0 < RADIX; d0 += 4 * DIG) {
+        vec_t v[DIG][JMAX];
+#pragma unroll
+        for (int q = 0; q < DIG; ++q)
+#pragma unroll
+            for (int j = 0; j < JMAX; ++j) {
+                const int32_t i = (j * 64 + lane) * VEC;
+                const vec_t x = *reinterpret_cast<const vec_t*>(ghist + (int64_t)(d0 + q) * nb + (i < nb ? i : 0));
+                v[q][j] = i < nb ? x : (vec_t)0u;
+            }
+#pragma unroll
+        for (int q = 0; q < DIG; ++q) {
+            uint32_t* col = ghist + (int64_t)(d0 + q) * nb;
+            uint32_t run = 0;
+#pragma unroll
+            for (int j = 0; j < JMAX; ++j) {
+                if (j * 64 * VEC < nb) {
+                    uint32_t sum = 0;
+#pragma unroll
+                    for (int c = 0; c < VEC; ++c) sum += v[q][j][c];
+                    uint32_t inc = sum;
+#pragma unroll
+                    for (int o = 1; o < 64; o <<= 1) {
+                        const uint32_t y = (uint32_t)__shfl_up((int)inc, o, 64);
+                        if (lane >= o) inc += y;
+                    }
+                    uint32_t x = run + inc - sum;
+                    vec_t out;
+#pragma unroll
+                    for (int c = 0; c < VEC; ++c) { out[c] = x; x += v[q][j][c]; }
+                    const int32_t i = (j * 64 + lane) * VEC;
+                    if (i < nb) *reinterpret_cast<vec_t*>(col + i) = out;
+                    run += (uint32_t)__shfl((int)inc, 63, 64);
+                }
+            }
+            if (lane == 0) tot[d0 + q] = run;
+        }
+    }
+}
+
 constexpr int FRONT_GROUP = 4;
 template <bool HASH, bool TRANS>
 __global__ __launch_bounds__(256) void plan_front_kernel(const int64_t* __restrict__ src, int64_t B, int32_t F,
                                                          const uint64_t* __restrict__ col_buckets, int64_t* __restrict__ ids_out,
                                                          int32_t* __restrict__ ids_t, const int64_t* __restrict__ row_base,
                                                          uint64_t sentinel, uint32_t mul, int32_t sub, uint64_t* __restrict__ keys,
-                                                         uint32_t* __restrict__ ghist) {
+                                                         uint32_t* __restrict__ ghist, uint32_t* __restrict__ tot,
+                                                         Ctrl* __restrict__ ctrl, int32_t* __restrict__ dup_count,
+                                                         uint32_t* __restrict__ ticket) {
     extern __shared__ uint64_t fsm[];
     __shared__ uint32_t h[RADIX];
     int64_t* rb = reinterpret_cast<int64_t*>(fsm);
@@ -128,6 +175,14 @@
     }
     __syncthreads();
     ghist[t * nb + blockIdx.x] = h[t];
+    if (ticket == nullptr) return;
+    if (!dr_last_block_arrives(ticket, (uint32_t)nb)) return;
+    int32_t* c = reinterpret_cast<int32_t*>(ctrl);
+    for (int i = t; i < (int)(sizeof(Ctrl) / 4); i += 256) c[i] = 0;
+    if (t < 2) dup_count[t] = 0;
+    if ((nb & 3) == 0) scan_digits_one_block<4>(ghist, nb, tot);
+    else scan_digits_one_block<1>(ghist, nb, tot);
+    if (t == 0) dr_ticket_reset(ticket);
 }
 
 __global__ __launch_bounds__(256) void radix_hist_kernel(const uint64_t* __restrict__ keys, int32_t n, uint32_t shift,
@@ -357,19 +412,14 @@
     if (t == 0) ctrl->bcnt[b] = ndup;
 }
 
-__global__ __launch_bounds__(256) void plan_bucket_sort_kernel(const uint64_t* __restrict__ blist, Ctrl* __restrict__ ctrl,
-                                                               int32_t small_limit, uint64_t* __restrict__ rows,
-                                                               int32_t* __restrict__ slots, int32_t* __restrict__ dup_heads,
-                                                               int32_t* __restrict__ dup_count) {
-    __shared__ uint64_t s[CAPB];
-    __shared__ int32_t cnts[NBK];
-    __shared__ int32_t nheads, hbase;
+__device__ __forceinline__ bool plan_verdict_large(const Ctrl* __restrict__ ctrl, int32_t small_limit, int32_t* __restrict__ cnts,
+                                                   int32_t& m, int32_t& off) {
     const int t = threadIdx.x, b = blockIdx.x;
-    if (ctrl->large != 0) return;
+    const int32_t large = ctrl->large;
     if (t < NBK) cnts[t] = ctrl->bcnt[t];
-    if (t == 0) nheads = 0;
-    __syncthreads();
-    int32_t m = 0, off = 0;
+    __syncthreads();
+    m = 0;
+    off = 0;
     bool over = false;
     for (int i = 0; i < NBK; ++i) {
         const int32_t c = cnts[i];
@@ -377,11 +427,16 @@
         if (i < b) off += c;
         m += c;
     }
-    if (over || m > small_limit) {
-        if (b == 0 && t == 0) ctrl->large = 1;
-        return;
-    }
-    const int cnt = cnts[b];
+    return large != 0 || over || m > small_limit;
+}
+
+__device__ __forceinline__ void plan_bucket_body(const uint64_t* __restrict__ blist, int cnt, int32_t off, int32_t m,
+                                                 uint64_t* __restrict__ rows, int32_t* __restrict__ slots,
+                                                 int32_t* __restrict__ dup_heads, int32_t* __restrict__ dup_count) {
+    __shared__ uint64_t s[CAPB];
+    __shared__ int32_t nheads, hbase;
+    const int t = threadIdx.x, b = blockIdx.x;
+    if (t == 0) nheads = 0;
     int n2 = 64;
     while (n2 < cnt) n2 <<= 1;
     if (t < n2) s[t] = t < cnt ? blist[b * CAPB + t] : ~0ull;
@@ -423,6 +478,20 @@
         if (head) dup_heads[hbase + wbase + __popcll(bal & ((1ull << lane) - 1ull))] = gi;
     }
     if (b == 0 && t == 0) dup_count[1] = m;
+}
+
+__global__ __launch_bounds__(256) void plan_bucket_sort_kernel(const uint64_t* __restrict__ blist, Ctrl* __restrict__ ctrl,
+                                                               int32_t small_limit, uint64_t* __restrict__ rows,
+                                                               int32_t* __restrict__ slots, int32_t* __restrict__ dup_heads,
+                                                               int32_t* __restrict__ dup_count) {
+    __shared__ int32_t cnts[NBK];
+    if (ctrl->large != 0) return;
+    int32_t m, off;
+    if (plan_verdict_large(ctrl, small_limit, cnts, m, off)) {
+        if (blockIdx.x == 0 && threadIdx.x == 0) ctrl->large = 1;
+        return;
+    }
+    plan_bucket_body(blist, cnts[blockIdx.x], off, m, rows, slots, dup_heads, dup_count);
 }
 
 __global__ __launch_bounds__(256) void radix_mark_kernel(const uint64_t* __restrict__ rows, const int32_t* __restrict__ slots,
@@ -460,12 +529,10 @@
     for (int j = t; j < nh; j += 256) dup_heads[gbase + j] = hl[j];
 }
 
-__global__ __launch_bounds__(LG_T) void plan_large_kernel(uint64_t* __restrict__ ka, const uint32_t* __restrict__ tot,
-                                                          uint64_t num_rows, int32_t n, uint64_t* __restrict__ rows,
-                                                          int32_t* __restrict__ slots, uint8_t* __restrict__ flags,
-                                                          int32_t* __restrict__ dup_heads, int32_t* __restrict__ dup_count,
-                                                          const Ctrl* __restrict__ ctrl) {
-    if (ctrl->large == 0) return;
+__device__ __forceinline__ void plan_large_body(uint64_t* __restrict__ ka, const uint32_t* __restrict__ tot, uint64_t num_rows,
+                                                int32_t n, uint64_t* __restrict__ rows, int32_t* __restrict__ slots,
+                                                uint8_t* __restrict__ flags, int32_t* __restrict__ dup_heads,
+                                                int32_t* __restrict__ dup_count) {
     __shared__ uint32_t running[RADIX];
     __shared__ uint32_t wcnt[LG_W][RADIX];
     __shared__ uint32_t starts[RADIX];
@@ -557,6 +624,29 @@
     }
 }
 
+__global__ __launch_bounds__(LG_T) void plan_large_kernel(uint64_t* __restrict__ ka, const uint32_t* __restrict__ tot,
+                                                          uint64_t num_rows, int32_t n, uint64_t* __restrict__ rows,
+                                                          int32_t* __restrict__ slots, uint8_t* __restrict__ flags,
+                                                          int32_t* __restrict__ dup_heads, int32_t* __restrict__ dup_count,
+                                                          const Ctrl* __restrict__ ctrl) {
+    if (ctrl->large == 0) return;
+    plan_large_body(ka, tot, num_rows, n, rows, slots, flags, dup_heads, dup_count);
+}
+
+__global__ __launch_bounds__(LG_T) void plan_finish_kernel(const uint64_t* __restrict__ blist, const Ctrl* __restrict__ ctrl,
+                                                           int32_t small_limit, uint64_t* __restrict__ ka,
+                                                           const uint32_t* __restrict__ tot, uint64_t num_rows, int32_t n,
+                                                           uint64_t* __restrict__ rows, int32_t* __restrict__ slots,
+                                                           uint8_t* __restrict__ flags, int32_t* __restrict__ dup_heads,
+                                                           int32_t* __restrict__ dup_count) {
+    __shared__ int32_t cnts[NBK];
+    int32_t m, off;
+    if (plan_verdict_large(ctrl, small_limit, cnts, m, off))
+        plan_large_body(ka, tot, num_rows, n, rows, slots, flags, dup_heads, dup_count);
+    else
+        plan_bucket_body(blist, cnts[blockIdx.x], off, m, rows, slots, dup_heads, dup_count);
+}
+
 }
 
 extern "C" int32_t dr_emb_plan_set_small_limit(int32_t limit) {
@@ -573,7 +663,7 @@
 namespace {
 int plan_small_front(const int64_t* raw, const uint64_t* col_buckets, int64_t* ids_out, int32_t* ids_t, const int64_t* ids, int64_t B,
                      int32_t F, const int64_t* row_base, int64_t num_rows, uint64_t* rows_y, uint64_t* keys_x, uint32_t* ghist,
-                     uint32_t* tot, Ctrl* ctrl, int32_t* dup_count, hipStream_t s) {
+                     uint32_t* tot, Ctrl* ctrl, int32_t* dup_count, uint32_t* ticket, hipStream_t s) {
     const int64_t n64 = B * F;
     const int32_t n = (int32_t)n64;
     const uint32_t mul = (uint32_t)((((uint64_t)RADIX) << 32) / (uint64_t)num_rows);
@@ -588,22 +678,24 @@
     if (raw) {
         if (trans)
             hipLaunchKernelGGL((plan_front_kernel<true, true>), dim3(nbf), dim3(256), lds, s, raw, B, F, col_buckets, ids_out, ids_t, row_base,
-                               (uint64_t)num_rows, mul, (int32_t)sub, rows_y, ghist);
+                               (uint64_t)num_rows, mul, (int32_t)sub, rows_y, ghist, tot, ctrl, dup_count, ticket);
         else
             hipLaunchKernelGGL((plan_front_kernel<true, false>), dim3(nbf), dim3(256), lds, s, raw, B, F, col_buckets, ids_out, ids_t,
-                               row_base, (uint64_t)num_rows, mul, (int32_t)sub, rows_y, ghist);
+                               row_base, (uint64_t)num_rows, mul, (int32_t)sub, rows_y, ghist, tot, ctrl, dup_count, ticket);
     } else {
         hipLaunchKernelGGL((plan_front_kernel<false, false>), dim3(nbf), dim3(256), lds, s, ids, B, F, col_buckets, ids_out, ids_t, row_base,
-                           (uint64_t)num_rows, mul, (int32_t)sub, rows_y, ghist);
-    }
-    hipLaunchKernelGGL((radix_scan_kernel<true>), dim3(RADIX), dim3(256), 0, s, ghist, (int32_t)nbf, tot, ctrl, dup_count);
+                           (uint64_t)num_rows, mul, (int32_t)sub, rows_y, ghist, tot, ctrl, dup_count, ticket);
+    }
+    if (ticket == nullptr)
+        hipLaunchKernelGGL((radix_scan_kernel<true>), dim3(RADIX), dim3(256), 0, s, ghist, (int32_t)nbf, tot, ctrl, dup_count);
     hipLaunchKernelGGL(plan_scatter_kernel, dim3(nbs), dim3(LG_T), 0, s, rows_y, keys_x, n, mul, (int32_t)chunk, ghist, (int32_t)nbf, tot);
     return DR_OK;
 }
 
 int sort_slots_impl(const int64_t* raw, const uint64_t* col_buckets, int32_t* ids_t, const int64_t* ids, int64_t B, int32_t F,
                     const int64_t* row_base, int64_t num_rows, int64_t* sorted_rows, int32_t* sorted_slots, uint8_t* unique_flags,
-                    int32_t* dup_heads, int32_t* dup_count, void* workspace, int64_t workspace_bytes, dr_stream_t stream) {
+                    int32_t* dup_heads, int32_t* dup_count, void* workspace, int64_t workspace_bytes, uint32_t* ticket,
+                    dr_stream_t stream) {
     if (B < 0 || F <= 0 || num_rows <= 0) return DR_EINVAL;
     const int64_t n64 = B * F;
     if (n64 == 0) return DR_OK;
@@ -635,7 +727,7 @@
     }
     if (claimable) {
         int rc = plan_small_front(fused_front ? raw : nullptr, col_buckets, const_cast<int64_t*>(ids), fused_front ? ids_t : nullptr, ids, B,
-                                  F, row_base, num_rows, rows_y, keys_x, ghist, tot, ctrl, dup_count, s);
+                                  F, row_base, num_rows, rows_y, keys_x, ghist, tot, ctrl, dup_count, ticket, s);
         if (rc != DR_OK) return rc;
         static const hipError_t lds_optin = hipFuncSetAttribute(reinterpret_cast<const void*>(plan_lds_claim_kernel),
                                                                 hipFuncAttributeMaxDynamicSharedMemorySize, 4 << LDS_TAB_MAX_LOG);
@@ -644,6 +736,12 @@
         while (log_tab < LDS_TAB_MAX_LOG && (1 << log_tab) < 2 * ((n + NBK - 1) / NBK)) ++log_tab;
         hipLaunchKernelGGL(plan_lds_claim_kernel, dim3(NBK), dim3(CLAIM_T), (size_t)4 << log_tab, s, keys_x, tot, (uint64_t)num_rows,
                            (int32_t)log_tab, unique_flags, blist, ctrl);
+        if (ticket != nullptr) {
+            hipLaunchKernelGGL(plan_finish_kernel, dim3(NBK), dim3(LG_T), 0, s, blist, ctrl, (int32_t)g_small_limit.load(), keys_x, tot,
+                               (uint64_t)num_rows, n, rows_y, sorted_slots, unique_flags, dup_heads, dup_count);
+            DR_CHECK_LAUNCH();
+            return DR_OK;
+        }
         hipLaunchKernelGGL(plan_bucket_sort_kernel, dim3(NBK), dim3(256), 0, s, blist, ctrl, (int32_t)g_small_limit.load(), rows_y,
                            sorted_slots, dup_heads, dup_count);
         hipLaunchKernelGGL(plan_large_kernel, dim3(NBK), dim3(LG_T), 0, s, keys_x, tot, (uint64_t)num_rows, n, rows_y, sorted_slots,
@@ -679,7 +777,16 @@
                                  int64_t* sorted_rows, int32_t* sorted_slots, uint8_t* unique_flags, int32_t* dup_heads,
                                  int32_t* dup_count, void* workspace, int64_t workspace_bytes, dr_stream_t stream) {
     return sort_slots_impl(nullptr, nullptr, nullptr, ids, B, F, row_base, num_rows, sorted_rows, sorted_slots, unique_flags, dup_heads,
-                           dup_count, workspace, workspace_bytes, stream);
+                           dup_count, workspace, workspace_bytes, nullptr, stream);
+}
+
+extern "C" int dr_emb_sort_slots_merged(const int64_t* ids, int64_t B, int32_t F, const int64_t* row_base, int64_t num_rows,
+                                        int64_t* sorted_rows, int32_t* sorted_slots, uint8_t* unique_flags, int32_t* dup_heads,
+                                        int32_t* dup_count, void* workspace, int64_t workspace_bytes, uint32_t* ticket,
+                                        dr_stream_t stream) {
+    if (!ticket) return DR_EINVAL;
+    return sort_slots_impl(nullptr, nullptr, nullptr, ids, B, F, row_base, num_rows, sorted_rows, sorted_slots, unique_flags, dup_heads,
+                           dup_count, workspace, workspace_bytes, ticket, stream);
 }
 
 extern "C" int dr_hash_sort_slots(const int64_t* keys, int64_t B, int32_t F, const uint64_t* col_buckets, int64_t* ids_out,
@@ -688,5 +795,14 @@
                                   int64_t workspace_bytes, dr_stream_t stream) {
     if (!keys || !col_buckets || !ids_out) return DR_EINVAL;
     return sort_slots_impl(keys, col_buckets, ids_t_out, ids_out, B, F, row_base, num_rows, sorted_rows, sorted_slots, unique_flags,
-                           dup_heads, dup_count, workspace, workspace_bytes, stream);
-}
+                           dup_heads, dup_count, workspace, workspace_bytes, nullptr, stream);
+}
+
+extern "C" int dr_hash_sort_slots_merged(const int64_t* keys, int64_t B, int32_t F, const uint64_t* col_buckets, int64_t* ids_out,
+                                         int32_t* ids_t_out, const int64_t* row_base, int64_t num_rows, int64_t* sorted_rows,
+                                         int32_t* sorted_slots, uint8_t* unique_flags, int32_t* dup_heads, int32_t* dup_count,
+                                         void* workspace, int64_t workspace_bytes, uint32_t* ticket, dr_stream_t stream) {
+    if (!keys || !col_buckets || !ids_out || !ticket) return DR_EINVAL;
+    return sort_slots_impl(keys, col_buckets, ids_t_out, ids_out, B, F, row_base, num_rows, sorted_rows, sorted_slots, unique_flags,
+                           dup_heads, dup_count, workspace, workspace_bytes, ticket, stream);
+}
diff --git a/deep_recommenders_amd/engine.py b/deep_recommenders_amd/engine.py
--- a/deep_recommenders_amd/engine.py
+++ b/deep_recommenders_amd/engine.py
@@ -131,6 +131,7 @@
         self._dense_pads = ([torch.zeros((B, 32), dtype=torch.float32, device=device) for _ in range(2)]
                             if (self.fuse_k3 and self.Nd) else None)
         self._dense_amaxs = None
+        self._dense_scratch = None
         self.no_concat = (os.environ.get("DR_NO_CONCAT", "1") == "1" and self.fuse_k3 and self.wplanes[0] is not None
                           and self.wg_ws[0] is not None and sorted_bwd and self.acts[0] in (0, 1) and len(dnn_units) >= 1
                           and not (self.fuse_head and len(self.Ws) == 2) and V < (1 << 24) - 1)
@@ -289,9 +290,14 @@
             nd.record_stream(self.side_r)
             with torch.cuda.stream(self.side_r):
                 self.side_r.wait_event(self.ev_fwd0)
-                self._dense_pads[nxt][:, :self.Nd].copy_(nd)
-                if self.h2:
-                    ops.h2_amax(self._dense_pads[nxt], self._dense_amaxs[nxt])
+                if self.h2 and nd.dtype == torch.float32 and nd.stride(1) == 1:
+                    if self._dense_scratch is None:
+                        self._dense_scratch = ops.h2_place_scratch(nd.device)
+                    ops.h2_place_dense(nd, self._dense_pads[nxt], self._dense_amaxs[nxt], self._dense_scratch)
+                else:
+                    self._dense_pads[nxt][:, :self.Nd].copy_(nd)
+                    if self.h2:
+                        ops.h2_amax(self._dense_pads[nxt], self._dense_amaxs[nxt])
                 self._ev_dense[nxt].record(self.side_r)
         with torch.cuda.stream(self.side):
             self.side.wait_event(self.ev_fwd0)
@@ -363,10 +369,17 @@
             self.ev_small.record(self.side)
         self._small_pending = True
 
+    def _w0_planes_of(self, dstW):
+        wp = self.wplanes[0]
+        if isinstance(wp, ops.H2WeightPlanes) and dstW.data_ptr() == wp.W.data_ptr() and dstW.shape == wp.W.shape:
+            return wp
+        return None
+
     def _wgrad(self, i, x, dy, sc, dstW, dstb):
         if i == 0 and self.h2:
             ops.h2_wgrad_emb(self._ids_t[self.cur], self.row_base, self.table, self.tab_amax, self.dense_pad, self.dense_amax, dy,
-                             self.dh0_amax, sc, dstW, dstb, workspace=self.wg_ws[0], parts=1 if self._wgrad_reduce_deferred(i) else 3)
+                             self.dh0_amax, sc, dstW, dstb, workspace=self.wg_ws[0], parts=1 if self._wgrad_reduce_deferred(i) else 3,
+                             w_planes=self._w0_planes_of(dstW))
         elif i == 0 and self.no_concat:
             ops.bf3_wgrad_emb(self._ids_t[self.cur], self.row_base, self.table, self.dense_pad, dy, sc, dstW, dstb,
                               workspace=self.wg_ws[0], parts=1 if self._wgrad_reduce_deferred(i) else 3)
@@ -584,11 +597,15 @@
                         self.side.wait_event(self.ev_dw_done)
                         if self._wgrad_reduce_deferred(i) and self.h2:
                             ops.h2_wgrad_emb(self._ids_t[self.cur], self.row_base, self.table, self.tab_amax, self.dense_pad, self.dense_amax,
-                                             dy, self.dh0_amax, sc, dstW, dstb, workspace=self.wg_ws[0], parts=2)
+                                             dy, self.dh0_amax, sc, dstW, dstb, workspace=self.wg_ws[0], parts=2,
+                                             w_planes=self._w0_planes_of(dstW))
                         elif self._wgrad_reduce_deferred(i):
                             ops.bf3_wgrad_emb(self._ids_t[self.cur], self.row_base, self.table, self.dense_pad, dy, sc, dstW, dstb,
                                               workspace=self.wg_ws[0], parts=2)
-                        self.wplanes[i].refresh()
+                        if i == 0 and self.h2:
+                            self.wplanes[i].refresh(from_wgrad=True)
+                        else:
+                            self.wplanes[i].refresh()
                         self.ev_planes.record(self.side)
                     self._planes_pending = True
                     self._planes_pending_l0 = (i == 0)
@@ -640,7 +657,7 @@
         self.ev_dw_done.record()
         with torch.cuda.stream(rs):
             rs.wait_event(self.ev_dw_done)
-            self.wplanes[0].refresh()
+            self.wplanes[0].refresh(from_wgrad=True)
             self.ev_planes.record(rs)
         self._planes_pending = True
         self._planes_pending_l0 = True
diff --git a/deep_recommenders_amd/ops.py b/deep_recommenders_amd/ops.py
--- a/deep_recommenders_amd/ops.py
+++ b/deep_recommenders_amd/ops.py
@@ -1,3 +1,4 @@
+import ctypes
 from typing import Optional, Sequence
 
 import torch
@@ -468,6 +469,7 @@
         self.flags = torch.empty(n, dtype=torch.uint8, device=device)
         self.dup_heads = torch.empty(n, dtype=torch.int32, device=device)
         self.dup_count = torch.zeros(4, dtype=torch.int32, device=device)
+        self.ticket = torch.zeros(1, dtype=torch.int32, device=device)
         self.workspace = emb_sort_workspace(n, device)
 
     def sorted_len(self):
@@ -479,9 +481,9 @@
     B, F = ids.shape
     if plan is None or plan.n < B * F:
         plan = SortPlan(B * F, ids.device)
-    check(lib().dr_emb_sort_slots(ptr(ids), B, F, ptr(row_base), int(num_rows), ptr(plan.rows), ptr(plan.slots),
-                                  ptr(plan.flags), ptr(plan.dup_heads), ptr(plan.dup_count), ptr(plan.workspace),
-                                  plan.workspace.numel(), stream_ptr()), "dr_emb_sort_slots")
+    check(lib().dr_emb_sort_slots_merged(ptr(ids), B, F, ptr(row_base), int(num_rows), ptr(plan.rows), ptr(plan.slots),
+                                         ptr(plan.flags), ptr(plan.dup_heads), ptr(plan.dup_count), ptr(plan.workspace),
+                                         plan.workspace.numel(), ptr(plan.ticket), stream_ptr()), "dr_emb_sort_slots_merged")
     return plan
 
 
@@ -493,9 +495,10 @@
         assert ids_t_out.shape == (F, B) and ids_t_out.dtype == torch.int32 and ids_t_out.is_contiguous()
     if plan is None or plan.n < B * F:
         plan = SortPlan(B * F, keys.device)
-    check(lib().dr_hash_sort_slots(ptr(keys), B, F, ptr(col_buckets), ptr(ids_out), ptr(ids_t_out), ptr(row_base), int(num_rows),
-                                   ptr(plan.rows), ptr(plan.slots), ptr(plan.flags), ptr(plan.dup_heads), ptr(plan.dup_count),
-                                   ptr(plan.workspace), plan.workspace.numel(), stream_ptr()), "dr_hash_sort_slots")
+    check(lib().dr_hash_sort_slots_merged(ptr(keys), B, F, ptr(col_buckets), ptr(ids_out), ptr(ids_t_out), ptr(row_base), int(num_rows),
+                                          ptr(plan.rows), ptr(plan.slots), ptr(plan.flags), ptr(plan.dup_heads), ptr(plan.dup_count),
+                                          ptr(plan.workspace), plan.workspace.numel(), ptr(plan.ticket), stream_ptr()),
+          "dr_hash_sort_slots_merged")
     return plan
 
 
@@ -1136,6 +1139,19 @@
     return amax
 
 
+def h2_place_scratch(device):
+    return torch.zeros(257, dtype=torch.int32, device=device)
+
+
+def h2_place_dense(src, dst_pad, amax, scratch):
+    B, Nd = src.shape
+    assert src.dtype == torch.float32 and src.stride(1) == 1 and dst_pad.dtype == torch.float32
+    assert dst_pad.shape == (B, 32) and dst_pad.is_contiguous() and scratch.numel() >= 257
+    check(lib().dr_h2_place_dense(ptr(src), src.stride(0) if B > 1 else max(Nd, 1), B, Nd, ptr(dst_pad), ptr(amax), ptr(scratch),
+                                  stream_ptr()), "dr_h2_place_dense")
+    return amax
+
+
 def h2_amax_value(amax):
     return float(amax.view(torch.float32).item())
 
@@ -1209,24 +1225,47 @@
     return out
 
 
-def h2_wgrad(x, x_amax, dy, dy_amax, scale, dstW, dstb=None, workspace=None):
+def _wgrad_parts_of(w_planes, dstW, F, N):
+    assert dstW.data_ptr() == w_planes.W.data_ptr() and dstW.shape == w_planes.W.shape and dstW.stride(0) == w_planes.W.stride(0)
+    if w_planes._wg_parts is None:
+        w_planes._wg_parts = torch.zeros(lib().dr_h2_wgrad_amax_parts_max(F, N), dtype=torch.int32, device=dstW.device)
+    return w_planes._wg_parts
+
+
+def h2_wgrad(x, x_amax, dy, dy_amax, scale, dstW, dstb=None, workspace=None, w_planes=None):
     R, F = x.shape
     N = dy.shape[1]
     assert x.stride(1) == 1 and dy.stride(1) == 1 and dstW.shape == (F, N) and dstW.stride(1) == 1 and dy.shape[0] == R
     if workspace is None:
         workspace = bf3_wgrad_workspace(R, F, N, x.device)
+    if w_planes is not None:
+        wparts, np_ = _wgrad_parts_of(w_planes, dstW, F, N), ctypes.c_int32(0)
+        check(lib().dr_h2_wgrad_ex(ptr(x), x.stride(0), ptr(x_amax), ptr(dy), dy.stride(0), ptr(dy_amax), R, F, N, float(scale), ptr(dstW),
+                                   dstW.stride(0), ptr(dstb), ptr(workspace), workspace.numel() * 4, ptr(wparts), ctypes.byref(np_),
+                                   stream_ptr()), "dr_h2_wgrad_ex")
+        w_planes._wg_np = int(np_.value)
+        return dstW
     check(lib().dr_h2_wgrad(ptr(x), x.stride(0), ptr(x_amax), ptr(dy), dy.stride(0), ptr(dy_amax), R, F, N, float(scale), ptr(dstW),
                             dstW.stride(0), ptr(dstb), ptr(workspace), workspace.numel() * 4, stream_ptr()), "dr_h2_wgrad")
     return dstW
 
 
-def h2_wgrad_emb(ids_t, row_base, table, table_amax, dense_pad, dense_amax, dy, dy_amax, scale, dstW, dstb=None, workspace=None, parts=3):
+def h2_wgrad_emb(ids_t, row_base, table, table_amax, dense_pad, dense_amax, dy, dy_amax, scale, dstW, dstb=None, workspace=None, parts=3,
+                 w_planes=None):
     nf, R = ids_t.shape
     F, N = dstW.shape
     assert ids_t.dtype == torch.int32 and ids_t.is_contiguous() and dy.stride(1) == 1 and dstW.stride(1) == 1 and dy.shape == (R, N)
     assert dense_pad is None or (dense_pad.shape == (R, 32) and dense_pad.is_contiguous())
     if workspace is None:
         workspace = bf3_wgrad_workspace(R, F, N, dy.device)
+    if w_planes is not None and (parts & 2):
+        wparts, np_ = _wgrad_parts_of(w_planes, dstW, F, N), ctypes.c_int32(0)
+        check(lib().dr_h2_wgrad_emb_ex(ptr(ids_t), R, nf, ptr(row_base), ptr(table), table.shape[1], ptr(table_amax), ptr(dense_pad),
+                                       ptr(dense_amax), ptr(dy), dy.stride(0), ptr(dy_amax), F, N, float(scale), ptr(dstW), dstW.stride(0),
+                                       ptr(dstb), ptr(workspace), workspace.numel() * 4, int(parts), ptr(wparts), ctypes.byref(np_),
+                                       stream_ptr()), "dr_h2_wgrad_emb_ex")
+        w_planes._wg_np = int(np_.value)
+        return dstW
     check(lib().dr_h2_wgrad_emb(ptr(ids_t), R, nf, ptr(row_base), ptr(table), table.shape[1], ptr(table_amax), ptr(dense_pad), ptr(dense_amax),
                                 ptr(dy), dy.stride(0), ptr(dy_amax), F, N, float(scale), ptr(dstW), dstW.stride(0), ptr(dstb), ptr(workspace),
                                 workspace.numel() * 4, int(parts), stream_ptr()), "dr_h2_wgrad_emb")
@@ -1243,9 +1282,10 @@
         self.w = H2Planes(K, N, W.device, self.amax)
         self._w_alt = H2Planes(K, N, W.device, h2_record(W.device)) if double_buffer else None
         self._parts = None
+        self._wg_parts, self._wg_np = None, 0
         self.refresh()
 
-    def refresh(self):
+    def refresh(self, from_wgrad=False):
         if self._parts is None:
             self._parts = torch.zeros(256, dtype=torch.int32, device=self.W.device)
         K, N = self.W.shape
@@ -1253,6 +1293,13 @@
             self.w, self._w_alt = self._w_alt, self.w
             self.amax = self.w.amax
             self.wt.amax = self.amax
+        wg_np, self._wg_np = self._wg_np, 0
+        if from_wgrad and wg_np > 0:
+            check(lib().dr_h2_refresh_weight_from_parts(ptr(self.W), self.W.stride(0), K, N, ptr(self.w.buf), self.w.plane_stride, self.w.ld,
+                                                        ptr(self.wt.buf), self.wt.plane_stride, self.wt.ld, ptr(self.amax),
+                                                        ptr(self._wg_parts), wg_np, stream_ptr()), "dr_h2_refresh_weight_from_parts")
+            self._ver = self.W._version
+            return
         check(lib().dr_h2_refresh_weight(ptr(self.W), self.W.stride(0), K, N, ptr(self.w.buf), self.w.plane_stride, self.w.ld,
                                          ptr(self.wt.buf), self.wt.plane_stride, self.wt.ld, ptr(self.amax), ptr(self._parts),
                                          stream_ptr()), "dr_h2_refresh_weight")
diff --git a/include/dr_hotpath.h b/include/dr_hotpath.h
--- a/include/dr_hotpath.h
+++ b/include/dr_hotpath.h
@@ -75,6 +75,13 @@
                        int32_t* ids_t_out, const int64_t* row_base, int64_t num_rows, int64_t* sorted_rows,
                        int32_t* sorted_slots, uint8_t* unique_flags, int32_t* dup_heads, int32_t* dup_count, void* workspace,
                        int64_t workspace_bytes, dr_stream_t stream);
+int dr_emb_sort_slots_merged(const int64_t* ids, int64_t B, int32_t F, const int64_t* row_base, int64_t num_rows,
+                             int64_t* sorted_rows, int32_t* sorted_slots, uint8_t* unique_flags, int32_t* dup_heads,
+                             int32_t* dup_count, void* workspace, int64_t workspace_bytes, uint32_t* ticket, dr_stream_t stream);
+int dr_hash_sort_slots_merged(const int64_t* keys, int64_t B, int32_t F, const uint64_t* col_buckets, int64_t* ids_out,
+                              int32_t* ids_t_out, const int64_t* row_base, int64_t num_rows, int64_t* sorted_rows,
+                              int32_t* sorted_slots, uint8_t* unique_flags, int32_t* dup_heads, int32_t* dup_count, void* workspace,
+                              int64_t workspace_bytes, uint32_t* ticket, dr_stream_t stream);
 int dr_emb_pool_bwd_sorted(const int64_t* ids, const int64_t* row_base, const int64_t* sorted_rows,
                            const int32_t* sorted_slots, const uint8_t* unique_flags,
                            const int32_t* dup_heads, const int32_t* dup_count, int64_t B, int32_t F,
@@ -340,6 +347,11 @@
                 int64_t row_offset, int64_t col_offset, int32_t transpose, const uint32_t* amax, dr_stream_t stream);
 int dr_h2_refresh_weight(const float* W, int64_t ldw, int64_t K, int32_t N, void* w_planes, int64_t w_plane_stride, int64_t w_ld,
                          void* wt_planes, int64_t wt_plane_stride, int64_t wt_ld, uint32_t* amax, uint32_t* parts, dr_stream_t stream);
+int dr_h2_refresh_weight_from_parts(const float* W, int64_t ldw, int64_t K, int32_t N, void* w_planes, int64_t w_plane_stride, int64_t w_ld,
+                                    void* wt_planes, int64_t wt_plane_stride, int64_t wt_ld, uint32_t* amax, const uint32_t* parts,
+                                    int32_t np, dr_stream_t stream);
+int dr_h2_place_dense(const float* src, int64_t ld_src, int64_t B, int32_t Nd, float* dst_pad, uint32_t* amax, uint32_t* scratch,
+                      dr_stream_t stream);
 int dr_h2_linear_nt(const float* A, int64_t lda, const uint32_t* a_amax, const void* b_planes, int64_t b_plane_stride, int64_t b_ld,
                     const uint32_t* b_amax, int64_t M, int32_t N, int32_t K, const float* bias, int32_t act, const float* mask,
                     int64_t ld_mask, int32_t accumulate, float* C, int64_t ldc, uint32_t* c_amax, dr_stream_t stream);
@@ -365,6 +377,14 @@
                     const uint32_t* table_amax, const float* dense_pad, const uint32_t* dense_amax, const float* dy, int64_t ld_dy,
                     const uint32_t* dy_amax, int32_t F, int32_t N, float scale, float* dstW, int64_t ld_w, float* dstb, void* workspace,
                     int64_t workspace_bytes, int32_t parts, dr_stream_t stream);
+int64_t dr_h2_wgrad_amax_parts_max(int32_t F, int32_t N);
+int dr_h2_wgrad_ex(const float* x, int64_t ld_x, const uint32_t* x_amax, const float* dy, int64_t ld_dy, const uint32_t* dy_amax, int64_t R,
+                   int32_t F, int32_t N, float scale, float* dstW, int64_t ld_w, float* dstb, void* workspace, int64_t workspace_bytes,
+                   uint32_t* w_amax_parts, int32_t* w_amax_np, dr_stream_t stream);
+int dr_h2_wgrad_emb_ex(const int32_t* ids_t, int64_t R, int32_t nf, const int64_t* row_base, const float* table, int32_t D,
+                       const uint32_t* table_amax, const float* dense_pad, const uint32_t* dense_amax, const float* dy, int64_t ld_dy,
+                       const uint32_t* dy_amax, int32_t F, int32_t N, float scale, float* dstW, int64_t ld_w, float* dstb, void* workspace,
+                       int64_t workspace_bytes, int32_t parts, uint32_t* w_amax_parts, int32_t* w_amax_np, dr_stream_t stream);
 
 
 int dr_cin_fwd(const float* x0, const float* x, int64_t B, int32_t H0, int32_t Hk, int32_t D, const float* W,
```

Result: slower. 62.99 million examples/sec (-7.8%).
